# ZPP-Robotics/OSQP-Solver

Hardware: AMD Instinct MI355X
Metric: QPs/sec on a 1024-QP batch of box-QPs (n=512, m=1024), OSQP defaults; ADMM iters/sec alongside (higher is better)
Workload: dtype f64

## Files before the change

include/mi_osqp.h:

```cpp
#ifndef MI_OSQP_H
#define MI_OSQP_H

#include <stdint.h>

#ifdef __cplusplus
extern "C" {
#endif

typedef enum {
  MI_OSQP_OK = 0,
  MI_OSQP_ERR_INVALID_DATA = 1,
  MI_OSQP_ERR_INVALID_SETTINGS = 2,
  MI_OSQP_ERR_PATTERN_CHANGED = 3,
  MI_OSQP_ERR_NONCONVEX = 4,
  MI_OSQP_ERR_DEVICE = 5,
  MI_OSQP_ERR_NULL = 6,
  MI_OSQP_ERR_ALLOC = 7
} mi_osqp_error;

typedef enum {
  MI_OSQP_EXIT_OPTIMAL = 0,
  MI_OSQP_EXIT_PRIMAL_INFEASIBLE = 1,
  MI_OSQP_EXIT_DUAL_INFEASIBLE = 2,
  MI_OSQP_EXIT_OPTIMAL_INACCURATE = 3,
  MI_OSQP_EXIT_PRIMAL_INFEASIBLE_INACCURATE = 4,
  MI_OSQP_EXIT_DUAL_INFEASIBLE_INACCURATE = 5,
  MI_OSQP_EXIT_MAX_ITERATIONS = 6,
  MI_OSQP_EXIT_INTERRUPTED = 7,
  MI_OSQP_EXIT_TIME_LIMIT_REACHED = 8,
  MI_OSQP_EXIT_NON_CONVEX = 9,
  MI_OSQP_EXIT_UNKNOWN = 10
} mi_osqp_exit_code;

typedef struct {
  double  rho;
  double  sigma;
  int64_t scaling;
  int64_t adaptive_rho;
  int64_t adaptive_rho_interval;
  double  adaptive_rho_tolerance;
  int64_t max_iter;
  double  eps_abs;
  double  eps_rel;
  double  eps_prim_inf;
  double  eps_dual_inf;
  double  alpha;
  int64_t scaled_termination;
  int64_t check_termination;
  int64_t warm_start;
  int64_t verbose;
  int64_t polish;
  int64_t polish_refine_iter;
  double  delta;
} mi_osqp_settings;

typedef struct {
  int64_t iter;
  int64_t status_val;
  int64_t exit_code;
  double  obj_val;
  double  pri_res;
  double  dua_res;
  int64_t rho_updates;
  double  rho_estimate;
  double  rho;
  int64_t status_polish;
} mi_osqp_info;

typedef struct {
  int64_t n, m, N, batch, tile, n_tiles;
  int64_t nnz_P_triu, nnz_A, nnz_KKT, nnz_L;
  int64_t n_supernodes, n_blocks;
  int64_t fwd_levels, bwd_levels, fwd_slots, bwd_slots, chk_slots;
  int64_t lds_bytes, threads_per_block;
  int64_t dense_tail_rows, dense_tail_slots;
  double  setup_seconds_host, setup_seconds_factor, setup_seconds_upload;
  int64_t nnz_L_before_tail;
  int64_t solve_groups, solve_group_threads;
  int64_t resident_state, lds_bytes_iterate;
  int64_t pipelined_refactors;
  int64_t resident_factor_steps, lds_bytes_factor;
  int64_t dense_tail_tasks, dense_tail_waves_used, dense_tail_wave_tasks_max;
} mi_osqp_stats;

typedef struct mi_osqp_solver mi_osqp_solver;
typedef struct mi_osqp_batch  mi_osqp_batch;

void        mi_osqp_default_settings(mi_osqp_settings *s);
const char *mi_osqp_exit_code_name(int64_t exit_code);
const char *mi_osqp_error_name(int64_t err);
const char *mi_osqp_version(void);
const char *mi_osqp_last_error(void);

int mi_osqp_setup(mi_osqp_solver **out, int64_t n, int64_t m,
                  const int64_t *P_colptr, const int64_t *P_rowidx, const double *P_val,
                  const double *q,
                  const int64_t *A_colptr, const int64_t *A_rowidx, const double *A_val,
                  const double *l, const double *u, const mi_osqp_settings *settings);
int mi_osqp_update_A(mi_osqp_solver *h, const int64_t *A_colptr, const int64_t *A_rowidx,
                     const double *A_val);
int mi_osqp_update_bounds(mi_osqp_solver *h, const double *l, const double *u);
int mi_osqp_update_A_bounds(mi_osqp_solver *h, const int64_t *A_colptr, const int64_t *A_rowidx, const double *A_val,
                            const double *l, const double *u);
int mi_osqp_warm_start_x(mi_osqp_solver *h, const double *x);
int mi_osqp_update_q(mi_osqp_solver *h, const double *q);
int mi_osqp_update_P(mi_osqp_solver *h, const int64_t *P_colptr, const int64_t *P_rowidx, const double *P_val);
int mi_osqp_update_P_A(mi_osqp_solver *h, const int64_t *P_colptr, const int64_t *P_rowidx, const double *P_val,
                       const int64_t *A_colptr, const int64_t *A_rowidx, const double *A_val);
int mi_osqp_warm_start_y(mi_osqp_solver *h, const double *y);
int mi_osqp_solve(mi_osqp_solver *h, mi_osqp_info *info);
int mi_osqp_get_primal(mi_osqp_solver *h, double *x_out);
int mi_osqp_get_dual(mi_osqp_solver *h, double *y_out);
int mi_osqp_get_prim_inf_cert(mi_osqp_solver *h, double *dy_out );
int mi_osqp_get_dual_inf_cert(mi_osqp_solver *h, double *dx_out );
int mi_osqp_adjoint(mi_osqp_solver *h, const double *dx, const double *dy, double *dq, double *dP, double *dA, double *dl, double *du,
                    int32_t *status);
int mi_osqp_get_stats(mi_osqp_solver *h, mi_osqp_stats *st);
int mi_osqp_get_settings(mi_osqp_solver *h, mi_osqp_settings *out);
int mi_osqp_update_settings(mi_osqp_solver *h, const mi_osqp_settings *s);
void mi_osqp_free(mi_osqp_solver *h);

int mi_osqp_batch_setup(mi_osqp_batch **out, int64_t B, int64_t n, int64_t m,
                        const int64_t *P_colptr, const int64_t *P_rowidx, const double *P_val,
                        const double *q,
                        const int64_t *A_colptr, const int64_t *A_rowidx, const double *A_val,
                        const double *l, const double *u, const mi_osqp_settings *settings,
                        int64_t device);
int mi_osqp_batch_update_A(mi_osqp_batch *h, const int64_t *A_colptr, const int64_t *A_rowidx,
                           const double *A_val);
int mi_osqp_batch_update_bounds(mi_osqp_batch *h, const double *l, const double *u);
int mi_osqp_batch_update_A_bounds(mi_osqp_batch *h, const int64_t *A_colptr, const int64_t *A_rowidx, const double *A_val,
                                  const double *l, const double *u);
int mi_osqp_batch_warm_start_x(mi_osqp_batch *h, const double *x);
int mi_osqp_batch_update_q(mi_osqp_batch *h, const double *q);
int mi_osqp_batch_update_P(mi_osqp_batch *h, const int64_t *P_colptr, const int64_t *P_rowidx, const double *P_val);
int mi_osqp_batch_update_P_A(mi_osqp_batch *h, const int64_t *P_colptr, const int64_t *P_rowidx, const double *P_val,
                             const int64_t *A_colptr, const int64_t *A_rowidx, const double *A_val);
int mi_osqp_batch_warm_start_y(mi_osqp_batch *h, const double *y);
int mi_osqp_batch_get_P_upper_pattern(mi_osqp_batch *h, int64_t *colptr, int64_t *rowidx, int64_t *nnz_out);
int mi_osqp_batch_solve(mi_osqp_batch *h);
int mi_osqp_batch_get_primal(mi_osqp_batch *h, double *x_out );
int mi_osqp_batch_get_dual(mi_osqp_batch *h, double *y_out );
int mi_osqp_batch_get_info(mi_osqp_batch *h, mi_osqp_info *info );
int mi_osqp_batch_get_prim_inf_cert(mi_osqp_batch *h, double *dy_out );
int mi_osqp_batch_get_dual_inf_cert(mi_osqp_batch *h, double *dx_out );
int mi_osqp_batch_get_stats(mi_osqp_batch *h, mi_osqp_stats *st);
int mi_osqp_batch_get_ordering(mi_osqp_batch *h, int64_t *kkt_perm);
void mi_osqp_batch_free(mi_osqp_batch *h);
int mi_osqp_prefetch_analysis(int64_t B, int64_t n, int64_t m, const int64_t *Pp, const int64_t *Pi,
                              const int64_t *Ap, const int64_t *Ai, int64_t device);
void mi_osqp_release_device_cache(void);

int mi_osqp_batch_update_bounds_device(mi_osqp_batch *h, const double *d_l, const double *d_u, void *stream);
int mi_osqp_batch_update_A_bounds_device(mi_osqp_batch *h, const double *d_Av, const double *d_l, const double *d_u, void *stream);
int mi_osqp_batch_update_q_device(mi_osqp_batch *h, const double *d_q, void *stream);
int mi_osqp_batch_update_P_device(mi_osqp_batch *h, const double *d_Pv, void *stream);
int mi_osqp_batch_update_P_A_bounds_device(mi_osqp_batch *h, const double *d_Pv, const double *d_Av, const double *d_l, const double *d_u,
                                           void *stream);
int mi_osqp_batch_solve_device(mi_osqp_batch *h, double *d_x_out, int32_t *d_status, int32_t *d_iters, void *stream);
int mi_osqp_batch_reset(mi_osqp_batch *h);
int mi_osqp_batch_last_solve_stats(mi_osqp_batch *h, int64_t *total_iters, int64_t *kernel_launches,
                                   double *device_seconds, double *refactor_seconds, int64_t *refactor_count,
                                   double *compact_seconds);
int mi_osqp_batch_last_polish_stats(mi_osqp_batch *h, int64_t *polished, int64_t *accepted, double *seconds);
int mi_osqp_batch_get_polish_active(mi_osqp_batch *h, int8_t *act);
// ... 40 lines not shown
  MI_GOMP_MODEL_DH_CHAIN = 6
} mi_gomp_model;
typedef struct { int32_t model; int32_t is_gripper; double radius; double param[12]; } mi_gomp_ball;
typedef struct { double dir[2]; double point[3]; int32_t below; int32_t reserved; } mi_gomp_line;
typedef struct mi_gomp_scene mi_gomp_scene;
int mi_gomp_scene_create(mi_gomp_scene **out, mi_osqp_batch *h, int64_t dims, int64_t waypoints,
                         int64_t n_balls, const mi_gomp_ball *balls, int64_t n_lines, const mi_gomp_line *lines,
                         const double *con_lo, const double *con_hi);
typedef struct { int32_t n_joints; int32_t reserved; double a[8], d[8], alpha[8], theta0[8]; } mi_gomp_chain;
int mi_gomp_scene_create_chain(mi_gomp_scene **out, mi_osqp_batch *h, int64_t dims, int64_t waypoints,
                               const mi_gomp_chain *chain, int64_t n_balls, const mi_gomp_ball *balls,
                               int64_t n_lines, const mi_gomp_line *lines, const double *con_lo, const double *con_hi);
typedef struct { double a[3], b[3]; double radius; double margin; } mi_gomp_capsule;
int mi_gomp_scene_create_world(mi_gomp_scene **out, mi_osqp_batch *h, int64_t dims, int64_t waypoints,
                               const mi_gomp_chain *chain, int64_t n_balls, const mi_gomp_ball *balls,
                               int64_t n_lines, const mi_gomp_line *lines, int64_t n_capsules, const mi_gomp_capsule *capsules,
                               const double *con_lo, const double *con_hi);
void mi_gomp_scene_free(mi_gomp_scene *sc);
int mi_gomp_scene_set_rows(mi_gomp_scene *sc, int64_t n_ids, const int64_t *ids, const double *A_val, const double *l, const double *u);
int mi_gomp_scene_get_rows(mi_gomp_scene *sc, int64_t id, double *A_val, double *l, double *u);
int mi_gomp_assemble_some(mi_gomp_scene *sc, int64_t n_ids, const int64_t *ids, const double *x, int32_t *ok_out);
int mi_gomp_relinearise_some(mi_gomp_scene *sc, int64_t n_ids, const int64_t *ids, const double *x, int32_t *ok_out);

typedef struct mi_osqp_multi mi_osqp_multi;
int mi_osqp_multi_batch_setup(mi_osqp_multi **out, int64_t n_devices, const int64_t *devices,
                              int64_t B, int64_t n, int64_t m,
                              const int64_t *P_colptr, const int64_t *P_rowidx, const double *P_val,
                              const double *q,
                              const int64_t *A_colptr, const int64_t *A_rowidx, const double *A_val,
                              const double *l, const double *u, const mi_osqp_settings *settings);
int mi_osqp_multi_batch_update_A(mi_osqp_multi *h, const int64_t *A_colptr, const int64_t *A_rowidx, const double *A_val);
int mi_osqp_multi_batch_update_bounds(mi_osqp_multi *h, const double *l, const double *u);
int mi_osqp_multi_batch_update_A_bounds(mi_osqp_multi *h, const int64_t *A_colptr, const int64_t *A_rowidx, const double *A_val,
                                        const double *l, const double *u);
int mi_osqp_multi_batch_warm_start_x(mi_osqp_multi *h, const double *x);
int mi_osqp_multi_batch_update_q(mi_osqp_multi *h, const double *q);
int mi_osqp_multi_batch_update_P(mi_osqp_multi *h, const int64_t *P_colptr, const int64_t *P_rowidx, const double *P_val);
int mi_osqp_multi_batch_update_P_A(mi_osqp_multi *h, const int64_t *P_colptr, const int64_t *P_rowidx, const double *P_val,
                                   const int64_t *A_colptr, const int64_t *A_rowidx, const double *A_val);
int mi_osqp_multi_batch_warm_start_y(mi_osqp_multi *h, const double *y);
int mi_osqp_multi_batch_get_settings(mi_osqp_multi *h, mi_osqp_settings *out);
int mi_osqp_multi_batch_update_settings(mi_osqp_multi *h, const mi_osqp_settings *s);
int mi_osqp_multi_batch_update_rho_each(mi_osqp_multi *h, const double *rho );
int mi_osqp_multi_batch_solve(mi_osqp_multi *h);
int mi_osqp_multi_batch_solve_async(mi_osqp_multi *h);
int mi_osqp_multi_batch_wait(mi_osqp_multi *h);
int mi_osqp_multi_batch_get_primal(mi_osqp_multi *h, double *x_out );
int mi_osqp_multi_batch_get_dual(mi_osqp_multi *h, double *y_out );
int mi_osqp_multi_batch_get_info(mi_osqp_multi *h, mi_osqp_info *info );
int mi_osqp_multi_batch_get_prim_inf_cert(mi_osqp_multi *h, double *dy_out );
int mi_osqp_multi_batch_get_dual_inf_cert(mi_osqp_multi *h, double *dx_out );
int64_t mi_osqp_multi_batch_shards(mi_osqp_multi *h);
int mi_osqp_multi_batch_shard(mi_osqp_multi *h, int64_t k, int64_t *device, int64_t *begin, int64_t *end, mi_osqp_batch **handle);
void mi_osqp_multi_batch_free(mi_osqp_multi *h);

int mi_osqp_batch_spmv(mi_osqp_batch *h, const double *d_x, const double *d_y,
                       double *d_Px, double *d_Aty, double *d_Ax, void *stream);
int mi_osqp_batch_kkt_solve(mi_osqp_batch *h, const double *d_rhs, double *d_sol, void *stream);
int mi_osqp_batch_refactor_device(mi_osqp_batch *h);
int mi_osqp_batch_kernel_time(mi_osqp_batch *h, double *avg_ms, int64_t *launches);
int mi_osqp_batch_refactor_time(mi_osqp_batch *h, double *factor_ms, double *tail_ms, int64_t *launches, int64_t *qps);
int mi_osqp_batch_refactor_peak(mi_osqp_batch *h, int64_t *qps, double *factor_ms, double *tail_ms);

int mi_osqp_batch_get_scaling(mi_osqp_batch *h, double *D , double *E , double *c );

int mi_osqp_debug_host_kkt_solve(int64_t n, int64_t m,
                                 const int64_t *P_colptr, const int64_t *P_rowidx, const double *P_val,
                                 const int64_t *A_colptr, const int64_t *A_rowidx, const double *A_val,
                                 const double *l, const double *u, const mi_osqp_settings *settings,
                                 int64_t tile, const double *rhs ,
                                 double *sol_schedule , double *sol_direct ,
                                 mi_osqp_stats *st);

int mi_osqp_debug_host_block_factor(int64_t n, int64_t m,
                                    const int64_t *P_colptr, const int64_t *P_rowidx, const double *P_val,
                                    const int64_t *A_colptr, const int64_t *A_rowidx, const double *A_val,
                                    const double *l, const double *u, const mi_osqp_settings *settings,
                                    double *max_rel_diff_L, double *max_rel_diff_Dinv, int64_t *counts);

int mi_osqp_debug_refactor_chunks(int64_t n_flagged, const int64_t *flagged, int64_t n_active, const int64_t *active, int64_t tile,
                                  int64_t chunk_qps, int64_t max_chunks, int64_t *n_chunks, int64_t *work_begin, int64_t *tiles,
                                  int64_t *tile_begin);

int mi_osqp_debug_trace_kkt_solve(mi_osqp_batch *h, int32_t which, const double *d_rhs, double *d_sol,
                                  uint32_t *out, int64_t out_capacity_words, int64_t *dims);

#ifdef __cplusplus
}
#endif
#endif
```

osqp-solver_amd/__init__.py:

```python
import ctypes as C
import os

import numpy as np

try:
    import torch
except ImportError:
    torch = None

from . import build as _build

_HERE = os.path.dirname(os.path.abspath(__file__))
_LIB = None

EXIT_NAMES = ["kOptimal", "kPrimalInfeasible", "kDualInfeasible", "kOptimalInaccurate",
              "kPrimalInfeasibleInaccurate", "kDualInfeasibleInaccurate", "kMaxIterations",
              "kInterrupted", "kTimeLimitReached", "kNonConvex", "kUnknown"]
K_OPTIMAL = 0


class Settings(C.Structure):
    _fields_ = [("rho", C.c_double), ("sigma", C.c_double), ("scaling", C.c_int64),
                ("adaptive_rho", C.c_int64), ("adaptive_rho_interval", C.c_int64),
                ("adaptive_rho_tolerance", C.c_double), ("max_iter", C.c_int64),
                ("eps_abs", C.c_double), ("eps_rel", C.c_double), ("eps_prim_inf", C.c_double),
                ("eps_dual_inf", C.c_double), ("alpha", C.c_double), ("scaled_termination", C.c_int64),
                ("check_termination", C.c_int64), ("warm_start", C.c_int64), ("verbose", C.c_int64),
                ("polish", C.c_int64), ("polish_refine_iter", C.c_int64), ("delta", C.c_double)]


class Info(C.Structure):
    _fields_ = [("iter", C.c_int64), ("status_val", C.c_int64), ("exit_code", C.c_int64),
                ("obj_val", C.c_double), ("pri_res", C.c_double), ("dua_res", C.c_double),
                ("rho_updates", C.c_int64), ("rho_estimate", C.c_double), ("rho", C.c_double),
                ("status_polish", C.c_int64)]

    def as_dict(self):
        return {k: getattr(self, k) for k, _ in self._fields_}


class Stats(C.Structure):
    _fields_ = [(k, C.c_int64) for k in
                ("n", "m", "N", "batch", "tile", "n_tiles", "nnz_P_triu", "nnz_A", "nnz_KKT", "nnz_L",
                 "n_supernodes", "n_blocks", "fwd_levels", "bwd_levels", "fwd_slots", "bwd_slots",
                 "chk_slots", "lds_bytes", "threads_per_block", "dense_tail_rows", "dense_tail_slots")] + \
               [(k, C.c_double) for k in ("setup_seconds_host", "setup_seconds_factor", "setup_seconds_upload")] + \
               [("nnz_L_before_tail", C.c_int64), ("solve_groups", C.c_int64), ("solve_group_threads", C.c_int64),
                ("resident_state", C.c_int64), ("lds_bytes_iterate", C.c_int64), ("pipelined_refactors", C.c_int64),
                ("resident_factor_steps", C.c_int64), ("lds_bytes_factor", C.c_int64),
                ("dense_tail_tasks", C.c_int64), ("dense_tail_waves_used", C.c_int64), ("dense_tail_wave_tasks_max", C.c_int64)]

    def as_dict(self):
        return {k: getattr(self, k) for k, _ in self._fields_}


class MiOsqpError(RuntimeError):
    def __init__(self, code, where):
        self.code = int(code)
        L = lib()
        msg = L.mi_osqp_error_name(int(code)).decode()
        extra = L.mi_osqp_last_error().decode()
        super().__init__(f"{where}: error {int(code)} ({msg}) {extra}")


def lib():
    global _LIB
    if _LIB is None:
        path = os.path.join(_HERE, "libmi_osqp.so")
        if os.environ.get("MI_OSQP_LIBRARY"):
            path = os.environ["MI_OSQP_LIBRARY"]
        else:
            try:
                path = _build.build()
            except Exception as e:
                if not os.path.exists(path):
                    raise ImportError(f"libmi_osqp.so missing and could not be built: {e}") from e
        L = C.CDLL(path)
        ip, dp, vp = C.POINTER(C.c_int64), C.POINTER(C.c_double), C.c_void_p
        L.mi_osqp_default_settings.argtypes = [C.POINTER(Settings)]
        for f in ("mi_osqp_exit_code_name", "mi_osqp_error_name"):
            getattr(L, f).restype = C.c_char_p; getattr(L, f).argtypes = [C.c_int64]
        L.mi_osqp_version.restype = C.c_char_p
        L.mi_osqp_last_error.restype = C.c_char_p
        L.mi_osqp_batch_setup.argtypes = [C.POINTER(vp), C.c_int64, C.c_int64, C.c_int64, ip, ip, dp, dp, ip, ip, dp,
                                          dp, dp, C.POINTER(Settings), C.c_int64]
        L.mi_osqp_batch_update_A.argtypes = [vp, ip, ip, dp]
        L.mi_osqp_batch_update_A_bounds.argtypes = [vp, ip, ip, dp, dp, dp]
        L.mi_osqp_batch_update_bounds.argtypes = [vp, dp, dp]
        L.mi_osqp_batch_warm_start_x.argtypes = [vp, dp]
        L.mi_osqp_batch_update_q.argtypes = [vp, dp]
        L.mi_osqp_batch_update_q_device.argtypes = [vp, vp, vp]
        L.mi_osqp_batch_update_P.argtypes = [vp, ip, ip, dp]
        L.mi_osqp_batch_update_P_A.argtypes = [vp, ip, ip, dp, ip, ip, dp]
        L.mi_osqp_batch_warm_start_y.argtypes = [vp, dp]
        L.mi_osqp_batch_get_P_upper_pattern.argtypes = [vp, ip, ip, ip]
        L.mi_osqp_batch_update_P_device.argtypes = [vp, vp, vp]
        L.mi_osqp_batch_update_P_A_bounds_device.argtypes = [vp, vp, vp, vp, vp, vp]
        L.mi_osqp_batch_update_P_some.argtypes = [vp, C.c_int64, ip, dp]
        L.mi_osqp_batch_update_P_A_bounds_some.argtypes = [vp, C.c_int64, ip, dp, dp, dp, dp]
        L.mi_osqp_batch_update_q_some.argtypes = [vp, C.c_int64, ip, dp]
        L.mi_osqp_batch_warm_start_y_some.argtypes = [vp, C.c_int64, ip, dp]
        L.mi_osqp_settings_update_check.argtypes = [C.POINTER(Settings), C.POINTER(Settings)]
        L.mi_osqp_batch_get_settings.argtypes = [vp, C.POINTER(Settings)]
        L.mi_osqp_batch_update_settings.argtypes = [vp, C.POINTER(Settings)]
        L.mi_osqp_batch_update_rho_each.argtypes = [vp, dp]
        L.mi_osqp_batch_update_rho_some.argtypes = [vp, C.c_int64, ip, dp]
        L.mi_osqp_get_settings.argtypes = [vp, C.POINTER(Settings)]
        L.mi_osqp_update_settings.argtypes = [vp, C.POINTER(Settings)]
        L.mi_osqp_multi_batch_get_settings.argtypes = [vp, C.POINTER(Settings)]
        L.mi_osqp_multi_batch_update_settings.argtypes = [vp, C.POINTER(Settings)]
        L.mi_osqp_multi_batch_update_rho_each.argtypes = [vp, dp]
        L.mi_osqp_batch_solve.argtypes = [vp]
        L.mi_osqp_batch_get_primal.argtypes = [vp, dp]
        L.mi_osqp_batch_get_dual.argtypes = [vp, dp]
        L.mi_osqp_batch_get_info.argtypes = [vp, C.POINTER(Info)]
        for f in ("mi_osqp_get_prim_inf_cert", "mi_osqp_get_dual_inf_cert", "mi_osqp_batch_get_prim_inf_cert",
                  "mi_osqp_batch_get_dual_inf_cert", "mi_osqp_multi_batch_get_prim_inf_cert", "mi_osqp_multi_batch_get_dual_inf_cert"):
            getattr(L, f).argtypes = [vp, dp]
        L.mi_osqp_batch_get_prim_inf_cert_some.argtypes = [vp, C.c_int64, ip, dp]
        L.mi_osqp_batch_get_dual_inf_cert_some.argtypes = [vp, C.c_int64, ip, dp]
        L.mi_osqp_batch_get_stats.argtypes = [vp, C.POINTER(Stats)]
        L.mi_osqp_batch_get_ordering.argtypes = [vp, ip]
        L.mi_osqp_batch_free.argtypes = [vp]; L.mi_osqp_batch_free.restype = None
        L.mi_osqp_batch_update_bounds_device.argtypes = [vp, vp, vp, vp]
        L.mi_osqp_batch_update_A_bounds_device.argtypes = [vp, vp, vp, vp, vp]
        L.mi_osqp_batch_solve_device.argtypes = [vp, vp, vp, vp, vp]
        L.mi_osqp_batch_reset.argtypes = [vp]
        L.mi_osqp_batch_refactor_device.argtypes = [vp]
        L.mi_osqp_batch_last_solve_stats.argtypes = [vp, ip, ip, dp, dp, ip, dp]
        L.mi_osqp_batch_last_polish_stats.argtypes = [vp, ip, ip, dp]
        L.mi_osqp_batch_get_polish_active.argtypes = [vp, C.POINTER(C.c_int8)]
        L.mi_osqp_batch_adjoint.argtypes = [vp, dp, dp, dp, dp, dp, dp, dp, C.POINTER(C.c_int32)]
        L.mi_osqp_adjoint.argtypes = [vp, dp, dp, dp, dp, dp, dp, dp, C.POINTER(C.c_int32)]
        L.mi_osqp_batch_adjoint_device.argtypes = [vp] * 10
        L.mi_osqp_batch_get_scaling.argtypes = [vp, dp, dp, dp]
        L.mi_osqp_batch_spmv.argtypes = [vp, vp, vp, vp, vp, vp, vp]
        L.mi_osqp_batch_kkt_solve.argtypes = [vp, vp, vp, vp]
        L.mi_osqp_batch_kernel_time.argtypes = [vp, dp, ip]
        L.mi_osqp_batch_refactor_time.argtypes = [vp, dp, dp, ip, ip]
        L.mi_osqp_batch_refactor_peak.argtypes = [vp, ip, dp, dp]
        L.mi_osqp_batch_reinit_some.argtypes = [vp, C.c_int64, ip, dp, dp, dp]
        L.mi_osqp_batch_update_A_bounds_some.argtypes = [vp, C.c_int64, ip, dp, dp, dp]
        L.mi_osqp_batch_warm_start_x_some.argtypes = [vp, C.c_int64, ip, dp]
        L.mi_osqp_batch_solve_begin_some.argtypes = [vp, C.c_int64, ip]
        L.mi_osqp_batch_polish_some.argtypes = [vp, C.c_int64, ip]
        L.mi_osqp_batch_advance.argtypes = [vp, C.c_int64]
        L.mi_osqp_batch_poll.argtypes = [vp, C.c_int64, ip, ip, C.c_int64]
        L.mi_osqp_batch_get_primal_some.argtypes = [vp, C.c_int64, ip, dp]
        L.mi_osqp_batch_get_dual_some.argtypes = [vp, C.c_int64, ip, dp]
        L.mi_osqp_batch_get_info_some.argtypes = [vp, C.c_int64, ip, C.POINTER(Info)]
        L.mi_osqp_batch_running.argtypes = [vp]; L.mi_osqp_batch_running.restype = C.c_int64
        L.mi_osqp_batch_ring_wraps.argtypes = [vp]; L.mi_osqp_batch_ring_wraps.restype = C.c_int64
        L.mi_osqp_release_device_cache.argtypes = []; L.mi_osqp_release_device_cache.restype = None
        L.mi_osqp_setup.argtypes = [C.POINTER(vp), C.c_int64, C.c_int64, ip, ip, dp, dp, ip, ip, dp, dp, dp, C.POINTER(Settings)]
        L.mi_osqp_update_A.argtypes = [vp, ip, ip, dp]
        L.mi_osqp_update_bounds.argtypes = [vp, dp, dp]
        L.mi_osqp_warm_start_x.argtypes = [vp, dp]
        L.mi_osqp_update_q.argtypes = [vp, dp]
        L.mi_osqp_update_P.argtypes = [vp, ip, ip, dp]
        L.mi_osqp_update_P_A.argtypes = [vp, ip, ip, dp, ip, ip, dp]
        L.mi_osqp_warm_start_y.argtypes = [vp, dp]
        L.mi_osqp_solve.argtypes = [vp, C.POINTER(Info)]
        L.mi_osqp_get_primal.argtypes = [vp, dp]
        L.mi_osqp_get_dual.argtypes = [vp, dp]
        L.mi_osqp_get_stats.argtypes = [vp, C.POINTER(Stats)]
        L.mi_osqp_free.argtypes = [vp]; L.mi_osqp_free.restype = None
        L.mi_osqp_multi_batch_setup.argtypes = [C.POINTER(vp), C.c_int64, ip, C.c_int64, C.c_int64, C.c_int64, ip, ip, dp, dp,
                                                ip, ip, dp, dp, dp, C.POINTER(Settings)]
        L.mi_osqp_multi_batch_update_A.argtypes = [vp, ip, ip, dp]
        L.mi_osqp_multi_batch_update_bounds.argtypes = [vp, dp, dp]
        L.mi_osqp_multi_batch_update_A_bounds.argtypes = [vp, ip, ip, dp, dp, dp]
        L.mi_osqp_multi_batch_warm_start_x.argtypes = [vp, dp]
        L.mi_osqp_multi_batch_update_q.argtypes = [vp, dp]
        L.mi_osqp_multi_batch_update_P.argtypes = [vp, ip, ip, dp]
        L.mi_osqp_multi_batch_update_P_A.argtypes = [vp, ip, ip, dp, ip, ip, dp]
        L.mi_osqp_multi_batch_warm_start_y.argtypes = [vp, dp]
        L.mi_osqp_multi_batch_solve.argtypes = [vp]
        L.mi_osqp_multi_batch_solve_async.argtypes = [vp]
        L.mi_osqp_multi_batch_wait.argtypes = [vp]
        L.mi_osqp_multi_batch_get_primal.argtypes = [vp, dp]
        L.mi_osqp_multi_batch_get_dual.argtypes = [vp, dp]
        L.mi_osqp_multi_batch_get_info.argtypes = [vp, C.POINTER(Info)]
        L.mi_osqp_multi_batch_shards.argtypes = [vp]; L.mi_osqp_multi_batch_shards.restype = C.c_int64
        L.mi_osqp_multi_batch_shard.argtypes = [vp, C.c_int64, ip, ip, ip, C.POINTER(vp)]
        L.mi_osqp_multi_batch_free.argtypes = [vp]; L.mi_osqp_multi_batch_free.restype = None
        L.mi_osqp_debug_host_kkt_solve.argtypes = [C.c_int64, C.c_int64, ip, ip, dp, ip, ip, dp, dp, dp,
                                                   C.POINTER(Settings), C.c_int64, dp, dp, dp, C.POINTER(Stats)]
        L.mi_osqp_debug_refactor_chunks.argtypes = [C.c_int64, ip, C.c_int64, ip, C.c_int64, C.c_int64, C.c_int64, ip, ip, ip, ip]
        L.mi_osqp_prefetch_analysis.argtypes = [C.c_int64, C.c_int64, C.c_int64, ip, ip, ip, ip, C.c_int64]
        L.mi_osqp_debug_host_block_factor.argtypes = [C.c_int64, C.c_int64, ip, ip, dp, ip, ip, dp, dp, dp,
                                                      C.POINTER(Settings), dp, dp, ip]
        _LIB = L
    return _LIB


def host_cores():
    try:
        n = len(os.sched_getaffinity(0))
    except Exception:
        n = os.cpu_count() or 1
    for path in ("/sys/fs/cgroup/cpu.max",):
        try:
            quota, period = open(path).read().split()[:2]
            if quota != "max":
                n = min(n, max(1, int(round(int(quota) / int(period)))))
        except Exception:
            pass
    try:
        q = int(open("/sys/fs/cgroup/cpu/cpu.cfs_quota_us").read())
        p = int(open("/sys/fs/cgroup/cpu/cpu.cfs_period_us").read())
        if q > 0:
            n = min(n, max(1, int(round(q / p))))
    except Exception:
        pass
    return n


def default_settings(**kw):
    s = Settings()
    lib().mi_osqp_default_settings(C.byref(s))
    for k, v in kw.items():
        if not hasattr(s, k):
            raise KeyError(k)
        setattr(s, k, v)
    return s


class HandleSettings(Settings):

    def bind(self, getter):
        self._getter = getter
        return self

    def __call__(self):
        out = Settings()
        self._getter(out)
        C.memmove(C.byref(self), C.byref(out), C.sizeof(Settings))
        return out


def settings_update_check(in_force, wanted):
    return int(lib().mi_osqp_settings_update_check(C.byref(in_force), C.byref(wanted)))


def _handle_settings(kw, get_name, owner):
    import weakref
    hs = HandleSettings()
    C.memmove(C.byref(hs), C.byref(default_settings(**kw)), C.sizeof(Settings))
    ref = weakref.ref(owner)

    def getter(out):
        _chk(getattr(lib(), get_name)(ref()._h, C.byref(out)), get_name)
    return hs.bind(getter)


def _update_settings(self, fn_name, fields):
    s = self.settings()
    for k, v in fields.items():
        if not hasattr(s, k):
            raise KeyError(k)
        setattr(s, k, v)
    _chk(getattr(lib(), fn_name)(self._h, C.byref(s)), fn_name)
    return self.settings()


def _i64(a):
    return np.ascontiguousarray(a, dtype=np.int64)


def _f64(a):
    return np.ascontiguousarray(a, dtype=np.float64)
# ... 479 lines not shown

    def __init__(self, constraints, P, q=None, **settings):
        l, A, u = constraints
        self._b = BatchSolver(P, _csc(P).data, q, A, _csc(A).data, l, u, **settings)

    def update(self, constraints):
        l, A, u = constraints
        A = _csc(A)
        try:
            self._b.update_A(A.data, A_pattern=A)
            self._b.update_bounds(l, u)
        except MiOsqpError as e:
            raise ValueError(str(e)) from e

    def setWarmStart(self, x):
        self._b.warm_start_x(x)

    def update_settings(self, **fields):
        return self._b.update_settings(**fields)

    def solve(self):
        info = self._b.solve()[0]
        return int(info.exit_code), self._b.primal()[0]

    def info(self):
        return self._b.info()[0]

    def dual(self):
        return self._b.dual()[0]

    def prim_inf_cert(self):
        return self._b.prim_inf_cert()[0]

    def dual_inf_cert(self):
        return self._b.dual_inf_cert()[0]

    def adjoint(self, dx, dy=None):
        out = self._b.adjoint(dx, dy)
        return {k: (int(v[0]) if k == "status" else v[0]) for k, v in out.items()}

    def stats(self):
        return self._b.stats()


def debug_host_kkt_solve(P, A, l, u, rhs, tri_waves=0, **settings):
    L = lib()
    P, A = _csc(P), _csc(A)
    n, m = A.shape[1], A.shape[0]
    s = default_settings(**settings)
    rhs = _f64(rhs)
    sol_s, sol_d = np.empty(n + m), np.empty(n + m)
    st = Stats()
    Pp, Pi, Px = _i64(P.indptr), _i64(P.indices), _f64(P.data)
    Ap, Ai, Ax = _i64(A.indptr), _i64(A.indices), _f64(A.data)
    l, u = _f64(l), _f64(u)
    rc = L.mi_osqp_debug_host_kkt_solve(n, m, _ip(Pp), _ip(Pi), _dp(Px), _ip(Ap), _ip(Ai), _dp(Ax), _dp(l), _dp(u),
                                        C.byref(s), 1 + int(tri_waves), _dp(rhs), _dp(sol_s), _dp(sol_d), C.byref(st))
    _chk(rc, "debug_host_kkt_solve")
    return sol_s, sol_d, st.as_dict()


def prefetch_analysis(P, A, B=1, device=-1, check=True):
    L = lib()
    P, A = _csc(P), _csc(A)
    n, m = A.shape[1], A.shape[0]
    Pp, Pi, Ap, Ai = _i64(P.indptr), _i64(P.indices), _i64(A.indptr), _i64(A.indices)
    rc = L.mi_osqp_prefetch_analysis(B, n, m, _ip(Pp), _ip(Pi), _ip(Ap), _ip(Ai), device)
    if check:
        _chk(rc, "prefetch_analysis")
    return rc


def debug_refactor_chunks(flagged, active, tile, chunk_qps, max_chunks=8):
    f, a = _i64(flagged), _i64(active)
    nch = C.c_int64()
    wb = np.zeros(max_chunks + 2, dtype=np.int64); tb = np.zeros(max_chunks + 2, dtype=np.int64)
    tl = np.zeros(max(1, len(a)), dtype=np.int64)
    _chk(lib().mi_osqp_debug_refactor_chunks(len(f), _ip(f), len(a), _ip(a), tile, chunk_qps, max_chunks, C.byref(nch), _ip(wb), _ip(tl),
                                             _ip(tb)), "debug_refactor_chunks")
    k = int(nch.value)
    return ([f[wb[c]:wb[c + 1]].tolist() for c in range(k)], [tl[tb[c]:tb[c + 1]].tolist() for c in range(k)])


def debug_host_block_factor(P, A, l, u, **settings):
    L = lib()
    P, A = _csc(P), _csc(A)
    n, m = A.shape[1], A.shape[0]
    s = default_settings(**settings)
    Pp, Pi, Px = _i64(P.indptr), _i64(P.indices), _f64(P.data)
    Ap, Ai, Ax = _i64(A.indptr), _i64(A.indices), _f64(A.data)
    l, u = _f64(l), _f64(u)
    dL, dD = C.c_double(), C.c_double()
    cnt = (C.c_int64 * 4)()
    rc = L.mi_osqp_debug_host_block_factor(n, m, _ip(Pp), _ip(Pi), _dp(Px), _ip(Ap), _ip(Ai), _dp(Ax), _dp(l), _dp(u),
                                           C.byref(s), C.byref(dL), C.byref(dD), cnt)
    _chk(rc, "debug_host_block_factor")
    return dL.value, dD.value, dict(blocks=cnt[0], triples=cnt[1], storage=cnt[2], levels=cnt[3])
```

osqp-solver_amd/csrc/device_types.h:

```cpp
#pragma once
#include <hip/hip_runtime.h>
#include <stdint.h>

namespace miosqp {

#define MI_CHUNK 16

struct SchedDev {
  const uint32_t *step, *idxw;
  const uint64_t *idxw64;
  const uint32_t *lvl_pos, *tail_bar;
  int n_phases, nw, n_levels;
  uint32_t n_steps, n_slots;
};

struct DenseTailDev {
  int s, k, n_phases;
  uint32_t n_steps;
  const uint32_t *task;
  const uint32_t *wave_task, *wave_step, *tail_bar;
};

enum { DS_C = 0, DS_CINV, DS_RHO, DS_RHO_EST, DS_PRI_RES, DS_DUA_RES, DS_OBJ, DS_COUNT };
enum { IS_STATUS = 0, IS_ITER, IS_RHO_UPDATES, IS_DONE, IS_NEED_REFACTOR, IS_CUR, IS_PENDING, IS_EPOCH, IS_COUNT };

struct KernelArgs {
  int n, m, N, B;
  SchedDev fwd, bwd, chk;
  const uint32_t *pinv;
  const uint32_t *xloc;
  const double *fwd_val, *bwd_val, *chk_val, *dinv;
  DenseTailDev dt;
  const double *dt_val;
  const double *fwd_val0, *bwd_val0, *dt_val0;
  const int *use_work;
  double *x, *z, *y;
  const double *q, *l, *u, *rho_vec, *rho_inv, *Dsc, *Dsc_inv, *Esc, *Esc_inv;
  double *dx, *dy, *out1, *out2, *dscal;
  int *iscal;
  double *x_out, *y_out;
  double *cert_out;
  int cert_stride;
  double *xs_global;
  int xs_len;
  int rs_off;
  int rf_off;
  int wide;
  double sigma, alpha, eps_abs, eps_rel, eps_prim_inf, eps_dual_inf, rho_tolerance;
  int check_termination, rho_interval, max_iter, scaled_termination, scaling, adaptive_rho;
  int iter_begin, iter_end;
  int op_out_lds;
  int info_at_end;
  int mw_groups;
  unsigned *mw_bar;
  double *mw_scratch;
  int df;
  unsigned df_shadow;
  const unsigned char *rflag;
  const int *sel;
  const int *tiles;
};

struct FactorArgs {
  int n, m, N, B, nnzP, nnzK, pa_len, n_levels, force_all;
  int debug_skip;
  uint32_t storage;
  SchedDev fwd, bwd;
  const uint32_t *blk, *lvl, *utask, *tri4, *dtask, *ttask, *asm_dst, *asm_src;
  const uint32_t *ubig;
  int *use_work;
  const int32_t *fwd_srcblk, *bwd_srcblk;
  const double *pa_val, *l, *u, *dscal;
  double *rho_vec, *rho_inv, *Lblk, *Dl, *dinv_scratch, *fwd_val, *bwd_val, *dinv;
  int *iscal, *npos;
  int home_bt;
  const int *work;
  double sigma;
  int dt_k;
  int mw_groups;
  unsigned *mw_bar;
  const signed char *pmask;
  const int32_t *arow;
  int *pstat;
  double pdelta;
};

struct TailArgs {
  int n, N, s, k, kbt, home_bt;
  uint32_t storage, n_slots;
  int n_lt, n_ltcol;
  uint32_t n_quads;
  int nh;
  uint32_t cs_doubles;
  const int *work;
  const uint32_t *lt_pos, *ltcol_col, *tile_tab, *wave_tiles, *diag_tile;
  const uint64_t *asm_q64;
  const int32_t *src_tile;
  const uint32_t *dt_task, *dt_task_step;
  uint32_t n_tasks;
  const double *Lblk, *Dl;
  double *Sd, *dt_val, *dinv;
  int *npos, *iscal;
  unsigned long long *trace;
  int *pstat;
};
hipError_t launch_tail(const TailArgs &a, int nwork, size_t lds_asm, size_t lds, hipStream_t st);

struct PolishArgs {
  int *stat;
  signed char *act;
  double *sol;
  int refine_iter;
  int inner;
  double delta;
};
hipError_t launch_polish_active(const KernelArgs &a, const PolishArgs &p, int BT, hipStream_t st);
hipError_t launch_polish_active_list(const KernelArgs &a, const PolishArgs &p, const int *slots, int nslots, int BT, hipStream_t st);
hipError_t launch_polish_publish(const KernelArgs &a, const PolishArgs &p, const int *slots, int nslots, int *host_stat, int BT, hipStream_t st);
hipError_t launch_polish(const KernelArgs &a, const PolishArgs &p, int BT, int tiles, int threads, size_t lds, int n_cus, hipStream_t st);
struct AdjointArgs {
  const double *gx, *gy;
  double *dq, *dP, *dA, *dl, *du;
  const int32_t *prow, *pcol, *arow, *acol;
  int nnzP, nnzA;
};
hipError_t launch_adjoint(const KernelArgs &a, const PolishArgs &p, const AdjointArgs &g, int BT, int tiles, int threads, size_t lds, int n_cus, hipStream_t st);
hipError_t launch_adjoint_finish(const int *stat, const AdjointArgs &g, int32_t *status, int B, int n, int m, hipStream_t st);
hipError_t launch_factor(const FactorArgs &a, int BT, int tiles, int threads, hipStream_t st);
size_t factor_lds_bytes(int BT, int threads);
bool factor_fits_lds(const FactorArgs &a, int threads);

int max_coresident_groups(int threads, size_t lds, int n_cus);
int max_coresident_factor_groups(int threads, int n_cus);
hipError_t launch_iterate(const KernelArgs &a, int BT, int tiles, int threads, size_t lds, hipStream_t st);
int rf_head_steps();
int rf_lds_steps();
hipError_t launch_check(const KernelArgs &a, int BT, int tiles, int threads, size_t lds, hipStream_t st);
hipError_t launch_advance(const KernelArgs &a, int BT, int tiles, int threads, size_t lds, hipStream_t st, int max_segments, int seg_len,
                          int *host_is, double *host_ds, unsigned *stop, unsigned seq, unsigned *counter, unsigned *host_done);
hipError_t launch_spmv(const KernelArgs &a, int BT, int tiles, int threads, size_t lds, hipStream_t st,
                       const double *x, const double *y, double *Px, double *Aty, double *Ax);
struct SpmvFused {
  const uint32_t *ptr, *ent;
  const double *pa_val;
  int pa_len;
  const uint32_t *ell, *rowid;
  int n_pass;
  uint32_t ell_off[4], ell_k[4];
};
hipError_t launch_spmv_fused(const KernelArgs &a, const SpmvFused &t, int BT, int tiles, int n_cus, hipStream_t st,
                             const double *x, const double *y, double *Px, double *Aty, double *Ax);
size_t spmv_fused_lds_bytes(int n, int m, int pa_len, int BT);
hipError_t launch_kkt_solve(const KernelArgs &a, int BT, int tiles, int threads, size_t lds, hipStream_t st,
                            const double *rhs, double *sol);
hipError_t launch_kkt_trace(const KernelArgs &a, int BT, int tiles, int threads, size_t lds, hipStream_t st,
                            const double *rhs, double *sol, uint32_t *trace, uint32_t words);
hipError_t launch_warm_start(const KernelArgs &a, int BT, int tiles, int threads, size_t lds, hipStream_t st,
                             const double *x0);
hipError_t launch_interleave(const double *src, double *dst, const int *ids, int nq, int len, int BT, hipStream_t st);
hipError_t launch_scatter(const double *src, double *dst, const int *map, const int *ids, int nq, int srclen,
                          const SchedDev &sd, int BT, hipStream_t st);
hipError_t launch_deinterleave(const double *src, double *dst, int nq, int len, int BT, hipStream_t st);
struct RuizArgs {
  int n, m, nnzP, nnzA, B, BT, iters;
  const int *ids;
  int raw_by_qp;
  int fresh;
  const double *rawP, *rawq;
  const int32_t *Prow, *Pcol, *Arow, *Acol;
  const double *rawPnew;
  const double *rawA;
  const double *rawl, *rawu;
  double *pa_val, *q, *Dsc, *Dsc_inv, *Esc, *Esc_inv, *l, *u, *dscal;
  double *dn, *en;
  double *pa_out;
};
hipError_t launch_ruiz(const RuizArgs &a, hipStream_t st);
hipError_t launch_lin_cost(const double *gq, const int *ids, double *q, double *rawq, const double *Dsc, const double *dscal,
                           int nq, int n, int BT, int scaling, hipStream_t st);
hipError_t launch_warm_start_y(const KernelArgs &a, int nslots, int BT, hipStream_t st, const double *y0);
hipError_t launch_start_slots(const KernelArgs &a, const int *slots, const int *clear, int nslots, int BT, int cold, hipStream_t st);
hipError_t launch_fresh_slots(const KernelArgs &a, const int *slots, int nslots, int BT, double rho0, hipStream_t st);
hipError_t launch_set_rho_slots(const KernelArgs &a, const int *slots, const double *rho, double rho_all, int nslots, int BT, hipStream_t st);
hipError_t launch_worklist(const int *iscal, int *work, int nslots, int BT, hipStream_t st);
hipError_t launch_resume_flagged(const KernelArgs &a, int nslots, int BT, hipStream_t st);
hipError_t launch_copy_slot_streams(double *dst, const double *src, const int *slots, int nslots, size_t per, hipStream_t st);
hipError_t launch_keep_rows(double *dst, const double *src, const int *ids, int n_ids, int len, hipStream_t st);
hipError_t launch_copy_flagged_streams(double *dst, const double *src, const int *flags, int want, int nslots, size_t per, hipStream_t st);
hipError_t launch_copy_slot_rows(double *dst, const double *src, const int *slots, int nslots, int len, int BT, hipStream_t st);
enum { MI_GM_UR5E_FLANGE = 1, MI_GM_UR5E_WRIST3 = 2, MI_GM_UR5E_ELBOW = 3, MI_GM_YAW_2LINK = 4, MI_GM_TABLE = 5, MI_GM_DH_CHAIN = 6 };
#define MI_GOMP_MAXD 8
struct GompChainDev { int n_joints, pad; double a[MI_GOMP_MAXD], d[MI_GOMP_MAXD], ca[MI_GOMP_MAXD], sa[MI_GOMP_MAXD], theta0[MI_GOMP_MAXD]; };
struct GompBallDev { int model, is_gripper; double radius; double param[12]; };
struct GompLineDev { double D[3], A[3]; int below, pad; };
struct GompCapsuleDev { double a[3], e[3], ee, R, margin; };
struct GompArgs {
  int dims, W, n_balls, n_lines, n, m, nnzA, n_ids, row0, write_rows;
  int n_caps, pad;
  const int *ids;
  const GompBallDev *balls;
  const GompLineDev *lines;
  const GompCapsuleDev *caps;
  double con_lo[3], con_hi[3];
  const int *aidx;
  const double *traj;
  double *A, *l, *u;
  int *ok;
  GompChainDev chain;
};
hipError_t launch_gomp_relinearise(const GompArgs &g, hipStream_t st);
hipError_t launch_gather_status(const int *iscal, int32_t *status, int32_t *iters, int B, int BT, hipStream_t st);
hipError_t launch_fail_slots(const KernelArgs &a, const int *slots, int nfail, int BT, int iter, hipStream_t st);
hipError_t launch_bounds(const double *gl, const double *gu, double *l, double *u, const double *Esc,
                         const double *rho_vec, const double *dscal, int *changed, int B, int m, int BT,
                         int scaling, hipStream_t st);

}
```

osqp-solver_amd/csrc/host_core.cpp:

```cpp
#include "host_core.hpp"
#include "sched_format.h"

#include <algorithm>
#include <cmath>
#include <cstdio>
#include <cstdlib>
#include <cstring>
#include <numeric>
#include <set>
#include <chrono>
#include <thread>

#include "../../include/mi_osqp.h"

namespace miosqp {

int validate_settings(const Settings &s) {
  if (s.scaling < 0 || s.max_iter <= 0 || s.check_termination < 0) return 1;
  if (s.adaptive_rho != 0 && s.adaptive_rho != 1) return 1;
  if (s.adaptive_rho_interval < 0 || s.adaptive_rho_tolerance < 1.0) return 1;
  if (!(s.rho > 0.0) || !(s.sigma > 0.0)) return 1;
  if (s.eps_abs < 0.0 || s.eps_rel < 0.0 || (s.eps_abs == 0.0 && s.eps_rel == 0.0)) return 1;
  if (!(s.eps_prim_inf > 0.0) || !(s.eps_dual_inf > 0.0)) return 1;
  if (!(s.alpha > 0.0) || !(s.alpha < 2.0)) return 1;
// ... 841 lines not shown
        dt.lt_pos.push_back((uint32_t)bf.lpos[p]);
      }
    }
    dt.n_lt = (int)dt.lt_pos.size(); dt.n_ltcol = (int)dt.ltcol_col.size();
    const uint16_t zero_slot = (uint16_t)dt.n_lt;
    for (auto &fr : frag) for (auto &f : fr) for (uint16_t &v : f.second) if (v == 0xFFFFu) v = zero_slot;
    struct TileRec { int I, J; std::vector<std::pair<int, int>> src; };
    std::vector<TileRec> tiles;
    for (int I = 0; I < nt; I++)
      for (int J = 0; J <= I; J++) {
        TileRec t{I, J, {}};
        size_t a = 0, b = 0;
        while (a < frag[I].size() && b < frag[J].size()) {
          if (frag[I][a].first < frag[J][b].first) a++;
          else if (frag[I][a].first > frag[J][b].first) b++;
          else { t.src.push_back({(int)a, (int)b}); a++; b++; }
        }
        tiles.push_back(std::move(t));
      }
    const int nw = 16;
    std::vector<int> order(tiles.size());
    std::iota(order.begin(), order.end(), 0);
    std::stable_sort(order.begin(), order.end(), [&](int x, int y) { return tiles[x].src.size() > tiles[y].src.size(); });
    std::vector<std::vector<int>> mine(nw);
    for (size_t d = 0; d < order.size(); d++) { const size_t round = d / nw, pos = d % nw; mine[(round & 1) ? nw - 1 - pos : pos].push_back(order[d]); }
    dt.tile_tab.clear(); dt.wave_tiles.assign(nw + 1, 0u); dt.asm_q.clear(); dt.asm_qcol.clear();
    for (int w = 0; w < nw; w++) {
      dt.wave_tiles[w] = (uint32_t)(dt.tile_tab.size() / 4);
      for (int ti : mine[w]) {
        const TileRec &t = tiles[ti];
        const uint32_t q0 = (uint32_t)(dt.asm_q.size() / 64);
        const size_t padded = (t.src.size() + 31) / 32 * 32;
        for (size_t s0 = 0; s0 < padded; s0 += 4) {
          for (int g = 0; g < 4; g++) {
            const bool real = s0 + g < t.src.size();
            const auto *fa = real ? &frag[t.I][t.src[s0 + g].first] : nullptr;
            const auto *fb = real ? &frag[t.J][t.src[s0 + g].second] : nullptr;
            dt.asm_qcol.push_back(real ? (uint16_t)fa->first : (uint16_t)0);
            for (int e = 0; e < 16; e++) dt.asm_q.push_back(real ? ((uint32_t)fa->second[e] | ((uint32_t)fb->second[e] << 16)) : ((uint32_t)zero_slot | ((uint32_t)zero_slot << 16)));
          }
        }
        const uint32_t blk_id = find_blk(ct0 + t.I, ct0 + t.J);
        dt.tile_tab.insert(dt.tile_tab.end(), {((uint32_t)t.I << 16) | (uint32_t)t.J, bf.blk[4 * blk_id], q0, (uint32_t)(dt.asm_q.size() / 64)});
      }
    }
    dt.wave_tiles[nw] = (uint32_t)(dt.tile_tab.size() / 4);
    dt.asm_q64.resize(dt.asm_q.size());
    for (size_t e = 0; e < dt.asm_q.size(); e++) {
      const uint64_t w = dt.asm_q[e], ci = dt.asm_qcol[e / 16];
      dt.asm_q64[e] = ((w & 0xFFFFu) * 8u) | ((((w >> 16) * 8u) | ((ci * 8u) << 17)) << 32);
    }
    dt.src_tile.resize(dt.src.size());
    for (size_t e = 0; e < dt.src.size(); e++) {
      const int32_t sc = dt.src[e];
      dt.src_tile[e] = sc < 0 ? sc : (int32_t)dt_tile_offset(sc % k, sc / k);
    }
    dt.diag_tile.resize(k);
    for (int i = 0; i < k; i++) dt.diag_tile[i] = dt_tile_offset(i, i);
    dt.task_step.clear();
    { uint32_t pos = 0; for (size_t t = 0; t < dt.task.size() / 4; t++) { dt.task_step.push_back(pos); pos += dt.task[4 * t + 3]; } }
  }
}


Tuning tuning_from_env() {
  Tuning t;
  if (const char *e = getenv("MI_OSQP_TILE")) { const int v = atoi(e); if (v == 1 || v == 2 || v == 4) t.tile = v; }
  if (const char *e = getenv("MI_OSQP_THREADS")) t.threads = std::max(64, std::min(1024, atoi(e) / 64 * 64));
  t.global_xs = getenv("MI_OSQP_GLOBAL_XS") != nullptr;
  if (const char *e = getenv("MI_OSQP_GROUPS")) t.groups = std::max(0, std::min(256, atoi(e)));
  if (const char *e = getenv("MI_OSQP_GROUP_THREADS")) t.group_threads = std::max(64, std::min(512, atoi(e) / 64 * 64));
  if (const char *e = getenv("MI_OSQP_ASSUME_CUS")) t.assume_cus = std::max(0, atoi(e));
  if (const char *e = getenv("MI_OSQP_FACTOR_THREADS")) t.factor_threads = std::max(64, std::min(1024, atoi(e) / 64 * 64));
  if (const char *e = getenv("MI_OSQP_FACTOR_GROUPS")) t.factor_groups = std::max(1, std::min(256, atoi(e)));
  t.ruiz = getenv("MI_OSQP_HOST_RUIZ") ? 1 : getenv("MI_OSQP_DEVICE_RUIZ") ? -1 : 0;
  if (const char *e = getenv("MI_OSQP_CONT_RING_KB")) t.cont_ring_kb = std::max(0L, atol(e));
  if (const char *e = getenv("MI_OSQP_ANALYSIS_CACHE")) t.analysis_cache = atoi(e) != 0;
  t.stream_state = getenv("MI_OSQP_STREAM_STATE") != nullptr;
  t.stream_factor = getenv("MI_OSQP_STREAM_FACTOR") != nullptr;
  if (const char *e = getenv("MI_OSQP_REFACTOR_PIPELINE")) t.refactor_pipeline = atoi(e) != 0;
  if (const char *e = getenv("MI_OSQP_REFACTOR_PIPELINE_MIN")) t.pipeline_min = std::max(0, atoi(e));
  if (const char *e = getenv("MI_OSQP_REFACTOR_CHUNKS")) t.pipeline_chunks = std::max(0, std::min(8, atoi(e)));
  if (const char *e = getenv("MI_OSQP_REFACTOR_CHUNK_QPS")) t.pipeline_chunk_qps = std::max(0, atoi(e));
  AnalysisTuning &a = t.analysis;
  if (const char *e = getenv("MI_OSQP_DENSE_TAIL")) a.dense_tail = atoi(e);
  if (const char *e = getenv("MI_OSQP_ORDERING")) a.ordering = e[0];
  if (const char *e = getenv("MI_OSQP_ND_LEAF")) a.nd_leaf = atoi(e);
  if (const char *e = getenv("MI_OSQP_RELAX")) a.relax = atoi(e);
  a.serial = getenv("MI_OSQP_SERIAL_ANALYSIS") != nullptr;
  return t;
}

RefactorChunks refactor_chunks(const std::vector<int> &flagged, const std::vector<int> &active, int bt, int chunk_qps, int max_chunks) {
  RefactorChunks rc;
  const int nq = (int)flagged.size();
  max_chunks = std::max(1, max_chunks);
  chunk_qps = std::max(1, chunk_qps);
  if ((nq + chunk_qps - 1) / chunk_qps > max_chunks) chunk_qps = (nq + max_chunks - 1) / max_chunks;
  const int n_ref = (nq + chunk_qps - 1) / chunk_qps;
  rc.n_chunks = 1 + n_ref;
  rc.work_begin.assign(1, 0);
  for (int c = 0; c <= n_ref; c++) rc.work_begin.push_back(std::min(nq, c * chunk_qps));
  std::vector<std::pair<int, int>> tc;
  size_t f = 0;
  for (size_t i = 0; i < active.size(); i++) {
    const int tile = active[i] / bt;
    if (i && active[i - 1] / bt == tile) continue;
    int chunk = 0;
    while (f < flagged.size() && flagged[f] / bt < tile) f++;
    for (size_t g = f; g < flagged.size() && flagged[g] / bt == tile; g++) chunk = 1 + (int)g / chunk_qps;
    tc.emplace_back(chunk, tile);
  }
  std::stable_sort(tc.begin(), tc.end(), [](const std::pair<int, int> &x, const std::pair<int, int> &y) { return x.first < y.first; });
  rc.tile_begin.assign((size_t)rc.n_chunks + 1, 0);
  for (const auto &p : tc) { rc.tiles.push_back(p.second); rc.tile_begin[(size_t)p.first + 1]++; }
  for (int c = 0; c < rc.n_chunks; c++) rc.tile_begin[(size_t)c + 1] += rc.tile_begin[c];
  return rc;
}


int analyze(int64_t n64, int64_t m64, const int64_t *Pp, const int64_t *Pi, const int64_t *Ap,
            const int64_t *Ai, const AnalysisTuning &tune, Analysis &an, int nwaves, int bt, int max_extra_rows, int dense_tail_max, int tri_waves, int n_tiles) {
  if (nwaves < 1 || nwaves > 16 || (bt != 1 && bt != 2 && bt != 4) || tri_waves < 0 || tri_waves > 2048) return MI_OSQP_ERR_INVALID_SETTINGS;
  if (n64 <= 0 || m64 < 0 || !Pp || !Ap || n64 + m64 > (int64_t)1 << 30) return MI_OSQP_ERR_INVALID_DATA;
  int n = (int)n64, m = (int)m64, N = n + m;
  an = Analysis();
  an.n = n; an.m = m; an.N = N;
  if (Pp[0] != 0 || Ap[0] != 0) return MI_OSQP_ERR_INVALID_DATA;
  for (int j = 0; j < n; j++) {
    if (Pp[j + 1] < Pp[j] || Ap[j + 1] < Ap[j]) return MI_OSQP_ERR_INVALID_DATA;
    for (int64_t k = Pp[j]; k < Pp[j + 1]; k++) if (Pi[k] < 0 || Pi[k] >= n) return MI_OSQP_ERR_INVALID_DATA;
    for (int64_t k = Ap[j]; k < Ap[j + 1]; k++) if (Ai[k] < 0 || Ai[k] >= m) return MI_OSQP_ERR_INVALID_DATA;
  }
  if (Pp[n] > (int64_t)1 << 30 || Ap[n] > (int64_t)1 << 30) return MI_OSQP_ERR_INVALID_DATA;
  an.Pp.assign(n + 1, 0);
  for (int j = 0; j < n; j++) {
    an.Pp[j] = (int)an.Pi.size();
    for (int64_t k = Pp[j]; k < Pp[j + 1]; k++)
      if (Pi[k] <= j) { an.Pi.push_back((int)Pi[k]); an.Psrc.push_back((int)k); }
  }
  an.Pp[n] = (int)an.Pi.size();
  an.Ap.assign(Ap, Ap + n + 1);
  an.Ai.assign(Ai, Ai + Ap[n]);
  int nnzP = an.Pp[n], nnzA = an.Ap[n];
  std::vector<int> cnt(N, 0);
  an.PisDiag.assign(nnzP, 0);
  std::vector<char> hasDiag(n, 0);
  for (int j = 0; j < n; j++)
    for (int k = an.Pp[j]; k < an.Pp[j + 1]; k++) { cnt[j]++; if (an.Pi[k] == j) { hasDiag[j] = 1; an.PisDiag[k] = 1; } }
  for (int j = 0; j < n; j++) if (!hasDiag[j]) cnt[j]++;
  for (int k = 0; k < nnzA; k++) cnt[n + an.Ai[k]]++;
  for (int r = 0; r < m; r++) cnt[n + r]++;
  an.Kp.assign(N + 1, 0);
  for (int j = 0; j < N; j++) an.Kp[j + 1] = an.Kp[j] + cnt[j];
  an.Ki.assign(an.Kp[N], 0);
  an.PtoK.assign(nnzP, 0); an.AtoK.assign(nnzA, 0); an.rhotoK.assign(m, 0);
  std::vector<int> nxt(an.Kp.begin(), an.Kp.end() - 1);
  for (int j = 0; j < n; j++) {
    for (int k = an.Pp[j]; k < an.Pp[j + 1]; k++) { int pos = nxt[j]++; an.Ki[pos] = an.Pi[k]; an.PtoK[k] = pos; }
    if (!hasDiag[j]) { int pos = nxt[j]++; an.Ki[pos] = j; an.sigmaOnlyK.push_back(pos); }
  }
  for (int j = 0; j < n; j++)
    for (int k = an.Ap[j]; k < an.Ap[j + 1]; k++) { int pos = nxt[n + an.Ai[k]]++; an.Ki[pos] = j; an.AtoK[k] = pos; }
  for (int r = 0; r < m; r++) { int pos = nxt[n + r]++; an.Ki[pos] = n + r; an.rhotoK[r] = pos; }
  an.tri_waves = tri_waves;
  an.wide = N >= 65535 || 2 * n + m >= 65535 || tri_waves > 0;
  if (max_extra_rows < 0) max_extra_rows = 1 << 30;
  if (!an.wide && max_extra_rows > 65534 - N) max_extra_rows = 65534 - N;
  auto finalize = [&](Analysis &an, const std::vector<int> &perm0, double &cost, int relax_zeros = 0, int *phases_out = nullptr, double *stream_out = nullptr) {
    an.perm = perm0;
    an.pinv.assign(N, 0);
    for (int k = 0; k < N; k++) an.pinv[an.perm[k]] = k;
    build_permuted_lower(an);
    std::vector<std::vector<int>> cols;
    std::vector<int> parent, post;
    symbolic(an, cols, parent);
    postorder(parent, post);
    {
      std::vector<int> p2(N);
      for (int k = 0; k < N; k++) p2[k] = an.perm[post[k]];
      an.perm.swap(p2);
      for (int k = 0; k < N; k++) an.pinv[an.perm[k]] = k;
    }
    build_permuted_lower(an);
    symbolic(an, cols, parent);
    an.etree = parent;
    if (relax_zeros > 0) {
      auto close = [&](int s0, int e) {
        for (int c = s0; c < e; c++) {
          std::vector<int> ns;
          ns.reserve((size_t)(e - c) + cols[e].size());
          for (int r = c + 1; r <= e; r++) ns.push_back(r);
          ns.insert(ns.end(), cols[e].begin(), cols[e].end());
          cols[c].swap(ns);
        }
      };
      int s0 = 0;
      for (int j = 0; j < N; j++) {
        bool extend = false;
        if (j + 1 < N && parent[j] == j + 1 && j + 2 - s0 <= kChunk) {
// ... 712 lines not shown
```

osqp-solver_amd/csrc/host_core.hpp:

```cpp
#pragma once

#include <cstdint>
#include <string>
#include <vector>

namespace miosqp {

constexpr double kInfty = 1e30;
constexpr double kRhoMin = 1e-6, kRhoMax = 1e6, kRhoEqOverIneq = 1e3, kRhoTol = 1e-4;
constexpr double kMinScaling = 1e-4, kMaxScaling = 1e4;
constexpr double kDivisionTol = 1.0 / kInfty;
constexpr int kChunk = 16;
constexpr uint32_t kNoRow = 0xFFFFFFFFu;

struct Settings {
  double rho = 0.1, sigma = 1e-6;
  int64_t scaling = 10, adaptive_rho = 1, adaptive_rho_interval = 0;
  double adaptive_rho_tolerance = 5.0;
  int64_t max_iter = 4000;
  double eps_abs = 1e-3, eps_rel = 1e-3, eps_prim_inf = 1e-4, eps_dual_inf = 1e-4, alpha = 1.6;
  int64_t scaled_termination = 0, check_termination = 25, warm_start = 1, verbose = 0;
  int64_t polish = 0, polish_refine_iter = 3;
  double delta = 1e-6;
};
int validate_settings(const Settings &s);

struct AnalysisTuning {
  int dense_tail = -1;
  char ordering = 0;
  int nd_leaf = 0;
  int relax = -1;
  bool serial = false;
  bool operator==(const AnalysisTuning &o) const {
    return dense_tail == o.dense_tail && ordering == o.ordering && nd_leaf == o.nd_leaf && relax == o.relax && serial == o.serial;
  }
};
struct Tuning {
  int tile = 0;
  int threads = 0;
  bool global_xs = false;
  int groups = -1;
  int group_threads = 0;
  int assume_cus = 0;
  int factor_threads = 1024;
  int factor_groups = 0;
  int ruiz = 0;
  long cont_ring_kb = -1;
  bool analysis_cache = true;
  bool stream_state = false;
  bool stream_factor = false;
  bool refactor_pipeline = true;
  int pipeline_min = 0;
  int pipeline_chunks = 0;
  int pipeline_chunk_qps = 0;
  AnalysisTuning analysis;
};
Tuning tuning_from_env();

struct RefactorChunks {
  int n_chunks = 1;
  std::vector<int> work_begin;
  std::vector<int> tiles;
  std::vector<int> tile_begin;
};
RefactorChunks refactor_chunks(const std::vector<int> &flagged, const std::vector<int> &active, int bt, int chunk_qps, int max_chunks);

struct Schedule {
  int n_phases = 0, nw = 0, bt = 1;
  bool barriers = true;
  std::vector<uint32_t> phase;
  std::vector<int> level_first_phase;
  std::vector<uint32_t> step;
  std::vector<uint32_t> step_ob;
  std::vector<uint32_t> outA;
  std::vector<uint32_t> idx;
  std::vector<uint32_t> idxw;
  std::vector<uint64_t> idxw64;
  std::vector<int32_t> src;
  uint32_t n_slots = 0;
  uint32_t n_steps = 0;
  std::vector<uint32_t> wave_range;
  std::vector<uint32_t> lvl_pos;
  std::vector<uint32_t> tail_bar;
  bool dataflow = false;
  uint32_t shadow = 0, pad = 0;
  uint32_t phys_steps() const { return n_steps; }
  size_t phase_stride() const { return 4 * (size_t)nw + 1; }
  int n_levels = 0;
};

struct BlockFactor {
  uint32_t storage = 0;
  std::vector<uint32_t> blk;
  std::vector<uint32_t> lvl;
  std::vector<uint32_t> utask;
  std::vector<uint32_t> tri;
  std::vector<uint32_t> tri4;
  std::vector<uint32_t> utask4;
  bool overflow = false;
  std::vector<uint32_t> ubig;
  std::vector<uint32_t> dtask4;
  std::vector<uint32_t> ttask4;
  std::vector<uint32_t> dtask;
  std::vector<uint32_t> ttask;
  std::vector<uint32_t> asm_dst;
  std::vector<uint32_t> asm_src;
  std::vector<int32_t> lpos;
  int n_levels = 0;
  size_t n_blocks() const { return blk.size() / 4; }
};
enum { ASM_P = 0, ASM_P_SIGMA = 1, ASM_SIGMA = 2, ASM_A = 3, ASM_NEG_RHOINV = 4 };

struct DenseTail {
  int s = 0, k = 0, nb = 0;
  int nw = 0, n_phases = 0;
  uint32_t n_steps = 0;
  std::vector<uint32_t> task;
  std::vector<uint32_t> wave_task;
  std::vector<uint32_t> wave_step;
  std::vector<uint32_t> tail_bar;
  std::vector<int32_t> src;
  std::vector<uint32_t> sblk;
  int n_lt = 0, n_ltcol = 0;
  std::vector<uint32_t> lt_pos;
  std::vector<uint32_t> ltcol_col;
  std::vector<uint32_t> tile_tab;
  std::vector<uint32_t> wave_tiles;
  std::vector<uint32_t> asm_q;
  std::vector<uint16_t> asm_qcol;
  std::vector<uint64_t> asm_q64;
  std::vector<int32_t> src_tile;
  std::vector<uint32_t> diag_tile;
  std::vector<uint32_t> task_step;
  size_t asm_lds_bytes() const { return ((size_t)n_lt + 1 + (size_t)n_ltcol) * sizeof(double); }
};
inline uint32_t dt_tile_offset(int i, int j) {
  const int I = i / 16, J = j / 16, r = i % 16, c = j % 16;
  return (uint32_t)((I * (I + 1) / 2 + J) * 256 + ((r % 4) * 16 + c) * 4 + r / 4);
}
enum { DT_DIAG = 1, DT_SWAP = 2 };

struct Analysis {
  int n = 0, m = 0, N = 0;
  bool wide = false;
  std::vector<int> Pp, Pi, Psrc;
  std::vector<int> Ap, Ai;
  std::vector<int> Kp, Ki, PtoK, AtoK, rhotoK, sigmaOnlyK;
  std::vector<char> PisDiag;
// ... 65 lines not shown
```

osqp-solver_amd/csrc/kernels.hip:

```cpp
#include <hip/hip_runtime.h>
#include <stdint.h>
#include <stdlib.h>
#include <string.h>

#include <algorithm>
#include <map>
#include <mutex>

#include "device_types.h"
#include "sched_format.h"

namespace miosqp {

static hipError_t ensure_dynamic_lds(const void *kern, size_t lds);

#define MI_INFTY 1e30
#define MI_MIN_SCALING 1e-4
#define MI_DIV_TOL 1e-30
#define MI_RHO_EST_DIV 1e-10
#define MI_RHO_MIN 1e-6
#define MI_RHO_MAX 1e6
#define MI_NOROW 0xFFFFFFFFu
#ifdef MI_OSQP_DEBUG_BUILD
#define MI_DBG_SKIP(a) ((a).debug_skip)
// ... 2017 lines not shown
#define MI_QS(k, j) Ss[MI_BS(4 * g + (k), b, (j))]
#pragma unroll
  for (int k = 0; k < 4; k++) MI_QS(k, i) = (ok && (uint32_t)k < w) ? Lb[((size_t)off + k * w + i) * BT + b] : 0.0;
  wave_sync();
#pragma unroll
  for (int j = 0; j < 4; j++) {
    const bool on = ok && (uint32_t)j < w;
    const double d = MI_QS(j, j);
    const double di = 1.0 / d;
    double lij = 0.0;
    if (on && i > j) { lij = MI_QS(j, i) * di; MI_QS(j, i) = lij; }
    if (on && i == j) {
      Dl[((size_t)c0 + j) * BT + b] = d; dinv[((size_t)c0 + j) * BT + b] = di;
      if (d > 0.0) npos++;
    }
    wave_sync();
    if (on && i > j) {
      const double ld = lij * d;
      for (int k = j + 1; k <= i; k++) MI_QS(k, i) -= ld * MI_QS(j, k);
    }
    wave_sync();
  }
  if (ok) { for (int k = 0; k < i; k++) Lb[((size_t)off + k * w + i) * BT + b] = MI_QS(k, i); }
#pragma unroll
  for (int j = 2; j >= 0; j--) {
    const bool on = ok && (uint32_t)(j + 2) <= w && i > j;
    double x = 0.0;
    if (on) {
      x = -MI_QS(j, i);
      for (int p2 = j + 1; p2 < i; p2++) x = fma(-MI_QS(p2, i), MI_QS(j, p2), x);
    }
    wave_sync();
    if (on) MI_QS(j, i) = x;
    wave_sync();
  }
  if (ok && w >= 2) { for (int k = 0; k < i; k++) Lb[((size_t)off + (size_t)i * w + k) * BT + b] = MI_QS(k, i); }
}
template <int BT>
__device__ __forceinline__ void fct_trsm_quad(double *Lb, const double *dinv, double *Ss, const uint4 td, const bool valid, int lane) {
  const int g = lane / (MI_CHUNK * BT), i = (lane / BT) % MI_CHUNK, b = lane % BT;
  const uint32_t off = td.x, h = td.z >> 8, w = td.z & 255u, c0 = td.y, db_off = td.w;
#pragma unroll
  for (int k = 0; k < 4; k++) MI_QS(k, i) = (valid && (uint32_t)k < w && (uint32_t)i < w && i > k) ? Lb[((size_t)db_off + k * w + i) * BT + b] : 0.0;
  wave_sync();
  if (valid && (uint32_t)i < h) {
    double ld[4];
#pragma unroll
    for (int j = 0; j < 4; j++) {
      if ((uint32_t)j < w) {
        double v = Lb[((size_t)off + j * h + i) * BT + b];
#pragma unroll
        for (int k = 0; k < j; k++) v = fma(-ld[k], MI_QS(k, j), v);
        ld[j] = v;
        Lb[((size_t)off + j * h + i) * BT + b] = v * dinv[((size_t)c0 + j) * BT + b];
      }
    }
  }
  wave_sync();
#undef MI_QS
}

template <int BT, bool LBL = false>
__global__ __launch_bounds__(1024) void factor_kernel(FactorArgs a) {
  extern __shared__ double smem[];
  bool multi = false;
  if constexpr (BT == 1) multi = a.mw_groups > 1;
  const unsigned G = multi ? (unsigned)a.mw_groups : 1u;
  const int tile = (int)(blockIdx.x / G), gidx = (int)(blockIdx.x % G);
  const Mw mw{a.mw_bar + 4 * (size_t)tile, G};
  const int tid = gidx * (int)blockDim.x + (int)threadIdx.x, nthr = (int)(blockDim.x * G);
  const int lane = tid & 63, wave = __builtin_amdgcn_readfirstlane(tid >> 6), nw = nthr >> 6, b = tid % BT;
  auto sync = [&]() { if constexpr (BT == 1) wg_or_grid_barrier(mw); else __syncthreads(); };
  const int m = a.m, N = a.N;
  const int slot = a.work ? a.work[tile * BT + b] : tile * BT + b;
  const size_t hbt = (size_t)a.home_bt;
  const size_t home = slot >= 0 ? (size_t)slot / hbt : 0, hb = slot >= 0 ? (size_t)slot % hbt : 0;
  auto H = [&](size_t len, size_t i) { return (home * len + i) * hbt + hb; };
  int flag = 0;
  if (slot >= 0) flag = a.work ? 1 : (a.force_all ? (slot < a.B) : a.iscal[H(IS_COUNT, IS_NEED_REFACTOR)]);
  if (!__syncthreads_or(flag)) return;
  double *Ss = smem + (size_t)(threadIdx.x >> 6) * MI_CHUNK * MI_CHUNK * BT;
  double *lds_rest = smem + (size_t)(blockDim.x >> 6) * MI_CHUNK * MI_CHUNK * BT;
  double *Lb, *Dl;
  if constexpr (LBL) { Lb = lds_rest; Dl = lds_rest + (size_t)a.storage * BT; }
  else { Lb = a.Lblk + (size_t)tile * a.storage * BT; Dl = a.Dl + (size_t)tile * N * BT; }
  const double rho = a.dscal[H(DS_COUNT, DS_RHO)];
  if (flag && !a.force_all && !a.pmask) {
    for (int e = tid; e < m * BT; e += nthr) {
      const size_t k = H(m, e / BT);
      const double l = a.l[k], u = a.u[k];
      double rv;
      if (l < -MI_INFTY * MI_MIN_SCALING && u > MI_INFTY * MI_MIN_SCALING) rv = MI_RHO_MIN;
      else if (u - l < 1e-4) rv = 1e3 * rho;
      else rv = rho;
      a.rho_vec[k] = rv; a.rho_inv[k] = 1.0 / rv;
    }
  }
  {
    const size_t tot = (size_t)a.storage * BT, pairs = tot / 2;
    double2 *L2p = reinterpret_cast<double2 *>(Lb);
    for (size_t e = tid; e < pairs; e += nthr) L2p[e] = make_double2(0.0, 0.0);
    if (tid == 0 && (tot & 1)) Lb[tot - 1] = 0.0;
    if (multi && tid == 0 && slot >= 0) a.npos[slot] = 0;
  }
  sync();
  {
    constexpr int UA = 2;
    const int tot = a.nnzK * BT;
    for (int e0 = tid; e0 < tot; e0 += nthr * UA) {
      uint32_t src[UA], dst[UA];
      double v[UA];
#pragma unroll
      for (int u = 0; u < UA; u++) {
        const int e = e0 + u * nthr;
        const int k = e < tot ? e / BT : 0;
        src[u] = a.asm_src[k]; dst[u] = a.asm_dst[k];
      }
#pragma unroll
      for (int u = 0; u < UA; u++) {
        const uint32_t kind = src[u] >> 29, idx = src[u] & 0x1FFFFFFFu;
        if (kind == 0) v[u] = a.pa_val[H(a.pa_len, idx)];
        else if (kind == 1) v[u] = a.pa_val[H(a.pa_len, idx)] + a.sigma;
        else if (kind == 2) v[u] = a.sigma;
        else if (kind == 3) {
          const bool off = a.pmask && (slot < 0 || a.pmask[(size_t)slot * m + a.arow[idx]] == 0);
          v[u] = off ? 0.0 : a.pa_val[H(a.pa_len, (size_t)a.nnzP + idx)];
        }
        else v[u] = a.pmask ? -a.pdelta : -a.rho_inv[H(m, idx)];
      }
#pragma unroll
      for (int u = 0; u < UA; u++) if (e0 + u * nthr < tot) Lb[(size_t)dst[u] * BT + b] = v[u];
    }
  }
  sync();
  int npos = 0, bad_inertia = 0;
  double *dnew;
  if constexpr (LBL) dnew = lds_rest + ((size_t)a.storage + (size_t)N) * BT;
  else dnew = a.dinv_scratch + (size_t)tile * N * BT;
  for (int L = 0; L < a.n_levels; L++) {
    const uint32_t *lv = a.lvl + 6 * L;
    const uint4 *ut4 = reinterpret_cast<const uint4 *>(a.utask), *dt4 = reinterpret_cast<const uint4 *>(a.dtask), *tt4 = reinterpret_cast<const uint4 *>(a.ttask);
    if (lv[1] > lv[0]) {
      uint32_t ub = lv[1];
      if constexpr (BT <= 2) { if (!(MI_DBG_SKIP(a) & 32)) ub = a.ubig[3 * L]; }
      uint32_t t = lv[0] + wave;
      uint4 nxt = t < ub ? ut4[t] : make_uint4(0, 0, 0, 0);
      for (; t < ub; t += nw) {
        const uint4 cur = nxt;
        if (t + nw < ub) nxt = ut4[t + nw];
        fct_update<BT>(a, Lb, Dl, Ss, cur, lane);
      }
      if constexpr (BT <= 2) {
        constexpr uint32_t NG = 64 / (MI_CHUNK * BT);
        const uint32_t g = (uint32_t)lane / (MI_CHUNK * BT);
        uint32_t tq = ub + NG * (uint32_t)wave;
        uint4 nq = tq + g < lv[1] ? ut4[tq + g] : make_uint4(0, 0, 0, 0);
        for (; tq < lv[1]; tq += NG * (uint32_t)nw) {
          const uint4 cur = nq;
          const bool valid = tq + g < lv[1];
          const uint32_t tn = tq + NG * (uint32_t)nw + g;
          if (tn < lv[1]) nq = ut4[tn];
          fct_update_quad<BT>(a, Lb, Dl, Ss, cur, valid, lane);
        }
      }
      sync();
    }
    if (!(MI_DBG_SKIP(a) & 4)) {
      uint32_t db = lv[3];
      if constexpr (BT <= 2) { if (!(MI_DBG_SKIP(a) & 32)) db = a.ubig[3 * L + 1]; }
      uint32_t t = lv[2] + wave;
      uint4 nxt = t < db ? dt4[t] : make_uint4(0, 0, 0, 0);
      for (; t < db; t += nw) {
        const uint4 cur = nxt;
        if (t + nw < db) nxt = dt4[t + nw];
        fct_diag<BT>(a, Lb, Dl, dnew, Ss, cur, lane, npos);
      }
      if constexpr (BT <= 2) {
        constexpr uint32_t NG = 64 / (MI_CHUNK * BT);
        const uint32_t g = (uint32_t)lane / (MI_CHUNK * BT);
        uint32_t tq = db + NG * (uint32_t)wave;
        uint4 nq = tq + g < lv[3] ? dt4[tq + g] : make_uint4(0, 0, 0, 0);
        for (; tq < lv[3]; tq += NG * (uint32_t)nw) {
          const uint4 cur = nq;
          const bool valid = tq + g < lv[3];
          const uint32_t tn = tq + NG * (uint32_t)nw + g;
          if (tn < lv[3]) nq = dt4[tn];
          fct_diag_quad<BT>(Lb, Dl, dnew, Ss, cur, valid, lane, npos);
        }
      }
    }
    sync();
    if (lv[5] > lv[4] && !(MI_DBG_SKIP(a) & 8)) {
      uint32_t tbg = lv[5];
      if constexpr (BT <= 2) { if (!(MI_DBG_SKIP(a) & 32)) tbg = a.ubig[3 * L + 2]; }
      uint32_t t = lv[4] + wave;
      uint4 nxt = t < tbg ? tt4[t] : make_uint4(0, 0, 0, 0);
      for (; t < tbg; t += nw) {
        const uint4 cur = nxt;
        if (t + nw < tbg) nxt = tt4[t + nw];
        fct_trsm<BT>(a, Lb, Dl, dnew, Ss, cur, lane);
      }
      if constexpr (BT <= 2) {
        constexpr uint32_t NG = 64 / (MI_CHUNK * BT);
        const uint32_t g = (uint32_t)lane / (MI_CHUNK * BT);
        uint32_t tq = tbg + NG * (uint32_t)wave;
        uint4 nq = tq + g < lv[5] ? tt4[tq + g] : make_uint4(0, 0, 0, 0);
        for (; tq < lv[5]; tq += NG * (uint32_t)nw) {
          const uint4 cur = nq;
          const bool valid = tq + g < lv[5];
          const uint32_t tn = tq + NG * (uint32_t)nw + g;
          if (tn < lv[5]) nq = tt4[tn];
          fct_trsm_quad<BT>(Lb, dnew, Ss, cur, valid, lane);
        }
      }
      sync();
    }
  }
  {
    __shared__ int s_npos[4];
    if (threadIdx.x < 4) s_npos[threadIdx.x] = 0;
    __syncthreads();
// ... 3 lines not shown
      if (threadIdx.x == 0 && slot >= 0 && s_npos[0]) atomicAdd(&a.npos[slot], s_npos[0]);
      sync();
      if (threadIdx.x == 0 && slot >= 0) s_npos[0] = __hip_atomic_load(&a.npos[slot], __ATOMIC_RELAXED, __HIP_MEMORY_SCOPE_AGENT);
      __syncthreads();
    } else if (tid < BT && slot >= 0) a.npos[slot] = s_npos[b];
    if (tid < BT && flag && s_npos[b] != a.n && !MI_DBG_SKIP(a) && !a.dt_k) bad_inertia = 1;
  }
  if (flag && !(MI_DBG_SKIP(a) & 16)) {
    double *fv = a.fwd_val + (size_t)slot * a.fwd.n_steps * 64, *bv = a.bwd_val + (size_t)slot * a.bwd.n_steps * 64;
    auto scatter = [&](double *dst, const int32_t *map, uint32_t n_slots) {
      constexpr int US = 4;
      const uint32_t tot = n_slots * (uint32_t)BT;
      for (uint32_t e0 = tid; e0 < tot; e0 += (uint32_t)nthr * US) {
        int32_t mp[US];
        double v[US];
#pragma unroll
        for (int u = 0; u < US; u++) { const uint32_t e = e0 + (uint32_t)(u * nthr); mp[u] = e < tot ? map[e / BT] : MI_SRC_ZERO; }
#pragma unroll
        for (int u = 0; u < US; u++) v[u] = slot_value(mp[u], Lb, BT, b);
#pragma unroll
        for (int u = 0; u < US; u++) { const uint32_t e = e0 + (uint32_t)(u * nthr); if (e < tot) dst[e / BT] = v[u]; }
      }
    };
    scatter(fv, a.fwd_srcblk, a.fwd.n_slots);
    scatter(bv, a.bwd_srcblk, a.bwd.n_slots);
    for (int e = tid; e < N * BT; e += nthr) a.dinv[H(N, e / BT)] = dnew[e];
  }
  if (tid < BT && slot >= 0 && flag && a.use_work) a.use_work[slot] = 1;
  sync();
  __threadfence();
  if (a.pmask) { if (tid < BT && slot >= 0 && bad_inertia) a.pstat[slot] = -1; }
  else if (tid < BT && slot >= 0) a.iscal[H(IS_COUNT, IS_NEED_REFACTOR)] = bad_inertia ? -1 : 0;
}

template <int BT, bool LBL = false>
static hipError_t launch_factor_t(const FactorArgs &a, int tiles, int threads, hipStream_t st) {
  size_t lds = factor_lds_bytes(BT, threads);
  if (LBL) lds += ((size_t)a.storage + 2 * (size_t)a.N) * BT * sizeof(double);
  if (a.mw_groups > 1) { if (BT != 1 || !a.mw_bar || LBL) return hipErrorInvalidValue; tiles *= a.mw_groups; }
#ifdef MI_OSQP_DEBUG_BUILD
  if (a.mw_groups > 1 && debug_drop_group("factor")) tiles--;
#endif
  hipError_t e = ensure_dynamic_lds(reinterpret_cast<const void *>(&factor_kernel<BT, LBL>), lds);
  if (e != hipSuccess) return e;
  hipLaunchKernelGGL((factor_kernel<BT, LBL>), dim3(tiles), dim3(threads), lds, st, a);
  return hipGetLastError();
}
size_t factor_lds_bytes(int BT, int threads) { return (size_t)(threads / 64) * MI_CHUNK * MI_CHUNK * BT * sizeof(double); }
bool factor_fits_lds(const FactorArgs &a, int threads) {
  return !a.dt_k && factor_lds_bytes(1, threads) + ((size_t)a.storage + 2 * (size_t)a.N) * sizeof(double) <= 160 * 1024 - 1024;
}
hipError_t launch_factor(const FactorArgs &a, int BT, int tiles, int threads, hipStream_t st) {
  if (BT == 1 && a.mw_groups <= 1 && factor_fits_lds(a, threads)) return launch_factor_t<1, true>(a, tiles, threads, st);
  switch (BT) {
    case 1: return launch_factor_t<1>(a, tiles, threads, st);
    case 2: return launch_factor_t<2>(a, tiles, threads, st);
    default: return launch_factor_t<4>(a, tiles, threads, st);
  }
}


typedef double mi_v4d __attribute__((ext_vector_type(4)));
__device__ __forceinline__ mi_v4d mfma_f64(double a, double b, mi_v4d c) { return __builtin_amdgcn_mfma_f64_16x16x4f64(a, b, c, 0, 0, 0); }
__device__ __forceinline__ mi_v4d ld_tile(const double *A, uint32_t tix, int lane) {
  const double2 *p = reinterpret_cast<const double2 *>(A + (size_t)tix * 256 + (size_t)lane * 4);
  const double2 v0 = p[0], v1 = p[1];
  return mi_v4d{v0.x, v0.y, v1.x, v1.y};
}
__device__ __forceinline__ void st_tile(double *A, uint32_t tix, int lane, mi_v4d v) {
  double2 *p = reinterpret_cast<double2 *>(A + (size_t)tix * 256 + (size_t)lane * 4);
  p[0] = make_double2(v[0], v[1]); p[1] = make_double2(v[2], v[3]);
}
__device__ __forceinline__ uint32_t tile_ix(int I, int J) { return (uint32_t)(I * (I + 1) / 2 + J); }

#define MI_TAIL_NW 8
#define MI_TAIL_TS 65

__global__ __launch_bounds__(1024) void tail_assemble_kernel(TailArgs a) {
  extern __shared__ double smem[];
  const int g = blockIdx.x, tid = threadIdx.x, nthr = blockDim.x;
  const int lane = tid & 63, wave = __builtin_amdgcn_readfirstlane(tid >> 6);
  const int slot = a.work[g];
  if (slot < 0) return;
  const int k = a.k, kbt = a.kbt, wt = g / kbt, wb = g % kbt;
  double *A = a.Sd + (size_t)g * k * k;
  const double *Lb = a.Lblk + (size_t)wt * a.storage * kbt + wb;
  const double *Dl = a.Dl + (size_t)wt * a.N * kbt + wb;
  const int l15 = lane & 15, l4 = lane >> 4;
  {
    double *La = smem, *Dc = smem + a.n_lt + 1;
    for (int e = tid; e < a.n_lt; e += nthr) La[e] = Lb[(size_t)a.lt_pos[e] * kbt];
    if (tid == 0) La[a.n_lt] = 0.0;
    for (int c = tid; c < a.n_ltcol; c += nthr) Dc[c] = -Dl[(size_t)a.ltcol_col[c] * kbt];
    __syncthreads();
    constexpr int QB = 8;
    const uint32_t t_begin = a.wave_tiles[wave], t_end = a.wave_tiles[wave + 1];
    if (t_begin < t_end) {
      const uint4 *ttab = reinterpret_cast<const uint4 *>(a.tile_tab);
      auto load_init = [&](const uint4 &tt) {
        const int I = (int)(tt.x >> 16), J = (int)(tt.x & 0xFFFFu);
        mi_v4d v;
#pragma unroll
        for (int r = 0; r < 4; r++) {
          int row = l4 + 4 * r, col = l15;
          if (I == J && row < col) { const int t = row; row = col; col = t; }
          v[r] = Lb[((size_t)tt.y + (size_t)col * 16 + row) * kbt];
        }
        return v;
      };
      const mi_rsrc tab = make_rsrc(a.asm_q64, a.n_quads * 512u);
      const uint32_t q_last = a.n_quads ? a.n_quads - 1 : 0u;
      mi_u32x2 nxt[QB];
      auto fetch = [&](uint32_t qb) {
#pragma unroll
        for (int u = 0; u < QB; u++) {
          const uint32_t q = qb + u < q_last ? qb + u : q_last;
          nxt[u] = __builtin_amdgcn_raw_buffer_load_b64(tab, (uint32_t)lane * 8u, q * 512u, 0);
        }
      };
#pragma unroll
      for (int u = 0; u < QB; u++) nxt[u] = mi_u32x2{0u, 0u};
      uint32_t qnext = ttab[t_begin].z;
      if (a.n_quads) { fetch(qnext); qnext += QB; }
      const char *lds = reinterpret_cast<const char *>(smem);
      const uint32_t dc_off = (uint32_t)(a.n_lt + 1) * 8u;
      mi_v4d acc_next = load_init(ttab[t_begin]);
      for (uint32_t ti = t_begin; ti < t_end; ti++) {
        const uint4 tt = ttab[ti];
        mi_v4d acc = acc_next;
        acc_next = load_init(ttab[ti + 1 < t_end ? ti + 1 : ti]);
        for (uint32_t q = tt.z; q < tt.w; q += QB) {
          mi_u32x2 cur[QB];
#pragma unroll
          for (int u = 0; u < QB; u++) cur[u] = nxt[u];
          fetch(qnext); qnext += QB;
          double av[QB], bv[QB];
#pragma unroll
          for (int u = 0; u < QB; u++) {
            av[u] = *reinterpret_cast<const double *>(lds + cur[u].x);
            bv[u] = *reinterpret_cast<const double *>(lds + (cur[u].y & 0x1FFFFu)) * *reinterpret_cast<const double *>(lds + dc_off + (cur[u].y >> 17));
          }
#pragma unroll
          for (int u = 0; u < QB; u++) acc = mfma_f64(av[u], bv[u], acc);
        }
        st_tile(A, tile_ix((int)(tt.x >> 16), (int)(tt.x & 0xFFFFu)), lane, acc);
      }
    }
  }
}

template <int MI_TAIL_MAXSLOT, int PFT>
__global__ __launch_bounds__(512) void tail_kernel(TailArgs a) {
  extern __shared__ double smem[];
  const int g = blockIdx.x, tid = threadIdx.x, nthr = blockDim.x;
  const int lane = tid & 63, wave = __builtin_amdgcn_readfirstlane(tid >> 6);
  const int slot = a.work[g];
  if (slot < 0) return;
  const int k = a.k, kbt = a.kbt, wt = g / kbt, wb = g % kbt, nt = k / 16;
  const size_t hbt = (size_t)a.home_bt, home = (size_t)slot / hbt, hb = (size_t)slot % hbt;
  auto H = [&](size_t len, size_t i) { return (home * len + i) * hbt + hb; };
  double *A = a.Sd + (size_t)g * k * k;
  (void)wt; (void)wb;
  const int l15 = lane & 15, l4 = lane >> 4;
  unsigned long long tr_t = a.trace ? __builtin_amdgcn_s_memtime() : 0ull, tr_acc[8] = {0ull, 0ull, 0ull, 0ull, 0ull, 0ull, 0ull, 0ull};
  auto stamp = [&](int which) {
    if (a.trace && wave == 0) { const unsigned long long t = __builtin_amdgcn_s_memtime(); tr_acc[which] += t - tr_t; tr_t = t; }
  };
  stamp(0);
  const int nrt = nt - 4;
  const int nh = a.nh;
  double *Cs = smem;
  double *Ps = smem + (size_t)a.cs_doubles;
  double *Ts = Cs;
  int npos = 0;
  for (int p = 0; p < k / 64; p++) {
    const int P0 = 4 * p;
    auto nonp = [&](int x) { return x < P0 ? x : x + 4; };
    for (int t = wave; t < 10; t += MI_TAIL_NW) {
      int ta = 0, tb = t;
      while (tb > ta) { tb -= ta + 1; ta++; }
      const mi_v4d v = ld_tile(A, tile_ix(P0 + ta, P0 + tb), lane);
#pragma unroll
      for (int r = 0; r < 4; r++) {
        const int row = 16 * ta + l4 + 4 * r, col = 16 * tb + l15;
        if (ta != tb || row >= col) {
          Ts[row * MI_TAIL_TS + col] = v[r];
          Ts[col * MI_TAIL_TS + row] = v[r];
        }
      }
    }
    __syncthreads();
    for (int q = 0; q < 4; q++) {
      if (wave == 0) {
        double *U = Ts + (16 * q) * MI_TAIL_TS + 16 * q;
        double *rowbuf = Ps;
        const int r = l15, c0 = l4 * 4;
        double u[4];
#pragma unroll
        for (int cc = 0; cc < 4; cc++) u[cc] = U[r * MI_TAIL_TS + c0 + cc];
        for (int kk = 0; kk < 16; kk++) {
          if (r == kk) {
#pragma unroll
            for (int cc = 0; cc < 4; cc++) rowbuf[c0 + cc] = u[cc];
          }
          wave_sync();
          const double d = rowbuf[kk], ta = rowbuf[r];
          double tb[4];
#pragma unroll
          for (int cc = 0; cc < 4; cc++) tb[cc] = rowbuf[c0 + cc];
          wave_sync();
          if (lane == 0 && d > 0.0) npos++;
          double di = __builtin_amdgcn_rcp(d);
          di = fma(fma(-d, di, 1.0), di, di);
          di = fma(fma(-d, di, 1.0), di, di);
#pragma unroll
          for (int cc = 0; cc < 4; cc++) {
            const int c = c0 + cc;
            double v;
            if (r != kk && c != kk) v = fma(-(ta * tb[cc]), di, u[cc]);
            else if (r == kk && c == kk) v = -di;
            else if (c == kk) v = ta * di;
            else v = tb[cc] * di;
            u[cc] = v;
          }
        }
#pragma unroll
        for (int cc = 0; cc < 4; cc++) U[r * MI_TAIL_TS + c0 + cc] = u[cc];
      }
      __syncthreads();
      int ta = -1;
      mi_v4d gnT = {0.0, 0.0, 0.0, 0.0};
      if (wave < 3) {
        ta = wave < q ? wave : wave + 1;
#pragma unroll
        for (int s = 0; s < 4; s++)
          gnT = mfma_f64(Ts[(16 * q + l15) * MI_TAIL_TS + 16 * q + 4 * s + l4], Ts[(16 * ta + l15) * MI_TAIL_TS + 16 * q + 4 * s + l4], gnT);
        for (int bi = 0; bi < 3; bi++) {
          const int tb = bi < q ? bi : bi + 1;
          mi_v4d acc;
#pragma unroll
          for (int r = 0; r < 4; r++) acc[r] = Ts[(16 * ta + l4 + 4 * r) * MI_TAIL_TS + 16 * tb + l15];
#pragma unroll
          for (int s = 0; s < 4; s++) acc = mfma_f64(gnT[s], Ts[(16 * tb + l15) * MI_TAIL_TS + 16 * q + 4 * s + l4], acc);
#pragma unroll
// ... 190 lines not shown
    hipLaunchKernelGGL(kern, dim3(nwork), dim3(512), lds, st, a);
    return hipGetLastError();
  };
  const int slots = (a.k / 16 - 4 + MI_TAIL_NW - 1) / MI_TAIL_NW;
  if (slots <= 1) return go(&tail_kernel<1, 4>);
  if (slots == 2) return go(&tail_kernel<2, 4>);
  if (slots == 3) return go(&tail_kernel<3, 4>);
  return go(&tail_kernel<4, 4>);
}


__global__ void interleave_kernel(const double *__restrict__ src, double *dst, const int *ids, int nq,
                                  int len, int BT) {
  const size_t g = (size_t)blockIdx.x * blockDim.x + threadIdx.x;
  if (g >= (size_t)nq * len) return;
  const int j = (int)(g / len), i = (int)(g % len);
  const int q = ids ? ids[j] : j;
  dst[((size_t)(q / BT) * len + i) * BT + (q % BT)] = src[g];
}
__global__ void scatter_kernel(const double *__restrict__ src, double *dst, const int *__restrict__ map,
                               const int *ids, int nq, int srclen, SchedDev sd, int BT) {
  const size_t g = (size_t)blockIdx.x * blockDim.x + threadIdx.x;
  const uint32_t slots = sd.n_slots;
  if (g >= (size_t)nq * slots) return;
  const int j = (int)(g / slots);
  const uint32_t s = (uint32_t)(g % slots);
  const int q = ids ? ids[j] : j;
  dst[(size_t)q * slots + s] = slot_value(map[s], src + (size_t)j * srclen, 1, 0);
  (void)BT;
}
__global__ void deinterleave_kernel(const double *__restrict__ src, double *dst, int nq, int len, int BT) {
  const size_t g = (size_t)blockIdx.x * blockDim.x + threadIdx.x;
  if (g >= (size_t)nq * len) return;
  const int q = (int)(g / len), i = (int)(g % len);
  dst[g] = src[((size_t)(q / BT) * len + i) * BT + (q % BT)];
}
__global__ void gather_status_kernel(const int *__restrict__ iscal, int32_t *status, int32_t *iters, int B, int BT) {
  const int q = blockIdx.x * blockDim.x + threadIdx.x;
  if (q >= B) return;
  const int *t = iscal + (size_t)(q / BT) * IS_COUNT * BT;
  if (status) status[q] = t[IS_STATUS * BT + q % BT];
  if (iters) iters[q] = t[IS_ITER * BT + q % BT];
}
__global__ void fail_slots_kernel(KernelArgs a, const int *__restrict__ slots, int BT, int iter) {
  const int slot = slots[blockIdx.x], tid = threadIdx.x, nthr = blockDim.x;
  if (slot < 0) return;
  const size_t tile = (size_t)slot / BT, b = (size_t)slot % BT;
  const int qp = slot < a.B ? slot : -1;
  const double nanv = __builtin_nan("");
  for (int i = tid; i < a.n; i += nthr) {
    a.x[(tile * a.n + i) * BT + b] = 0.0;
    if (qp >= 0) a.x_out[(size_t)qp * a.n + i] = nanv;
  }
  for (int j = tid; j < a.m; j += nthr) {
    a.z[(tile * a.m + j) * BT + b] = 0.0; a.y[(tile * a.m + j) * BT + b] = 0.0;
    if (qp >= 0) a.y_out[(size_t)qp * a.m + j] = nanv;
  }
  if (tid == 0) {
    int *is = a.iscal + tile * IS_COUNT * BT;
    is[IS_DONE * BT + b] = 1; is[IS_STATUS * BT + b] = -7; is[IS_NEED_REFACTOR * BT + b] = 0; is[IS_ITER * BT + b] = iter;
    double *ds = a.dscal + tile * DS_COUNT * BT;
    ds[DS_OBJ * BT + b] = nanv; ds[DS_PRI_RES * BT + b] = nanv; ds[DS_DUA_RES * BT + b] = nanv;
  }
}
hipError_t launch_fail_slots(const KernelArgs &a, const int *slots, int nfail, int BT, int iter, hipStream_t st) {
  if (!nfail) return hipSuccess;
  hipLaunchKernelGGL(fail_slots_kernel, dim3(nfail), dim3(256), 0, st, a, slots, BT, iter);
  return hipGetLastError();
}
__device__ __forceinline__ void fail_one_slot(const KernelArgs &a, int slot, int BT, int iter, int tid, int nthr) {
  const size_t tile = (size_t)slot / BT, b = (size_t)slot % BT;
  const double nanv = __builtin_nan("");
  for (int i = tid; i < a.n; i += nthr) { a.x[(tile * a.n + i) * BT + b] = 0.0; if (slot < a.B) a.x_out[(size_t)slot * a.n + i] = nanv; }
  for (int j = tid; j < a.m; j += nthr) {
    a.z[(tile * a.m + j) * BT + b] = 0.0; a.y[(tile * a.m + j) * BT + b] = 0.0;
    if (slot < a.B) a.y_out[(size_t)slot * a.m + j] = nanv;
  }
  if (tid == 0) {
    int *is = a.iscal + tile * IS_COUNT * BT;
    is[IS_DONE * BT + b] = 1; is[IS_STATUS * BT + b] = -7; is[IS_ITER * BT + b] = iter;
    double *ds = a.dscal + tile * DS_COUNT * BT;
    ds[DS_OBJ * BT + b] = nanv; ds[DS_PRI_RES * BT + b] = nanv; ds[DS_DUA_RES * BT + b] = nanv;
  }
}
__global__ void start_slots_kernel(KernelArgs a, const int *__restrict__ slots, const int *__restrict__ clear, int BT, int cold) {
  const int slot = slots[blockIdx.x], tid = threadIdx.x, nthr = blockDim.x;
  if (slot < 0) return;
  const size_t tile = (size_t)slot / BT, b = (size_t)slot % BT;
  int *is = a.iscal + tile * IS_COUNT * BT;
  if (is[IS_NEED_REFACTOR * BT + b] < 0) {
    fail_one_slot(a, slot, BT, 0, tid, nthr);
    __syncthreads();
    if (tid == 0) { is[IS_PENDING * BT + b] = 0; __threadfence_system(); is[IS_EPOCH * BT + b] += 1; }
    return;
  }
  if (cold) {
    for (int i = tid; i < a.n; i += nthr) a.x[(tile * a.n + i) * BT + b] = 0.0;
    for (int j = tid; j < a.m; j += nthr) { a.z[(tile * a.m + j) * BT + b] = 0.0; a.y[(tile * a.m + j) * BT + b] = 0.0; }
  }
  __syncthreads();
  if (tid == 0) {
    is[IS_STATUS * BT + b] = -10; is[IS_ITER * BT + b] = 0; is[IS_NEED_REFACTOR * BT + b] = 0;
    is[IS_CUR * BT + b] = 0;
    if (clear[blockIdx.x]) is[IS_RHO_UPDATES * BT + b] = 0;
    __threadfence();
    __hip_atomic_store(&is[IS_PENDING * BT + b], 1, __ATOMIC_RELEASE, __HIP_MEMORY_SCOPE_AGENT);
    __threadfence();
    is[IS_EPOCH * BT + b] += 1;
  }
}
hipError_t launch_start_slots(const KernelArgs &a, const int *slots, const int *clear, int nslots, int BT, int cold, hipStream_t st) {
  if (!nslots) return hipSuccess;
  hipLaunchKernelGGL(start_slots_kernel, dim3(nslots), dim3(256), 0, st, a, slots, clear, BT, cold);
  return hipGetLastError();
}
__global__ void fresh_slots_kernel(KernelArgs a, const int *__restrict__ slots, int BT, double rho0) {
  const int slot = slots[blockIdx.x], tid = threadIdx.x, nthr = blockDim.x;
  if (slot < 0) return;
  const size_t tile = (size_t)slot / BT, b = (size_t)slot % BT;
  for (int i = tid; i < a.n; i += nthr) { a.x[(tile * a.n + i) * BT + b] = 0.0; a.dx[(tile * a.n + i) * BT + b] = 0.0; }
  for (int j = tid; j < a.m; j += nthr) { a.z[(tile * a.m + j) * BT + b] = 0.0; a.y[(tile * a.m + j) * BT + b] = 0.0; a.dy[(tile * a.m + j) * BT + b] = 0.0; }
  if (tid == 0) {
    int *is = a.iscal + tile * IS_COUNT * BT;
    is[IS_STATUS * BT + b] = -10; is[IS_ITER * BT + b] = 0; is[IS_RHO_UPDATES * BT + b] = 0; is[IS_DONE * BT + b] = 1;
    is[IS_NEED_REFACTOR * BT + b] = 0; is[IS_CUR * BT + b] = 0; is[IS_PENDING * BT + b] = 0;
    double *ds = a.dscal + tile * DS_COUNT * BT;
    ds[DS_RHO * BT + b] = rho0; ds[DS_RHO_EST * BT + b] = rho0; ds[DS_PRI_RES * BT + b] = 0.0; ds[DS_DUA_RES * BT + b] = 0.0; ds[DS_OBJ * BT + b] = 0.0;
  }
}
hipError_t launch_fresh_slots(const KernelArgs &a, const int *slots, int nslots, int BT, double rho0, hipStream_t st) {
  if (!nslots) return hipSuccess;
  hipLaunchKernelGGL(fresh_slots_kernel, dim3(nslots), dim3(256), 0, st, a, slots, BT, rho0);
  return hipGetLastError();
}
__global__ void set_rho_slots_kernel(KernelArgs a, const int *__restrict__ slots, const double *__restrict__ rho, double rho_all, int nslots, int BT) {
  const int j = (int)(blockIdx.x * blockDim.x + threadIdx.x);
  if (j >= nslots) return;
  const int slot = slots ? slots[j] : j;
  if (slot < 0) return;
  const size_t tile = (size_t)slot / BT, b = (size_t)slot % BT;
  a.dscal[(tile * DS_COUNT + DS_RHO) * BT + b] = rho ? rho[j] : rho_all;
}
hipError_t launch_set_rho_slots(const KernelArgs &a, const int *slots, const double *rho, double rho_all, int nslots, int BT, hipStream_t st) {
  if (nslots <= 0) return hipSuccess;
  hipLaunchKernelGGL(set_rho_slots_kernel, dim3((nslots + 255) / 256), dim3(256), 0, st, a, slots, rho, rho_all, nslots, BT);
  return hipGetLastError();
}
__global__ __launch_bounds__(1024) void worklist_kernel(const int *__restrict__ iscal, int *work, int nslots, int BT) {
  __shared__ int s_cnt;
  if (threadIdx.x == 0) s_cnt = 0;
  for (int s = threadIdx.x; s < nslots; s += blockDim.x) work[s] = -1;
  __syncthreads();
  for (int s = threadIdx.x; s < nslots; s += blockDim.x)
    if (iscal[(size_t)(s / BT) * IS_COUNT * BT + IS_NEED_REFACTOR * BT + s % BT] == 1) work[atomicAdd(&s_cnt, 1)] = s;
}
hipError_t launch_worklist(const int *iscal, int *work, int nslots, int BT, hipStream_t st) {
  hipLaunchKernelGGL(worklist_kernel, dim3(1), dim3(1024), 0, st, iscal, work, nslots, BT);
  return hipGetLastError();
}
__global__ void resume_flagged_kernel(KernelArgs a, int BT) {
  const int slot = blockIdx.x, tid = threadIdx.x, nthr = blockDim.x;
  const size_t tile = (size_t)slot / BT, b = (size_t)slot % BT;
  int *is = a.iscal + tile * IS_COUNT * BT;
  if (is[IS_PENDING * BT + b] != 2) return;
  const int flag = is[IS_NEED_REFACTOR * BT + b];
  if (flag == 1) return;
// ... 790 lines not shown
```

osqp-solver_amd/csrc/solver.hip:

```cpp
#include <hip/hip_runtime.h>
#include <time.h>

#include <algorithm>
#include <atomic>
#include <chrono>
#include <cmath>
#include <condition_variable>
#include <functional>
#include <limits>
#include <cstdio>
#include <cstdlib>
#include <cstring>
#include <string>
#include <thread>
#include <map>
#include <memory>
#include <mutex>
#include <vector>

#include "../../include/mi_osqp.h"
#include "device_types.h"
#include "host_core.hpp"

using namespace miosqp;
// ... 62 lines not shown
      fclose(f);
    }
    long long q1 = -1, p1 = 0;
    if (FILE *f = fopen("/sys/fs/cgroup/cpu/cpu.cfs_quota_us", "r")) { if (fscanf(f, "%lld", &q1) != 1) q1 = -1; fclose(f); }
    if (FILE *f = fopen("/sys/fs/cgroup/cpu/cpu.cfs_period_us", "r")) { if (fscanf(f, "%lld", &p1) != 1) p1 = 0; fclose(f); }
    if (q1 > 0 && p1 > 0) t = std::min<long long>(t, std::max<long long>(1, (q1 + p1 / 2) / p1));
  }
  cached = std::max(1, std::min(t, 128));
  return cached;
}

template <class F>
static void parallel_for(int count, F &&fn) {
  int nt = std::min(host_threads(), count);
  if (nt <= 1) { for (int i = 0; i < count; i++) fn(i, 0); return; }
  std::atomic<int> next{0};
  std::vector<std::thread> th;
  for (int t = 0; t < nt; t++)
    th.emplace_back([&, t]() { for (int i; (i = next.fetch_add(1)) < count;) fn(i, t); });
  for (auto &x : th) x.join();
}

namespace devpool {
static std::mutex mu;
static std::multimap<std::pair<int, size_t>, void *> blocks;
static size_t kept = 0;
constexpr size_t kMaxKept = (size_t)8 << 30;
static void *take(int dev, size_t bytes, size_t &cap) {
  std::lock_guard<std::mutex> lk(mu);
  auto it = blocks.lower_bound({dev, bytes});
  if (it == blocks.end() || it->first.first != dev || it->first.second > 2 * bytes + 4096) return nullptr;
  void *p = it->second; cap = it->first.second; kept -= cap;
  blocks.erase(it);
  return p;
}
static bool give(int dev, void *p, size_t cap) {
  std::lock_guard<std::mutex> lk(mu);
  if (kept + cap > kMaxKept) return false;
  blocks.emplace(std::make_pair(dev, cap), p); kept += cap;
  return true;
}
static void release_all() {
  std::lock_guard<std::mutex> lk(mu);
  for (auto &b : blocks) (void)hipFree(b.second);
  blocks.clear(); kept = 0;
}
}

namespace hostpool {
static std::mutex mu;
static std::multimap<size_t, void *> blocks;
static size_t kept = 0;
constexpr size_t kMaxKept = (size_t)1 << 30;
static void *take(size_t bytes, size_t &cap) {
  std::lock_guard<std::mutex> lk(mu);
  auto it = blocks.lower_bound(bytes);
  if (it == blocks.end() || it->first > 4 * bytes + 65536) return nullptr;
  void *p = it->second; cap = it->first; kept -= cap;
  blocks.erase(it);
  return p;
}
static void give(void *p, size_t cap) {
  if (!p) return;
  {
    std::lock_guard<std::mutex> lk(mu);
    if (kept + cap <= kMaxKept) { blocks.emplace(cap, p); kept += cap; return; }
  }
  (void)hipHostFree(p);
}
static void release_all() {
  std::lock_guard<std::mutex> lk(mu);
  for (auto &b : blocks) (void)hipHostFree(b.second);
  blocks.clear(); kept = 0;
}
static hipError_t alloc(void **p, size_t bytes, size_t *cap) {
  bytes = (bytes + 4095) & ~(size_t)4095;
  if (void *q = take(bytes, *cap)) { *p = q; return hipSuccess; }
  *cap = bytes;
  return hipHostMalloc(p, bytes, hipHostMallocPortable);
}
}
namespace streampool {
constexpr int kPipeChunks = 8;
constexpr int kPipeEvents = 3 + 3 * kPipeChunks;
struct Bundle { int dev; hipStream_t stream; hipEvent_t ev[5]; hipStream_t pipe_r, pipe_i; hipEvent_t pipe_ev[kPipeEvents]; };
static void destroy(const Bundle &b) {
  for (hipEvent_t e : b.ev) if (e) (void)hipEventDestroy(e);
  for (hipEvent_t e : b.pipe_ev) if (e) (void)hipEventDestroy(e);
  for (hipStream_t st : {b.stream, b.pipe_r, b.pipe_i}) if (st) (void)hipStreamDestroy(st);
}
static std::mutex mu;
static std::vector<Bundle> idle;
static bool take(int dev, Bundle &out) {
  std::lock_guard<std::mutex> lk(mu);
  for (size_t i = 0; i < idle.size(); i++)
    if (idle[i].dev == dev) { out = idle[i]; idle.erase(idle.begin() + i); return true; }
  return false;
}
static void give(const Bundle &b) {
  {
    std::lock_guard<std::mutex> lk(mu);
    if (idle.size() < 64) { idle.push_back(b); return; }
  }
  destroy(b);
}
static void release_all() {
  std::lock_guard<std::mutex> lk(mu);
  for (Bundle &b : idle) destroy(b);
  idle.clear();
}
}

template <class T>
struct DevBuf {
  T *p = nullptr; size_t n = 0;
  size_t cap = 0;
  int dev = 0;
  int alloc(size_t count) {
    free();
    n = count;
    if (!count) return 0;
    const size_t bytes = (count * sizeof(T) + 255) & ~(size_t)255;
    if (hipGetDevice(&dev) != hipSuccess) dev = 0;
    if (void *q = devpool::take(dev, bytes, cap)) { p = (T *)q; return 0; }
    hipError_t e = hipMalloc((void **)&p, bytes);
    if (e != hipSuccess) {
      devpool::release_all();
      e = hipMalloc((void **)&p, bytes);
    }
    if (e != hipSuccess) { p = nullptr; g_last_error = std::string("hipMalloc: ") + hipGetErrorString(e); return MI_OSQP_ERR_ALLOC; }
    cap = bytes;
    return 0;
  }
  int zero(hipStream_t s) { if (n && hipMemsetAsync(p, 0, n * sizeof(T), s) != hipSuccess) return MI_OSQP_ERR_DEVICE; return 0; }
  int upload(const std::vector<T> &v) {
    int rc = alloc(v.size());
    if (rc) return rc;
    if (v.size() && hipMemcpy(p, v.data(), v.size() * sizeof(T), hipMemcpyHostToDevice) != hipSuccess) return MI_OSQP_ERR_DEVICE;
    return 0;
  }
  void free() { if (p && !devpool::give(dev, p, cap)) (void)hipFree(p); p = nullptr; n = 0; cap = 0; }
  ~DevBuf() { free(); }
};

struct SchedBufs {
  DevBuf<uint32_t> step, idxw, lvl_pos, tail_bar;
  DevBuf<uint64_t> idxw64;
  DevBuf<int32_t> src;
  int upload(const Schedule &s) {
    int rc;
    if ((rc = step.upload(s.step)) || (rc = idxw.upload(s.idxw)) || (rc = idxw64.upload(s.idxw64)) || (rc = src.upload(s.src)) ||
        (rc = lvl_pos.upload(s.lvl_pos)) || (rc = tail_bar.upload(s.tail_bar))) return rc;
    return 0;
  }
  SchedDev view(const Schedule &s) const {
    SchedDev d; d.step = step.p; d.idxw = idxw.p; d.idxw64 = idxw64.p; d.lvl_pos = lvl_pos.p; d.tail_bar = tail_bar.p;
    d.n_phases = s.n_phases; d.nw = s.nw; d.n_levels = s.n_levels;
    d.n_steps = s.n_steps; d.n_slots = s.n_slots;
    return d;
  }
};

struct mi_osqp_batch {
  Settings st;
  bool rho_interval_auto = false;
  Tuning tune;
  std::shared_ptr<const Analysis> anp;
  int B = 0, BT = 1, ntiles = 0, threads = 512, device = 0, n_cus = 256;
  size_t lds = 0;
  size_t lds_iter = 0;
  int rs_off = 0;
  size_t lds_factor = 0;
  int rf_off = 0, rf_steps = 0;
  std::vector<QPNumeric> qp;
  bool host_bounds_stale = false;
  hipStream_t stream = nullptr;
  SchedBufs fwd, bwd, chk;
  DevBuf<uint32_t> pinv, xloc;
  DevBuf<double> fwd_val, bwd_val, chk_val, dinv, x, z, y, q, l, u, rho_vec, rho_inv, Dsc, Dsc_inv, Esc, Esc_inv;
  DevBuf<double> dx, dy, out1, out2, dscal, x_out, y_out, xs_global;
  DevBuf<double> cert_out;
  bool global_xs = false;
  int mw_groups = 0, mw_threads = 0;
  DevBuf<uint32_t> mw_bar;
  DevBuf<unsigned char> rflag;
  DevBuf<double> mw_scratch;
  DevBuf<double> fwd_val0, bwd_val0, dinv0, rho_vec0, rho_inv0, dscal0;
  DevBuf<int> use_work;
  DevBuf<int> iscal, flag, npos;
  DevBuf<uint32_t> bf_blk, bf_lvl, bf_utask, bf_tri, bf_dtask, bf_ttask, bf_asm_dst, bf_asm_src, bf_ubig;
  DevBuf<int32_t> fwd_srcblk, bwd_srcblk;
  DevBuf<double> pa_val, Lblk, Dl, dinv_scratch;
  DevBuf<uint32_t> dt_task, dt_wave_task, dt_wave_step, dt_tail_bar;
  DevBuf<uint32_t> dt_lt_pos, dt_ltcol_col, dt_tile_tab, dt_wave_tiles, dt_diag_tile, dt_task_step;
  DevBuf<uint64_t> dt_asm_q64;
  DevBuf<int32_t> dt_src_tile;
  int dt_nh = 0; uint32_t dt_cs_doubles = 0; size_t dt_lds = 0, dt_lds_asm = 0;
  DevBuf<int32_t> dt_src;
  DevBuf<double> dt_val, dt_val0, dt_Sd;
  DevBuf<uint32_t> sp_ptr, sp_ent;
  DevBuf<uint32_t> sp_ell, sp_rowid;
  int sp_npass = 0;
  uint32_t sp_ell_off[4] = {0, 0, 0, 0}, sp_ell_k[4] = {0, 0, 0, 0};
  bool host_rho_stale = false;
  bool host_scaling_stale = false;
  DevBuf<int32_t> rz_prow, rz_pcol, rz_arow, rz_acol;
  bool clear_rho_updates = true;
  int *h_npos = nullptr;
  DevBuf<double> stage; DevBuf<int> ids, work;
  int *h_iscal = nullptr;
  double *h_dscal = nullptr;
  size_t h_iscal_cap = 0, h_dscal_cap = 0, h_npos_cap = 0, pin_cap = 0;
  double *pin = nullptr;
  size_t pin_n = 0;
  hipEvent_t ev0 = nullptr, ev1 = nullptr, evf0 = nullptr, evf1 = nullptr, evf2 = nullptr;
  hipStream_t pipe_r = nullptr, pipe_i = nullptr;
  hipEvent_t pipe_ev[streampool::kPipeEvents] = {};
  DevBuf<int> tile_list;
  int64_t pipelined_refactors = 0;
  double factor_ms_sum = 0.0, dense_ms_sum = 0.0;
  int64_t refactor_launches = 0, refactor_qps = 0, peak_qps = 0;
  double peak_factor_ms = 0.0, peak_tail_ms = 0.0;
  mi_osqp_stats stats{};
  int64_t last_total_iters = 0, last_launches = 0, last_refactors = 0;
  double last_device_s = 0.0, last_refactor_s = 0.0, kernel_ms_sum = 0.0;
  int64_t kernel_launches = 0, kernel_qp_iters = 0;
  bool solved_once = false;
  std::vector<char> failed;
  DevBuf<int> fail_list;
  DevBuf<double> rawP, rawq;
  DevBuf<double> pol_fwd, pol_bwd, pol_dinv, pol_dt, pol_sol;
  DevBuf<signed char> pol_act;
  DevBuf<int> pol_stat;
  std::vector<int> pol_status;
  int64_t pol_count = 0, pol_accepted = 0;
  double pol_seconds = 0.0;
  hipEvent_t evp0 = nullptr, evp1 = nullptr;
  DevBuf<int> adj_stat;
  struct Cont {
    bool on = false;
    int L = 25;
    unsigned launch_seq = 0;
    DevBuf<unsigned> stop;
    int64_t adv_seq = 0, polled_seq = 0;
    std::vector<char> running, clear_rho;
    std::vector<mi_osqp_info> info;
    int n_running = 0;
    int *h_is[2] = {nullptr, nullptr}; double *h_ds[2] = {nullptr, nullptr}; size_t h_is_cap[2] = {0, 0}, h_ds_cap[2] = {0, 0};
    hipEvent_t ev[2] = {nullptr, nullptr}; int64_t seq_of[2] = {0, 0};
    double *xh = nullptr, *yh = nullptr; size_t xh_cap = 0, yh_cap = 0;
    double *ch = nullptr; size_t ch_cap = 0;
    std::vector<int> cert_status;
    char *ring_h = nullptr; size_t ring_cap = 0, ring_h_cap = 0, ring_head = 0;
    int64_t ring_wraps = 0;
    DevBuf<char> ring_d;
    DevBuf<int> work;
    hipEvent_t ev_adv = nullptr;
    std::vector<int> epoch;
    DevBuf<double> rz_scratch;
    double *keepA = nullptr, *keepl = nullptr, *keepu = nullptr;
    DevBuf<unsigned> counter;
    unsigned *h_done = nullptr; size_t h_done_cap = 0;
    std::vector<char> polishable, polishing;
    std::vector<int> pol_status;
    int *h_pstat = nullptr; size_t h_pstat_cap = 0;
  } cont;
  ~mi_osqp_batch() {
    DevGuard guard(device);
    if (stream) (void)hipStreamSynchronize(stream);
    for (int k = 0; k < 2; k++) { hostpool::give(cont.h_is[k], cont.h_is_cap[k]); hostpool::give(cont.h_ds[k], cont.h_ds_cap[k]); if (cont.ev[k]) (void)hipEventDestroy(cont.ev[k]); }
    hostpool::give(cont.xh, cont.xh_cap); hostpool::give(cont.yh, cont.yh_cap); hostpool::give(cont.ch, cont.ch_cap); hostpool::give(cont.ring_h, cont.ring_h_cap);
    if (cont.ev_adv) (void)hipEventDestroy(cont.ev_adv);
    if (evp0) (void)hipEventDestroy(evp0);
    if (evp1) (void)hipEventDestroy(evp1);
    hostpool::give(cont.h_done, cont.h_done_cap); hostpool::give(cont.h_pstat, cont.h_pstat_cap);
    hostpool::give(h_iscal, h_iscal_cap); hostpool::give(h_dscal, h_dscal_cap); hostpool::give(pin, pin_cap); hostpool::give(h_npos, h_npos_cap);
    if (pipe_r) (void)hipStreamSynchronize(pipe_r);
    if (pipe_i) (void)hipStreamSynchronize(pipe_i);
    streampool::Bundle sb{device, stream, {ev0, ev1, evf0, evf1, evf2}, pipe_r, pipe_i, {}};
    for (int k = 0; k < streampool::kPipeEvents; k++) sb.pipe_ev[k] = pipe_ev[k];
    if (stream && ev0 && ev1 && evf0 && evf1 && evf2) streampool::give(sb);
    else streampool::destroy(sb);
  }
};

struct mi_osqp_solver { mi_osqp_batch *b = nullptr; };


static Settings to_settings(const mi_osqp_settings *s) {
  Settings t;
  if (!s) return t;
  t.rho = s->rho; t.sigma = s->sigma; t.scaling = s->scaling; t.adaptive_rho = s->adaptive_rho;
  t.adaptive_rho_interval = s->adaptive_rho_interval; t.adaptive_rho_tolerance = s->adaptive_rho_tolerance;
  t.max_iter = s->max_iter; t.eps_abs = s->eps_abs; t.eps_rel = s->eps_rel; t.eps_prim_inf = s->eps_prim_inf;
  t.eps_dual_inf = s->eps_dual_inf; t.alpha = s->alpha; t.scaled_termination = s->scaled_termination;
  t.check_termination = s->check_termination; t.warm_start = s->warm_start; t.verbose = s->verbose;
  t.polish = s->polish; t.polish_refine_iter = s->polish_refine_iter; t.delta = s->delta;
  return t;
}

static void dense_tail_deal_stats(const DenseTail &dt, mi_osqp_stats &s) {
  s.dense_tail_tasks = s.dense_tail_waves_used = s.dense_tail_wave_tasks_max = 0;
  if (!dt.k) return;
  s.dense_tail_tasks = (int64_t)dt.task.size() / 4;
  for (int w = 0; w < dt.nw; w++) {
    const int64_t c = (int64_t)dt.wave_task[w + 1] - (int64_t)dt.wave_task[w];
    s.dense_tail_waves_used += c > 0; s.dense_tail_wave_tasks_max = std::max(s.dense_tail_wave_tasks_max, c);
  }
}

static size_t lds_bytes(int N, int BT, int threads) {
  int nw = threads / 64;
  return ((size_t)N * BT + (size_t)nw * 14 * BT + 14 * BT) * sizeof(double);
}

static KernelArgs make_args(mi_osqp_batch *h) {
  KernelArgs a{};
  a.n = (*h->anp).n; a.m = (*h->anp).m; a.N = (*h->anp).N; a.B = h->B;
  a.fwd = h->fwd.view((*h->anp).fwd); a.bwd = h->bwd.view((*h->anp).bwd); a.chk = h->chk.view((*h->anp).chk);
  a.pinv = h->pinv.p; a.xloc = h->xloc.p;
  a.fwd_val = h->fwd_val.p; a.bwd_val = h->bwd_val.p; a.chk_val = h->chk_val.p; a.dinv = h->dinv.p;
  a.fwd_val0 = h->fwd_val0.p; a.bwd_val0 = h->bwd_val0.p; a.dt_val0 = h->dt_val0.p;
  a.use_work = (h->fwd_val0.p && h->bwd_val0.p && (!(*h->anp).dt.k || h->dt_val0.p)) ? h->use_work.p : nullptr;
  a.x = h->x.p; a.z = h->z.p; a.y = h->y.p; a.q = h->q.p; a.l = h->l.p; a.u = h->u.p;
  a.rho_vec = h->rho_vec.p; a.rho_inv = h->rho_inv.p; a.Dsc = h->Dsc.p; a.Dsc_inv = h->Dsc_inv.p;
  a.Esc = h->Esc.p; a.Esc_inv = h->Esc_inv.p; a.dx = h->dx.p; a.dy = h->dy.p; a.out1 = h->out1.p; a.out2 = h->out2.p;
  a.dscal = h->dscal.p; a.iscal = h->iscal.p;
  a.x_out = h->x_out.p; a.y_out = h->y_out.p;
  a.cert_out = h->cert_out.p; a.cert_stride = (int)std::max<int64_t>(std::max<int64_t>(a.n, a.m), 1);
  a.xs_global = h->global_xs ? h->xs_global.p : nullptr; a.xs_len = (*h->anp).xs_total; a.wide = (*h->anp).wide ? 1 : 0;
  a.rs_off = h->rs_off; a.rf_off = h->rf_off;
  a.mw_groups = h->mw_groups; a.mw_bar = h->mw_bar.p; a.mw_scratch = h->mw_scratch.p;
  a.df = (*h->anp).df ? 1 : 0; a.df_shadow = (unsigned)(*h->anp).Next; a.rflag = h->rflag.p;
  {
    const DenseTail &dt = (*h->anp).dt;
    a.dt.s = dt.s; a.dt.k = dt.k; a.dt.n_phases = dt.n_phases; a.dt.n_steps = dt.n_steps;
    a.dt.task = h->dt_task.p; a.dt.wave_task = h->dt_wave_task.p; a.dt.wave_step = h->dt_wave_step.p; a.dt.tail_bar = h->dt_tail_bar.p;
    a.dt_val = h->dt_val.p;
  }
  const Settings &s = h->st;
  a.sigma = s.sigma; a.alpha = s.alpha; a.eps_abs = s.eps_abs; a.eps_rel = s.eps_rel;
  a.eps_prim_inf = s.eps_prim_inf; a.eps_dual_inf = s.eps_dual_inf; a.rho_tolerance = s.adaptive_rho_tolerance;
  a.check_termination = (int)s.check_termination; a.rho_interval = (int)s.adaptive_rho_interval;
  a.max_iter = (int)s.max_iter; a.scaled_termination = (int)s.scaled_termination; a.scaling = s.scaling ? 1 : 0;
  a.adaptive_rho = (int)s.adaptive_rho; a.iter_begin = 0; a.iter_end = 0; a.info_at_end = 1;
  return a;
}

static FactorArgs make_factor_args(mi_osqp_batch *h, int force_all) {
  FactorArgs a{};
  const Analysis &an = (*h->anp);
  a.n = an.n; a.m = an.m; a.N = an.N; a.B = h->B; a.nnzP = an.Pp[an.n]; a.nnzK = an.nnzK();
  a.pa_len = an.Pp[an.n] + an.Ap[an.n]; a.n_levels = an.bf.n_levels; a.force_all = force_all;
  a.storage = an.bf.storage; a.fwd = h->fwd.view(an.fwd); a.bwd = h->bwd.view(an.bwd);
  a.blk = h->bf_blk.p; a.lvl = h->bf_lvl.p; a.utask = h->bf_utask.p; a.tri4 = h->bf_tri.p; a.dtask = h->bf_dtask.p; a.ubig = h->bf_ubig.p;
  a.ttask = h->bf_ttask.p; a.asm_dst = h->bf_asm_dst.p; a.asm_src = h->bf_asm_src.p;
  a.fwd_srcblk = h->fwd_srcblk.p; a.bwd_srcblk = h->bwd_srcblk.p;
  a.pa_val = h->pa_val.p; a.l = h->l.p; a.u = h->u.p; a.dscal = h->dscal.p;
  a.rho_vec = h->rho_vec.p; a.rho_inv = h->rho_inv.p; a.Lblk = h->Lblk.p; a.Dl = h->Dl.p; a.dinv_scratch = h->dinv_scratch.p;
  a.fwd_val = h->fwd_val.p; a.bwd_val = h->bwd_val.p; a.dinv = h->dinv.p; a.iscal = h->iscal.p; a.npos = h->npos.p; a.use_work = h->use_work.p;
  a.sigma = h->st.sigma; a.home_bt = h->BT; a.dt_k = an.dt.k;
  a.mw_groups = 0; a.mw_bar = h->mw_bar.p;
// ... 283 lines not shown
    if (dev < 0 && hipGetDevice(&dev) != hipSuccess) dev = 0;
    if (hipDeviceGetAttribute(&cus, hipDeviceAttributeMultiprocessorCount, dev) != hipSuccess || cus <= 0) cus = 256;
    (void)hipGetLastError();
    const int64_t tiles = (B + BT - 1) / BT;
    if (tiles <= cus || lds_bytes((int)(n + m), BT, 1024) > 80 * 1024) h->threads = 1024;
  }
  h->global_xs = wide || lds_bytes((int)(n + m), BT, h->threads) > lds_cap || tu.global_xs;
  int max_extra = -1;
  if (!h->global_xs) {
    const size_t cap_rows = (lds_cap - lds_bytes(0, BT, h->threads)) / (sizeof(double) * BT);
    max_extra = (int)(cap_rows - (size_t)(n + m));
  }
  h->mw_groups = 0; h->mw_threads = 0;
  if (h->global_xs && BT == 1 && B == 1 && h->threads <= 512) {
    const int64_t Nrows = n + m;
    h->mw_groups = tu.groups >= 0 ? tu.groups : (Nrows >= 250000 ? 256 : Nrows >= 60000 ? 128 : Nrows >= 30000 ? 64 : 32);
    h->mw_threads = tu.group_threads ? tu.group_threads : 128;
    if (h->mw_groups * (h->mw_threads / 64) > 2048) h->mw_groups = 2048 / (h->mw_threads / 64);
    int dev = (int)device, cus = 0;
    if ((dev >= 0 || hipGetDevice(&dev) == hipSuccess) && hipDeviceGetAttribute(&cus, hipDeviceAttributeMultiprocessorCount, dev) == hipSuccess && cus > 0) {
      DevGuard guard(dev);
      if (tu.assume_cus > 0) cus = std::min(cus, tu.assume_cus);
      const int cap = max_coresident_groups(h->mw_threads, lds_bytes(0, 1, h->threads), cus);
      if (cap > 0 && h->mw_groups > cap) h->mw_groups = cap;
      if (h->mw_groups == 1) h->mw_groups = 0;
    }
    (void)hipGetLastError();
  }
  BT_out = BT; max_extra_out = max_extra;
}

static int shape_and_analysis(mi_osqp_batch *h, int64_t B, int64_t n, int64_t m, const int64_t *Pp, const int64_t *Pi, const int64_t *Ap,
                              const int64_t *Ai, int64_t device, int &BT, int &max_extra, std::shared_ptr<const Analysis> &out) {
  derive_shape(h, B, n, m, device, BT, max_extra);
  int rc = cached_analysis(n, m, Pp, Pi, Ap, Ai, h->tune, h->threads / 64, BT, max_extra, h->global_xs ? 0 : 512, h->mw_groups * (h->mw_threads / 64), (int)((B + BT - 1) / BT), out);
  if (rc) return rc;
  const size_t lds_cap = 160 * 1024 - 1024;
  if (out->dt.k > 0 && (BT != 1 || h->threads != 1024) && !h->global_xs && !h->tune.tile && !h->tune.threads &&
      lds_bytes((int)(n + m), 1, 1024) + (size_t)2 * 512 * sizeof(double) <= lds_cap) {
    const int BT2 = 1, thr2 = 1024;
    const size_t cap_rows = (lds_cap - lds_bytes(0, BT2, thr2)) / (sizeof(double) * BT2);
    const int max_extra2 = (int)(cap_rows - (size_t)(n + m));
    std::shared_ptr<const Analysis> an2;
    rc = cached_analysis(n, m, Pp, Pi, Ap, Ai, h->tune, thr2 / 64, BT2, max_extra2, 512, 0, (int)B, an2);
    if (!rc && an2->dt.k > 0) { BT = BT2; h->threads = thr2; max_extra = max_extra2; out = an2; }
  }
  return MI_OSQP_OK;
}

static int batch_setup_impl(mi_osqp_batch *h, int64_t B, int64_t n, int64_t m, const int64_t *Pp, const int64_t *Pi,
                            const double *Pv, const double *q, const int64_t *Ap, const int64_t *Ai,
                            const double *Av, const double *l, const double *u, int64_t device) {
  double t0 = now_s();
  if (B <= 0 || !Pp || !Ap || (m > 0 && (!l || !u)) || (Pp[n] > 0 && !Pv) || (Ap[n] > 0 && !Av)) return MI_OSQP_ERR_INVALID_DATA;
  if (validate_settings(h->st)) return MI_OSQP_ERR_INVALID_SETTINGS;
  if (h->st.adaptive_rho && !h->st.adaptive_rho_interval) {
    h->rho_interval_auto = true;
    h->st.adaptive_rho_interval = h->st.check_termination ? 4 * h->st.check_termination : 100;
  }
  for (int64_t k = 0; k < B * m; k++) if (l[k] > u[k]) return MI_OSQP_ERR_INVALID_DATA;
  int BT = 1, max_extra = -1;
  const size_t lds_cap = 160 * 1024 - 1024;
  h->tune = tuning_from_env();
  const double ta0 = now_s();
  int rc = shape_and_analysis(h, B, n, m, Pp, Pi, Ap, Ai, device, BT, max_extra, h->anp);
  const double t_analysis = now_s() - ta0;
  if (rc) return rc;
  const Analysis &an = (*h->anp);
  h->B = (int)B;
  h->failed.assign((size_t)B, 0);
  int ndev = 0;
  if (hipGetDeviceCount(&ndev) != hipSuccess || ndev <= 0) { g_last_error = "no HIP device visible"; return MI_OSQP_ERR_DEVICE; }
  if (device >= ndev) { g_last_error = "no such HIP device"; return MI_OSQP_ERR_DEVICE; }
  if (device >= 0) h->device = (int)device; else HIPCHK(hipGetDevice(&h->device));
  DevGuard guard(h->device);
  hipDeviceProp_t prop;
  HIPCHK(hipGetDeviceProperties(&prop, h->device));
  h->n_cus = prop.multiProcessorCount > 0 ? prop.multiProcessorCount : 256;
  if (strncmp(prop.gcnArchName, "gfx950", 6) != 0) { g_last_error = std::string("device is not gfx950: ") + prop.gcnArchName; return MI_OSQP_ERR_DEVICE; }
  {
    streampool::Bundle sb;
    if (streampool::take(h->device, sb)) {
      h->stream = sb.stream; h->ev0 = sb.ev[0]; h->ev1 = sb.ev[1]; h->evf0 = sb.ev[2]; h->evf1 = sb.ev[3]; h->evf2 = sb.ev[4];
      h->pipe_r = sb.pipe_r; h->pipe_i = sb.pipe_i;
      for (int k = 0; k < streampool::kPipeEvents; k++) h->pipe_ev[k] = sb.pipe_ev[k];
    }
    else {
      HIPCHK(hipStreamCreateWithFlags(&h->stream, hipStreamNonBlocking));
      HIPCHK(hipEventCreate(&h->ev0)); HIPCHK(hipEventCreate(&h->ev1));
      HIPCHK(hipEventCreate(&h->evf0)); HIPCHK(hipEventCreate(&h->evf1)); HIPCHK(hipEventCreate(&h->evf2));
    }
  }
  h->BT = BT; h->ntiles = (int)((B + BT - 1) / BT);
  h->lds = h->global_xs ? lds_bytes(0, BT, h->threads) : lds_bytes(an.Next + 2 * an.dt.k, BT, h->threads);
  if (h->lds > lds_cap) { g_last_error = "internal: LDS budget exceeded"; return MI_OSQP_ERR_ALLOC; }
  h->lds_iter = h->lds; h->rs_off = 0;
  {
    const size_t state = sizeof(double) * (size_t)BT * (2 * (size_t)n + 6 * (size_t)m + (size_t)an.N);
    if (!h->tune.stream_state && !h->global_xs && h->mw_groups <= 0 && h->threads == 1024 && h->lds + state <= lds_cap) {
      h->rs_off = (int)(h->lds / sizeof(double)); h->lds_iter = h->lds + state;
    }
  }
  h->lds_factor = 0; h->rf_off = 0; h->rf_steps = 0;
  if (h->rs_off && BT == 1 && an.dt.k > 0 && !h->tune.stream_factor) {
    const size_t part = (size_t)(h->threads / 64) * rf_lds_steps() * 64 * sizeof(double);
    if (h->lds_iter + part <= lds_cap) {
      h->rf_off = (int)(h->lds_iter / sizeof(double)); h->lds_factor = part; h->rf_steps = rf_head_steps();
    }
  }
  size_t T = (size_t)h->ntiles * BT;
  if ((rc = h->fwd.upload(an.fwd)) || (rc = h->bwd.upload(an.bwd)) || (rc = h->chk.upload(an.chk))) return rc;
  { std::vector<uint32_t> pv(an.pinv.begin(), an.pinv.end()); if ((rc = h->pinv.upload(pv))) return rc; }
  { std::vector<uint32_t> xv(an.xloc.begin(), an.xloc.end()); if ((rc = h->xloc.upload(xv))) return rc; }
  {
    std::vector<int32_t> pr(an.Pi.begin(), an.Pi.begin() + an.Pp[n]), pc(an.Pp[n]), ar(an.Ai.begin(), an.Ai.begin() + an.Ap[n]), ac(an.Ap[n]);
    for (int j = 0; j < n; j++) { for (int k = an.Pp[j]; k < an.Pp[j + 1]; k++) pc[k] = j; for (int k = an.Ap[j]; k < an.Ap[j + 1]; k++) ac[k] = j; }
    if ((rc = h->rz_prow.upload(pr)) || (rc = h->rz_pcol.upload(pc)) || (rc = h->rz_arow.upload(ar)) || (rc = h->rz_acol.upload(ac))) return rc;
  }
  if ((rc = h->use_work.alloc(T)) || (rc = h->use_work.zero(h->stream))) return rc;
#define ALLOC(buf, len) if ((rc = h->buf.alloc((size_t)(len) * T)) || (rc = h->buf.zero(h->stream))) return rc
  ALLOC(fwd_val, (size_t)an.fwd.phys_steps() * 64); ALLOC(bwd_val, (size_t)an.bwd.phys_steps() * 64); ALLOC(chk_val, (size_t)an.chk.phys_steps() * 64); ALLOC(dinv, an.N);
  ALLOC(x, n); ALLOC(z, m); ALLOC(y, m); ALLOC(q, n); ALLOC(l, m); ALLOC(u, m); ALLOC(rho_vec, m); ALLOC(rho_inv, m);
  ALLOC(Dsc, n); ALLOC(Dsc_inv, n); ALLOC(Esc, m); ALLOC(Esc_inv, m); ALLOC(dx, n); ALLOC(dy, m);
  ALLOC(out1, 2 * n + m); ALLOC(out2, 2 * n + m); ALLOC(dscal, DS_COUNT);
  if (h->global_xs) { ALLOC(xs_global, an.xs_total); }
  if ((rc = h->mw_bar.alloc(4 * (size_t)std::max(h->n_cus, 1))) || (rc = h->mw_bar.zero(h->stream))) return rc;
  if (an.df && ((rc = h->rflag.upload(an.rflag)) || (rc = h->mw_scratch.alloc((size_t)8 * 256 * 16)) || (rc = h->mw_scratch.zero(h->stream)))) return rc;
  if (an.dt.k) {
    const DenseTail &dt = an.dt;
    ALLOC(dt_val, (size_t)dt.n_steps * 64);
    if ((rc = h->dt_task.upload(dt.task)) || (rc = h->dt_wave_task.upload(dt.wave_task)) || (rc = h->dt_wave_step.upload(dt.wave_step)) ||
        (rc = h->dt_tail_bar.upload(dt.tail_bar)) || (rc = h->dt_src.upload(dt.src)) ||
        (rc = h->dt_lt_pos.upload(dt.lt_pos)) || (rc = h->dt_ltcol_col.upload(dt.ltcol_col)) || (rc = h->dt_tile_tab.upload(dt.tile_tab)) ||
        (rc = h->dt_wave_tiles.upload(dt.wave_tiles)) || (rc = h->dt_asm_q64.upload(dt.asm_q64)) ||
        (rc = h->dt_src_tile.upload(dt.src_tile)) || (rc = h->dt_diag_tile.upload(dt.diag_tile)) || (rc = h->dt_task_step.upload(dt.task_step)) ||
        (rc = h->dt_Sd.alloc((size_t)dt.k * dt.k * (T + 4)))) return rc;
    const int nrt = dt.k / 16 - 4;
    h->dt_nh = nrt <= 14 ? std::max(nrt, 1) : (nrt + 1) / 2;
    h->dt_cs_doubles = (uint32_t)std::max(h->dt_nh * 1024, 64 * 65 + 63) / 64 * 64;
    h->dt_lds = std::max<size_t>((size_t)h->dt_cs_doubles + 4096, 2 * 64 * 65) * sizeof(double);
    h->dt_lds_asm = (dt.asm_lds_bytes() + 255) & ~(size_t)255;
    if (h->dt_lds > lds_cap || h->dt_lds_asm > lds_cap) { g_last_error = "internal: LDS budget of tail_kernel exceeded"; return MI_OSQP_ERR_ALLOC; }
  }
#undef ALLOC
  if ((rc = h->iscal.alloc((size_t)IS_COUNT * T)) || (rc = h->flag.alloc(4))) return rc;
  {
    const BlockFactor &bf = an.bf;
    if ((rc = h->bf_blk.upload(bf.blk)) || (rc = h->bf_lvl.upload(bf.lvl)) || (rc = h->bf_ubig.upload(bf.ubig)) || (rc = h->bf_utask.upload(bf.utask4)) ||
        (rc = h->bf_tri.upload(bf.tri4)) || (rc = h->bf_dtask.upload(bf.dtask4)) || (rc = h->bf_ttask.upload(bf.ttask4)) ||
        (rc = h->bf_asm_dst.upload(bf.asm_dst)) || (rc = h->bf_asm_src.upload(bf.asm_src)) ||
        (rc = h->fwd_srcblk.upload(an.fwd_srcblk)) || (rc = h->bwd_srcblk.upload(an.bwd_srcblk))) return rc;
    if ((rc = h->pa_val.alloc((size_t)(an.Pp[n] + an.Ap[n]) * T)) || (rc = h->pa_val.zero(h->stream)) ||
        (rc = h->Lblk.alloc((size_t)bf.storage * (T + 4))) || (rc = h->Dl.alloc((size_t)an.N * (T + 4))) || (rc = h->Dl.zero(h->stream)) ||
        (rc = h->dinv_scratch.alloc((size_t)an.N * (T + 4))) || (rc = h->npos.alloc(T))) return rc;
    HIPCHK(hostpool::alloc((void **)&h->h_npos, T * sizeof(int), &h->h_npos_cap));
  }
  if (!h->global_xs && an.Pp[n] + an.Ap[n] < 65536 && n + m < 65536 &&
      spmv_fused_lds_bytes((int)n, (int)m, an.Pp[n] + an.Ap[n], BT) <= 150 * 1024) {
    const int nnzP = an.Pp[n];
    std::vector<std::vector<uint32_t>> rows((size_t)2 * n + m);
    for (int c = 0; c < (int)n; c++)
      for (int k = an.Pp[c]; k < an.Pp[c + 1]; k++) {
        const int r = an.Pi[k];
        rows[r].push_back((uint32_t)k | ((uint32_t)c << 16));
        if (r != c) rows[c].push_back((uint32_t)k | ((uint32_t)r << 16));
      }
    for (int c = 0; c < (int)n; c++)
// ... 275 lines not shown
  if ((int)bad.size() == h->B) { g_last_error = "the KKT factor lost its inertia"; return MI_OSQP_ERR_NONCONVEX; }
  return 0;
}

static int ensure_polish_buffers(mi_osqp_batch *h) {
  if (h->pol_stat.p) return MI_OSQP_OK;
  const Analysis &an = (*h->anp);
  const size_t T = (size_t)h->ntiles * h->BT;
  int rc;
  if ((rc = h->pol_fwd.alloc(h->fwd_val.n)) || (rc = h->pol_fwd.zero(h->stream)) || (rc = h->pol_bwd.alloc(h->bwd_val.n)) ||
      (rc = h->pol_bwd.zero(h->stream)) || (rc = h->pol_dinv.alloc(h->dinv.n)) || (rc = h->pol_dinv.zero(h->stream)) ||
      (rc = h->pol_sol.alloc(T * an.N)) || (rc = h->pol_act.alloc(std::max<size_t>(1, T * an.m))) || (rc = h->pol_act.zero(h->stream)) ||
      (rc = h->pol_stat.alloc(T)) || (rc = h->pol_stat.zero(h->stream))) return rc;
  if (an.dt.k && ((rc = h->pol_dt.alloc(h->dt_val.n)) || (rc = h->pol_dt.zero(h->stream)))) return rc;
  if (!h->evp0) HIPCHK(hipEventCreate(&h->evp0));
  if (!h->evp1) HIPCHK(hipEventCreate(&h->evp1));
  return MI_OSQP_OK;
}

static constexpr int kPolishInner = 4;

static int polish_impl(mi_osqp_batch *h, const KernelArgs &a) {
  const int BT = h->BT, ntl = h->ntiles;
  int rc;
  h->pol_count = h->pol_accepted = 0; h->pol_seconds = 0.0;
  h->pol_status.assign((size_t)h->B, 0);
  if ((rc = ensure_polish_buffers(h))) return rc;
  std::vector<int> work = koptimal_slots(h);
  PolishArgs pa{h->pol_stat.p, h->pol_act.p, h->pol_sol.p, (int)h->st.polish_refine_iter, kPolishInner, h->st.delta};
  HIPCHK(hipEventRecord(h->evp0, h->stream));
  HIPCHK(launch_polish_active(a, pa, BT, h->stream));
  const int n_pol = (int)work.size();
  if (n_pol) {
    if ((rc = device_refactor_slots(h, std::move(work), nullptr, &pa))) return rc;
    if ((rc = run_spinning(h, h->stream, [&]() -> int {
          HIPCHK(launch_polish(polish_stream_args(h, a), pa, BT, ntl, h->mw_groups > 0 ? h->mw_threads : h->threads, h->lds, h->n_cus, h->stream));
          HIPCHK(hipEventRecord(h->evp1, h->stream));
          return MI_OSQP_OK;
        }))) return rc;
  } else {
    HIPCHK(hipEventRecord(h->evp1, h->stream));
  }
  HIPCHK(hipMemcpyAsync(h->pol_status.data(), h->pol_stat.p, (size_t)h->B * sizeof(int), hipMemcpyDeviceToHost, h->stream));
  HIPCHK(hipStreamSynchronize(h->stream));
  float ms = 0.f;
  HIPCHK(hipEventElapsedTime(&ms, h->evp0, h->evp1));
  h->pol_seconds = ms * 1e-3;
  h->pol_count = n_pol;
  for (int v : h->pol_status) h->pol_accepted += v == 1;
  return MI_OSQP_OK;
}

static int adjoint_impl(mi_osqp_batch *h, const AdjointArgs &ga, int32_t *d_status, hipStream_t user_stream) {
  hipStream_t keep = h->stream;
  struct Restore { mi_osqp_batch *h; hipStream_t s; ~Restore() { h->stream = s; } } restore{h, keep};
  if (user_stream) h->stream = user_stream;
  const Analysis &an = (*h->anp);
  const int BT = h->BT, ntl = h->ntiles;
  int rc;
  if ((rc = ensure_polish_buffers(h))) return rc;
  if (!h->adj_stat.p && ((rc = h->adj_stat.alloc((size_t)ntl * BT)))) return rc;
  if ((rc = h->adj_stat.zero(h->stream))) return rc;
  std::vector<int> work;
  if (h->solved_once) {
    HIPCHK(hipMemcpyAsync(h->h_iscal, h->iscal.p, (size_t)ntl * IS_COUNT * BT * sizeof(int), hipMemcpyDeviceToHost, h->stream));
    HIPCHK(hipStreamSynchronize(h->stream));
    work = koptimal_slots(h);
  }
  if (!work.empty()) {
    const KernelArgs a = make_args(h);
    PolishArgs pa{h->adj_stat.p, h->pol_act.p, h->pol_sol.p, (int)h->st.polish_refine_iter};
    HIPCHK(launch_polish_active(a, pa, BT, h->stream));
    if ((rc = device_refactor_slots(h, std::move(work), nullptr, &pa))) return rc;
    if ((rc = run_spinning(h, h->stream, [&]() -> int {
          HIPCHK(launch_adjoint(polish_stream_args(h, a), pa, ga, BT, ntl, h->mw_groups > 0 ? h->mw_threads : h->threads, h->lds, h->n_cus, h->stream));
          return MI_OSQP_OK;
        }))) return rc;
  }
  HIPCHK(launch_adjoint_finish(h->adj_stat.p, ga, d_status, h->B, an.n, an.m, h->stream));
  HIPCHK(hipStreamSynchronize(h->stream));
  return MI_OSQP_OK;
}

static bool pipeline_applies(const mi_osqp_batch *h, int n_ref) {
  const int longer_than = h->tune.pipeline_min > 0 ? h->tune.pipeline_min : h->n_cus;
  return h->tune.refactor_pipeline && n_ref > longer_than && h->mw_groups <= 0 && !h->global_xs && !(*h->anp).wide && !(*h->anp).df;
}

static int pipelined_refactor_iterate(mi_osqp_batch *h, const KernelArgs &a, const std::vector<int> &work, const std::vector<int> &active, std::vector<int> *bad) {
  using streampool::kPipeChunks; using streampool::kPipeEvents;
  const double t_begin = now_s();
  const int BT = h->BT, nq = (int)work.size();
  int rc;
  if (!h->pipe_r) HIPCHK(hipStreamCreateWithFlags(&h->pipe_r, hipStreamNonBlocking));
  if (!h->pipe_i) HIPCHK(hipStreamCreateWithFlags(&h->pipe_i, hipStreamNonBlocking));
  for (int k = 0; k < kPipeEvents; k++) if (!h->pipe_ev[k]) HIPCHK(hipEventCreate(&h->pipe_ev[k]));
  hipEvent_t ev_fork = h->pipe_ev[0], ev_i0 = h->pipe_ev[1], ev_i1 = h->pipe_ev[2];
  auto ev_chunk = [&](int c, int k) { return h->pipe_ev[3 + 3 * (c - 1) + k]; };
  int n_even = h->tune.pipeline_chunks > 0 ? h->tune.pipeline_chunks : (nq + h->n_cus - 1) / h->n_cus;
  int chunk_qps = (nq + n_even - 1) / n_even;
  if (h->tune.pipeline_chunks <= 0 && h->tune.pipeline_chunk_qps > 0) chunk_qps = h->tune.pipeline_chunk_qps;
  const RefactorChunks ch = refactor_chunks(work, active, BT, chunk_qps, kPipeChunks);
  const int kbt = nq <= h->n_cus ? 1 : BT;
  std::vector<int> wl, wl_begin(1, 0);
  for (int c = 1; c < ch.n_chunks; c++) {
    wl.insert(wl.end(), work.begin() + ch.work_begin[c], work.begin() + ch.work_begin[c + 1]);
    wl.resize((wl.size() + kbt - 1) / kbt * kbt, -1);
    wl_begin.push_back((int)wl.size());
  }
  if (h->work.n < wl.size() && (rc = h->work.alloc((size_t)h->ntiles * BT + 4 + (size_t)BT * kPipeChunks))) return rc;
  if (h->tile_list.n < ch.tiles.size() && (rc = h->tile_list.alloc((size_t)h->ntiles))) return rc;
  HIPCHK(hipMemcpyAsync(h->work.p, wl.data(), wl.size() * sizeof(int), hipMemcpyHostToDevice, h->stream));
  HIPCHK(hipMemcpyAsync(h->tile_list.p, ch.tiles.data(), ch.tiles.size() * sizeof(int), hipMemcpyHostToDevice, h->stream));
  const double t_fork = now_s();
  HIPCHK(hipEventRecord(ev_fork, h->stream));
  HIPCHK(hipStreamWaitEvent(h->pipe_r, ev_fork, 0));
  HIPCHK(hipStreamWaitEvent(h->pipe_i, ev_fork, 0));
  FactorArgs fa = make_factor_args(h, 0);
  const bool tail = (*h->anp).dt.k != 0;
  for (int c = 1; c < ch.n_chunks; c++) {
    const int *wc = h->work.p + wl_begin[c - 1];
    const int slots = wl_begin[c] - wl_begin[c - 1];
    fa.work = wc;
    HIPCHK(hipEventRecord(ev_chunk(c, 0), h->pipe_r));
    HIPCHK(launch_factor(fa, kbt, slots / kbt, h->tune.factor_threads, h->pipe_r));
    HIPCHK(hipEventRecord(ev_chunk(c, 1), h->pipe_r));
    if (tail) HIPCHK(launch_tail(make_tail_args(h, kbt, wc), slots, h->dt_lds_asm, h->dt_lds, h->pipe_r));
    HIPCHK(hipEventRecord(ev_chunk(c, 2), h->pipe_r));
  }
  KernelArgs ai = a;
  HIPCHK(hipEventRecord(ev_i0, h->pipe_i));
  for (int c = 0; c < ch.n_chunks; c++) {
    const int nt = ch.tile_begin[c + 1] - ch.tile_begin[c];
    if (c) HIPCHK(hipStreamWaitEvent(h->pipe_i, ev_chunk(c, 2), 0));
    if (!nt) continue;
    ai.tiles = h->tile_list.p + ch.tile_begin[c];
    HIPCHK(launch_iterate(ai, BT, nt, h->threads, h->lds_iter + h->lds_factor, h->pipe_i));
  }
  HIPCHK(hipEventRecord(ev_i1, h->pipe_i));
  HIPCHK(hipStreamWaitEvent(h->stream, ev_i1, 0));
  HIPCHK(hipMemcpyAsync(h->h_iscal, h->iscal.p, (size_t)h->ntiles * IS_COUNT * BT * sizeof(int), hipMemcpyDeviceToHost, h->stream));
  HIPCHK(hipStreamSynchronize(h->stream));
  const double t_end = now_s();
  float f_ms = 0.f, d_ms = 0.f, r_ms = 0.f, i_ms = 0.f;
  for (int c = 1; c < ch.n_chunks; c++) {
    float f = 0.f, d = 0.f;
    HIPCHK(hipEventElapsedTime(&f, ev_chunk(c, 0), ev_chunk(c, 1))); HIPCHK(hipEventElapsedTime(&d, ev_chunk(c, 1), ev_chunk(c, 2)));
    f_ms += f; d_ms += tail ? d : 0.f;
  }
  HIPCHK(hipEventElapsedTime(&r_ms, ev_fork, ev_chunk(ch.n_chunks - 1, 2)));
  HIPCHK(hipEventElapsedTime(&i_ms, ev_i0, ev_i1));
  const double wall = t_end - t_begin, ref_s = std::min(wall, (t_fork - t_begin) + 1e-3 * r_ms);
  h->last_refactor_s += ref_s; h->last_device_s += wall - ref_s;
  h->kernel_ms_sum += i_ms; h->kernel_launches++; h->last_launches++;
  h->factor_ms_sum += f_ms; h->dense_ms_sum += d_ms; h->refactor_launches++; h->refactor_qps += nq;
  if (nq >= h->peak_qps) { h->peak_qps = nq; h->peak_factor_ms = f_ms; h->peak_tail_ms = d_ms; }
  h->pipelined_refactors++;
  for (int s : work)
    if (h->h_iscal[(size_t)(s / BT) * IS_COUNT * BT + IS_NEED_REFACTOR * BT + s % BT] < 0) bad->push_back(s);
  return 0;
}

static int solve_impl(mi_osqp_batch *h, double *d_x_out, hipStream_t user_stream) {
  hipStream_t keep = h->stream;
  struct Restore { mi_osqp_batch *h; hipStream_t s; ~Restore() { h->stream = s; } } restore{h, keep};
  if (user_stream) h->stream = user_stream;
  int rc;
  if ((rc = reset_solve_state(h, !h->st.warm_start))) return rc;
  KernelArgs a = make_args(h);
  if (d_x_out) a.x_out = d_x_out;
  h->last_total_iters = h->last_launches = h->last_refactors = 0;
  h->last_device_s = h->last_refactor_s = 0.0;
  const int BT = h->BT, ntl = h->ntiles, nslots = ntl * BT;
  const Settings &S = h->st;
  {
    std::vector<int> bad;
    for (int q = 0; q < h->B; q++) if (h->failed[q]) bad.push_back(q);
    if ((rc = fail_slots(h, a, bad, 0))) return rc;
  }
  auto segment_end = [&](int iter) {
    int seg_end = (int)S.max_iter;
    if (S.check_termination > 0) seg_end = std::min<int64_t>(seg_end, (iter / S.check_termination + 1) * S.check_termination);
    if (S.adaptive_rho && S.adaptive_rho_interval > 0)
      seg_end = std::min<int64_t>(seg_end, (iter / S.adaptive_rho_interval + 1) * S.adaptive_rho_interval);
    return seg_end;
  };
  auto loop = [&]() -> int {
    int iter = 0;
    bool iterated = false;
    while (true) {
      const int seg_end = segment_end(iter);
      a.iter_begin = iter; a.iter_end = seg_end; a.info_at_end = 1;
      {
        std::unique_lock<std::mutex> spin_lock(spin_mutex(h->device), std::defer_lock);
        if (h->mw_groups > 0) spin_lock.lock();
        if (!iterated) {
          HIPCHK(hipEventRecord(h->ev0, h->stream));
          if (h->mw_groups > 0) HIPCHK(hipMemsetAsync(h->mw_bar.p, 0, 4 * sizeof(uint32_t), h->stream));
          HIPCHK(launch_iterate(a, BT, ntl, h->mw_groups > 0 ? h->mw_threads : h->threads, h->lds_iter + h->lds_factor, h->stream));
          HIPCHK(hipEventRecord(h->ev1, h->stream));
        }
        {
          int chk_threads = h->mw_groups > 0 ? h->mw_threads : h->threads;
          if (h->mw_groups <= 0 && h->threads == 1024 && ntl > 2 * h->n_cus) chk_threads = 512;
          HIPCHK(launch_check(a, BT, ntl, chk_threads, h->lds, h->stream));
        }
        HIPCHK(hipMemcpyAsync(h->h_iscal, h->iscal.p, (size_t)ntl * IS_COUNT * BT * sizeof(int), hipMemcpyDeviceToHost, h->stream));
        HIPCHK(hipStreamSynchronize(h->stream));
      }
      if ((rc = mw_barrier_ok(h))) {
        const std::string why = g_last_error;
        (void)restore_snapshot(h);
        g_last_error = why + " (the handle is back in the state of its last setup / update, cold-started)";
        return rc;
      }
      if (!iterated) {
        float ms = 0.f;
        HIPCHK(hipEventElapsedTime(&ms, h->ev0, h->ev1));
        h->last_device_s += ms * 1e-3; h->kernel_ms_sum += ms; h->kernel_launches++; h->last_launches++;
      }
      iterated = false;
      iter = seg_end;
      std::vector<int> active, work;
      for (int s = 0; s < h->B; s++) {
        const int *t = h->h_iscal + (size_t)(s / BT) * IS_COUNT * BT;
        if (!t[IS_DONE * BT + s % BT]) active.push_back(s);
        if (t[IS_NEED_REFACTOR * BT + s % BT]) work.push_back(s);
      }
      const int n_ref = (int)work.size();
      if (active.empty() && !n_ref) break;
      if (n_ref) {
        double tr = now_s();
        std::vector<int> bad;
        int rc2;
        if (!active.empty() && pipeline_applies(h, n_ref)) {
          KernelArgs nx = a;
          nx.iter_begin = iter; nx.iter_end = segment_end(iter); nx.info_at_end = 1;
          if ((rc2 = pipelined_refactor_iterate(h, nx, work, active, &bad))) return rc2;
          iterated = true;
          tr = now_s();
        } else if ((rc2 = device_refactor_slots(h, std::move(work), &bad))) return rc2;
        if ((rc2 = fail_slots(h, a, bad, iter))) return rc2;
        h->host_rho_stale = true;
        h->last_refactors += n_ref;
        h->last_refactor_s += now_s() - tr;
        if (!bad.empty()) {
          std::vector<char> isbad(nslots, 0);
          for (int q : bad) isbad[q] = 1;
          active.erase(std::remove_if(active.begin(), active.end(), [&](int q) { return isbad[q] != 0; }), active.end());
        }
      }
      if (active.empty()) break;
    }
    return MI_OSQP_OK;
  };
  rc = loop();
  if (rc) {
    if (h->pipe_r) (void)hipStreamSynchronize(h->pipe_r);
    if (h->pipe_i) (void)hipStreamSynchronize(h->pipe_i);
    (void)hipStreamSynchronize(h->stream);
    return rc;
  }
  HIPCHK(hipMemcpyAsync(h->h_iscal, h->iscal.p, (size_t)nslots * IS_COUNT * sizeof(int), hipMemcpyDeviceToHost, h->stream));
  HIPCHK(hipStreamSynchronize(h->stream));
  for (int qi = 0; qi < h->B; qi++)
    h->last_total_iters += h->h_iscal[(size_t)(qi / BT) * IS_COUNT * BT + IS_ITER * BT + qi % BT];
  h->solved_once = true;
  if (h->st.polish && (rc = polish_impl(h, a))) return rc;
  if (!h->st.polish) { h->pol_status.clear(); h->pol_count = h->pol_accepted = 0; }
  return MI_OSQP_OK;
}


extern "C" {

void mi_osqp_default_settings(mi_osqp_settings *s) {
  if (!s) return;
  s->rho = 0.1; s->sigma = 1e-6; s->scaling = 10; s->adaptive_rho = 1; s->adaptive_rho_interval = 0;
  s->adaptive_rho_tolerance = 5.0; s->max_iter = 4000; s->eps_abs = 1e-3; s->eps_rel = 1e-3;
  s->eps_prim_inf = 1e-4; s->eps_dual_inf = 1e-4; s->alpha = 1.6; s->scaled_termination = 0;
  s->check_termination = 25; s->warm_start = 1; s->verbose = 0;
  s->polish = 0; s->polish_refine_iter = 3; s->delta = 1e-6;
}

const char *mi_osqp_exit_code_name(int64_t c) {
  static const char *names[] = {"kOptimal", "kPrimalInfeasible", "kDualInfeasible", "kOptimalInaccurate",
                                "kPrimalInfeasibleInaccurate", "kDualInfeasibleInaccurate", "kMaxIterations",
                                "kInterrupted", "kTimeLimitReached", "kNonConvex", "kUnknown"};
  return (c >= 0 && c <= 10) ? names[c] : "kUnknown";
}
const char *mi_osqp_error_name(int64_t e) {
  static const char *names[] = {"ok", "invalid data", "invalid settings", "sparsity pattern changed",
                                "non-convex problem / KKT inertia", "device error", "null argument", "allocation / size"};
  return (e >= 0 && e <= 7) ? names[e] : "unknown";
}
const char *mi_osqp_version(void) { return "mi-osqp 0.2 (gfx950)"; }
const char *mi_osqp_last_error(void) { return g_last_error.c_str(); }

static int64_t exit_code_of(int status) {
  switch (status) {
    case 1: return MI_OSQP_EXIT_OPTIMAL;
    case 2: return MI_OSQP_EXIT_OPTIMAL_INACCURATE;
    case -3: return MI_OSQP_EXIT_PRIMAL_INFEASIBLE;
    case 3: return MI_OSQP_EXIT_PRIMAL_INFEASIBLE_INACCURATE;
    case -4: return MI_OSQP_EXIT_DUAL_INFEASIBLE;
    case 4: return MI_OSQP_EXIT_DUAL_INFEASIBLE_INACCURATE;
    case -2: return MI_OSQP_EXIT_MAX_ITERATIONS;
    case -5: return MI_OSQP_EXIT_INTERRUPTED;
    case -6: return MI_OSQP_EXIT_TIME_LIMIT_REACHED;
    case -7: return MI_OSQP_EXIT_NON_CONVEX;
    default: return MI_OSQP_EXIT_UNKNOWN;
  }
}

int mi_osqp_batch_setup(mi_osqp_batch **out, int64_t B, int64_t n, int64_t m, const int64_t *Pp, const int64_t *Pi,
                        const double *Pv, const double *q, const int64_t *Ap, const int64_t *Ai, const double *Av,
                        const double *l, const double *u, const mi_osqp_settings *settings, int64_t device) {
  CallTimer timer_("batch_setup");
  if (!out) return MI_OSQP_ERR_NULL;
  *out = nullptr;
  if (n <= 0 || m < 0) return MI_OSQP_ERR_INVALID_DATA;
  mi_osqp_batch *h = new (std::nothrow) mi_osqp_batch();
  if (!h) return MI_OSQP_ERR_ALLOC;
  h->st = to_settings(settings);
  int rc = batch_setup_impl(h, B, n, m, Pp, Pi, Pv, q, Ap, Ai, Av, l, u, device);
  if (rc) { delete h; return rc; }
  *out = h;
  return MI_OSQP_OK;
}

int mi_osqp_prefetch_analysis(int64_t B, int64_t n, int64_t m, const int64_t *Pp, const int64_t *Pi, const int64_t *Ap, const int64_t *Ai, int64_t device) {
  CallTimer timer_("prefetch_analysis");
  if (B <= 0 || n <= 0 || m < 0 || !Pp || !Ap || (Pp[n] > 0 && !Pi) || (Ap[n] > 0 && !Ai)) return MI_OSQP_ERR_INVALID_DATA;
  mi_osqp_batch tmp;
  tmp.tune = tuning_from_env();
  int BT = 1, max_extra = -1;
  std::shared_ptr<const Analysis> an;
  return shape_and_analysis(&tmp, B, n, m, Pp, Pi, Ap, Ai, device, BT, max_extra, an);
}

void mi_osqp_batch_free(mi_osqp_batch *h) { delete h; }
void mi_osqp_release_device_cache(void) { devpool::release_all(); hostpool::release_all(); streampool::release_all(); }
// ... 103 lines not shown
}

int mi_osqp_batch_get_polish_active(mi_osqp_batch *h, int8_t *act) {
  if (!h || !act) return MI_OSQP_ERR_NULL;
  const size_t cnt = (size_t)h->B * (*h->anp).m;
  if (!h->pol_act.p) { memset(act, 0, cnt); return MI_OSQP_OK; }
  DevGuard guard(h->device);
  if (h->cont.on) HIPCHK(hipStreamSynchronize(h->stream));
  if (cnt) HIPCHK(hipMemcpy(act, h->pol_act.p, cnt, hipMemcpyDeviceToHost));
  return MI_OSQP_OK;
}

static AdjointArgs adjoint_args(mi_osqp_batch *h, const double *d_dx, const double *d_dy, double *d_dq, double *d_dP, double *d_dA,
                                double *d_dl, double *d_du) {
  const Analysis &an = (*h->anp);
  AdjointArgs ga{};
  ga.gx = d_dx; ga.gy = d_dy; ga.dq = d_dq; ga.dP = d_dP; ga.dA = d_dA; ga.dl = d_dl; ga.du = d_du;
  ga.prow = h->rz_prow.p; ga.pcol = h->rz_pcol.p; ga.arow = h->rz_arow.p; ga.acol = h->rz_acol.p;
  ga.nnzP = (int)an.Pp[an.n]; ga.nnzA = (int)an.Ap[an.n];
  return ga;
}
int mi_osqp_batch_adjoint_device(mi_osqp_batch *h, const double *d_dx, const double *d_dy, double *d_dq, double *d_dP, double *d_dA,
                                 double *d_dl, double *d_du, int32_t *d_status, void *stream) {
  CallTimer timer_("batch_adjoint_device");
  if (!h) return MI_OSQP_ERR_NULL;
  if (!d_dx) { g_last_error = "adjoint: dx is null (dL/dx is required; only dy may be null)"; return MI_OSQP_ERR_NULL; }
  for (const double *o : {(const double *)d_dq, (const double *)d_dP, (const double *)d_dA, (const double *)d_dl, (const double *)d_du})
    if (o && (o == d_dx || o == d_dy)) { g_last_error = "adjoint: an output aliases dx or dy"; return MI_OSQP_ERR_INVALID_DATA; }
  DevGuard guard(h->device);
  { const int rc_ = cont_leave(h); if (rc_) return rc_; }
  return adjoint_impl(h, adjoint_args(h, d_dx, d_dy, d_dq, d_dP, d_dA, d_dl, d_du), d_status, (hipStream_t)stream);
}
int mi_osqp_batch_adjoint(mi_osqp_batch *h, const double *dx, const double *dy, double *dq, double *dP, double *dA, double *dl,
                          double *du, int32_t *status) {
  CallTimer timer_("batch_adjoint");
  if (!h) return MI_OSQP_ERR_NULL;
  if (!dx) { g_last_error = "adjoint: dx is null (dL/dx is required; only dy may be null)"; return MI_OSQP_ERR_NULL; }
  DevGuard guard(h->device);
  { const int rc_ = cont_leave(h); if (rc_) return rc_; }
  const Analysis &an = (*h->anp);
  const size_t B = (size_t)h->B, n = (size_t)an.n, m = (size_t)an.m, nnzP = (size_t)an.Pp[an.n], nnzA = (size_t)an.Ap[an.n];
  const size_t len[7] = {B * n, dy ? B * m : 0, dq ? B * n : 0, dP ? B * nnzP : 0, dA ? B * nnzA : 0, dl ? B * m : 0, du ? B * m : 0};
  size_t off[8] = {0};
  for (int k = 0; k < 7; k++) off[k + 1] = off[k] + len[k];
  DevBuf<double> buf;
  DevBuf<int> stat;
  int rc;
  if ((rc = buf.alloc(off[7])) || (rc = stat.alloc(B))) return rc;
  auto at = [&](int k) -> double * { return len[k] ? buf.p + off[k] : nullptr; };
  HIPCHK(hipMemcpy(at(0), dx, len[0] * sizeof(double), hipMemcpyHostToDevice));
  if (len[1]) HIPCHK(hipMemcpy(at(1), dy, len[1] * sizeof(double), hipMemcpyHostToDevice));
  if ((rc = adjoint_impl(h, adjoint_args(h, at(0), at(1), at(2), at(3), at(4), at(5), at(6)), stat.p, nullptr))) return rc;
  double *out[7] = {nullptr, nullptr, dq, dP, dA, dl, du};
  for (int k = 2; k < 7; k++) if (len[k]) HIPCHK(hipMemcpy(out[k], at(k), len[k] * sizeof(double), hipMemcpyDeviceToHost));
  if (status) HIPCHK(hipMemcpy(status, stat.p, B * sizeof(int32_t), hipMemcpyDeviceToHost));
  return MI_OSQP_OK;
}

int mi_osqp_batch_get_scaling(mi_osqp_batch *h, double *D, double *E, double *c) {
  if (!h || !D || !E || !c) return MI_OSQP_ERR_NULL;
  DevGuard guard(h->device);
  { const int rc_ = cont_leave(h); if (rc_) return rc_; }
  const int n = (*h->anp).n, m = (*h->anp).m, B = h->B, BT = h->BT;
  int rc;
  if ((rc = ensure_stage(h, (size_t)B * std::max({n, m, 1}) + 1, 0))) return rc;
  auto down = [&](const double *src, int len, double *dst) -> int {
    if (!len) return 0;
    HIPCHK(launch_deinterleave(src, h->stage.p, B, len, BT, h->stream));
    HIPCHK(hipMemcpyAsync(dst, h->stage.p, (size_t)B * len * sizeof(double), hipMemcpyDeviceToHost, h->stream));
    HIPCHK(hipStreamSynchronize(h->stream));
    return 0;
  };
  if ((rc = down(h->Dsc.p, n, D)) || (rc = down(h->Esc.p, m, E))) return rc;
  const size_t dcnt = (size_t)h->ntiles * DS_COUNT * BT;
  HIPCHK(hipMemcpy(h->h_dscal, h->dscal.p, dcnt * sizeof(double), hipMemcpyDeviceToHost));
  for (int q = 0; q < B; q++) c[q] = h->h_dscal[(size_t)(q / BT) * DS_COUNT * BT + DS_C * BT + q % BT];
  return MI_OSQP_OK;
}

int mi_osqp_batch_get_stats(mi_osqp_batch *h, mi_osqp_stats *st) {
  if (!h || !st) return MI_OSQP_ERR_NULL;
  *st = h->stats;
  st->pipelined_refactors = h->pipelined_refactors;
  return MI_OSQP_OK;
}

int mi_osqp_batch_get_ordering(mi_osqp_batch *h, int64_t *kkt_perm) {
  if (!h || !kkt_perm) return MI_OSQP_ERR_NULL;
  const Analysis &an = (*h->anp);
  for (int k = 0; k < an.N; k++) kkt_perm[k] = an.perm[(size_t)k];
  return MI_OSQP_OK;
}

int mi_osqp_batch_last_solve_stats(mi_osqp_batch *h, int64_t *total_iters, int64_t *kernel_launches, double *device_seconds,
                                   double *refactor_seconds, int64_t *refactor_count, double *compact_seconds) {
  if (!h) return MI_OSQP_ERR_NULL;
  if (compact_seconds) *compact_seconds = 0.0;
  if (total_iters) *total_iters = h->last_total_iters;
  if (kernel_launches) *kernel_launches = h->last_launches;
  if (device_seconds) *device_seconds = h->last_device_s;
  if (refactor_seconds) *refactor_seconds = h->last_refactor_s;
  if (refactor_count) *refactor_count = h->last_refactors;
  return MI_OSQP_OK;
}

int mi_osqp_batch_kernel_time(mi_osqp_batch *h, double *avg_ms, int64_t *launches) {
  if (!h) return MI_OSQP_ERR_NULL;
  if (avg_ms) *avg_ms = h->kernel_launches ? h->kernel_ms_sum / (double)h->kernel_launches : 0.0;
  if (launches) *launches = h->kernel_launches;
  h->kernel_ms_sum = 0.0; h->kernel_launches = 0;
  return MI_OSQP_OK;
}

int mi_osqp_batch_refactor_time(mi_osqp_batch *h, double *factor_ms, double *dense_ms, int64_t *launches, int64_t *qps) {
  if (!h) return MI_OSQP_ERR_NULL;
  if (factor_ms) *factor_ms = h->factor_ms_sum;
  if (dense_ms) *dense_ms = h->dense_ms_sum;
  if (launches) *launches = h->refactor_launches;
  if (qps) *qps = h->refactor_qps;
  h->factor_ms_sum = h->dense_ms_sum = 0.0; h->refactor_launches = h->refactor_qps = 0;
  h->peak_qps = 0; h->peak_factor_ms = h->peak_tail_ms = 0.0;
  return MI_OSQP_OK;
}

int mi_osqp_batch_refactor_peak(mi_osqp_batch *h, int64_t *qps, double *factor_ms, double *tail_ms) {
  if (!h) return MI_OSQP_ERR_NULL;
  if (qps) *qps = h->peak_qps;
  if (factor_ms) *factor_ms = h->peak_factor_ms;
  if (tail_ms) *tail_ms = h->peak_tail_ms;
  return MI_OSQP_OK;
}

int mi_osqp_batch_reset(mi_osqp_batch *h) {
  CallTimer timer_("batch_reset");
  if (!h) return MI_OSQP_ERR_NULL;
  DevGuard guard(h->device);
  { const int rc_ = cont_leave(h); if (rc_) return rc_; }
  return restore_snapshot(h);
}
}
static int restore_snapshot(mi_osqp_batch *h) {
  h->clear_rho_updates = true;
  auto cp = [&](DevBuf<double> &dst, DevBuf<double> &src) -> int {
    if (src.n) HIPCHK(hipMemcpyAsync(dst.p, src.p, src.n * sizeof(double), hipMemcpyDeviceToDevice, h->stream));
    return 0;
  };
  int rc;
  const size_t nflags = (size_t)h->ntiles * h->BT;
  HIPCHK(hipMemsetD32Async((hipDeviceptr_t)h->use_work.p, 0, nflags, h->stream));
  if ((rc = cp(h->dinv, h->dinv0)) || (rc = cp(h->rho_vec, h->rho_vec0)) || (rc = cp(h->rho_inv, h->rho_inv0)) || (rc = cp(h->dscal, h->dscal0))) return rc;
  if ((rc = reset_solve_state(h, true))) return rc;
  HIPCHK(hipStreamSynchronize(h->stream));
  h->host_rho_stale = true;
  return MI_OSQP_OK;
}
extern "C" {

int mi_osqp_batch_warm_start_x(mi_osqp_batch *h, const double *x) {
  CallTimer timer_("batch_warm_start_x");
  if (!h || !x) return MI_OSQP_ERR_NULL;
  DevGuard guard(h->device);
  { const int rc_ = cont_leave(h); if (rc_) return rc_; }
  h->st.warm_start = 1;
  size_t cnt = (size_t)h->B * (*h->anp).n;
  int rc;
  if ((rc = ensure_stage(h, cnt, 0)) || (rc = ensure_pin(h, cnt))) return rc;
// ... 1515 lines not shown
}

int mi_gomp_relinearise_some(mi_gomp_scene *sc, int64_t n_ids, const int64_t *ids, const double *x, int32_t *ok_out) {
  CallTimer timer_("gomp_relinearise_some");
  if (!sc || (n_ids > 0 && (!ids || !x || !ok_out))) return MI_OSQP_ERR_NULL;
  if (!n_ids) return MI_OSQP_OK;
  mi_osqp_batch *h = sc->h;
  DevGuard guard(h->device);
  int rc;
  if ((rc = cont_enter(h)) || (rc = cont_check_ids(h, n_ids, ids, true))) return rc;
  if ((rc = gomp_launch(sc, n_ids, ids, x, 2, ok_out))) return rc;
  std::vector<int64_t> bad;
  for (int64_t j = 0; j < n_ids; j++) if (!ok_out[j]) bad.push_back(ids[j]);
  if (bad.empty()) return MI_OSQP_OK;
  return cont_new_data(h, (int64_t)bad.size(), bad.data(), nullptr, nullptr, nullptr, false, sc->A.p, sc->l.p, sc->u.p);
}

}

extern "C" {


int mi_osqp_setup(mi_osqp_solver **out, int64_t n, int64_t m, const int64_t *Pp, const int64_t *Pi, const double *Pv,
                  const double *q, const int64_t *Ap, const int64_t *Ai, const double *Av, const double *l,
                  const double *u, const mi_osqp_settings *settings) {
  if (!out) return MI_OSQP_ERR_NULL;
  *out = nullptr;
  mi_osqp_batch *b = nullptr;
  int rc = mi_osqp_batch_setup(&b, 1, n, m, Pp, Pi, Pv, q, Ap, Ai, Av, l, u, settings, -1);
  if (rc) return rc;
  mi_osqp_solver *s = new (std::nothrow) mi_osqp_solver();
  if (!s) { delete b; return MI_OSQP_ERR_ALLOC; }
  s->b = b; *out = s;
  return MI_OSQP_OK;
}
void mi_osqp_free(mi_osqp_solver *h) { if (h) { delete h->b; delete h; } }
int mi_osqp_update_A_bounds(mi_osqp_solver *h, const int64_t *Ap, const int64_t *Ai, const double *Av, const double *l, const double *u) {
  return h ? mi_osqp_batch_update_A_bounds(h->b, Ap, Ai, Av, l, u) : MI_OSQP_ERR_NULL;
}
int mi_osqp_update_A(mi_osqp_solver *h, const int64_t *Ap, const int64_t *Ai, const double *Av) {
  return h ? mi_osqp_batch_update_A(h->b, Ap, Ai, Av) : MI_OSQP_ERR_NULL;
}
int mi_osqp_update_bounds(mi_osqp_solver *h, const double *l, const double *u) {
  return h ? mi_osqp_batch_update_bounds(h->b, l, u) : MI_OSQP_ERR_NULL;
}
int mi_osqp_warm_start_x(mi_osqp_solver *h, const double *x) { return h ? mi_osqp_batch_warm_start_x(h->b, x) : MI_OSQP_ERR_NULL; }
int mi_osqp_update_q(mi_osqp_solver *h, const double *q) { return h ? mi_osqp_batch_update_q(h->b, q) : MI_OSQP_ERR_NULL; }
int mi_osqp_update_P(mi_osqp_solver *h, const int64_t *Pp, const int64_t *Pi, const double *Pv) {
  return h ? mi_osqp_batch_update_P(h->b, Pp, Pi, Pv) : MI_OSQP_ERR_NULL;
}
int mi_osqp_update_P_A(mi_osqp_solver *h, const int64_t *Pp, const int64_t *Pi, const double *Pv, const int64_t *Ap, const int64_t *Ai,
                       const double *Av) {
  return h ? mi_osqp_batch_update_P_A(h->b, Pp, Pi, Pv, Ap, Ai, Av) : MI_OSQP_ERR_NULL;
}
int mi_osqp_warm_start_y(mi_osqp_solver *h, const double *y) { return h ? mi_osqp_batch_warm_start_y(h->b, y) : MI_OSQP_ERR_NULL; }
int mi_osqp_solve(mi_osqp_solver *h, mi_osqp_info *info) {
  if (!h) return MI_OSQP_ERR_NULL;
  int rc = mi_osqp_batch_solve(h->b);
  if (rc) return rc;
  if (info) return mi_osqp_batch_get_info(h->b, info);
  return MI_OSQP_OK;
}
int mi_osqp_get_primal(mi_osqp_solver *h, double *x) { return h ? mi_osqp_batch_get_primal(h->b, x) : MI_OSQP_ERR_NULL; }
int mi_osqp_get_dual(mi_osqp_solver *h, double *y) { return h ? mi_osqp_batch_get_dual(h->b, y) : MI_OSQP_ERR_NULL; }
int mi_osqp_get_prim_inf_cert(mi_osqp_solver *h, double *dy_out) { return h ? mi_osqp_batch_get_prim_inf_cert(h->b, dy_out) : MI_OSQP_ERR_NULL; }
int mi_osqp_get_dual_inf_cert(mi_osqp_solver *h, double *dx_out) { return h ? mi_osqp_batch_get_dual_inf_cert(h->b, dx_out) : MI_OSQP_ERR_NULL; }
int mi_osqp_adjoint(mi_osqp_solver *h, const double *dx, const double *dy, double *dq, double *dP, double *dA, double *dl, double *du,
                    int32_t *status) {
  return h ? mi_osqp_batch_adjoint(h->b, dx, dy, dq, dP, dA, dl, du, status) : MI_OSQP_ERR_NULL;
}
int mi_osqp_debug_refactor_chunks(int64_t n_flagged, const int64_t *flagged, int64_t n_active, const int64_t *active, int64_t tile,
                                  int64_t chunk_qps, int64_t max_chunks, int64_t *n_chunks, int64_t *work_begin, int64_t *tiles,
                                  int64_t *tile_begin) {
  if (!n_chunks || !work_begin || !tiles || !tile_begin || (n_flagged > 0 && !flagged) || (n_active > 0 && !active)) return MI_OSQP_ERR_NULL;
  if (n_flagged < 0 || n_active < 0 || tile < 1 || chunk_qps < 1 || max_chunks < 1) return MI_OSQP_ERR_INVALID_DATA;
  const std::vector<int> f(flagged, flagged + n_flagged), a(active, active + n_active);
  const RefactorChunks ch = refactor_chunks(f, a, (int)tile, (int)chunk_qps, (int)max_chunks);
  *n_chunks = ch.n_chunks;
  std::copy(ch.work_begin.begin(), ch.work_begin.end(), work_begin);
  std::copy(ch.tiles.begin(), ch.tiles.end(), tiles);
  std::copy(ch.tile_begin.begin(), ch.tile_begin.end(), tile_begin);
  return MI_OSQP_OK;
}
int mi_osqp_get_stats(mi_osqp_solver *h, mi_osqp_stats *st) { return h ? mi_osqp_batch_get_stats(h->b, st) : MI_OSQP_ERR_NULL; }
int mi_osqp_get_settings(mi_osqp_solver *h, mi_osqp_settings *out) { return h ? mi_osqp_batch_get_settings(h->b, out) : MI_OSQP_ERR_NULL; }
int mi_osqp_update_settings(mi_osqp_solver *h, const mi_osqp_settings *s) { return h ? mi_osqp_batch_update_settings(h->b, s) : MI_OSQP_ERR_NULL; }


}

struct ShardWorker {
  std::thread th;
  std::mutex mu;
  std::condition_variable cv;
  std::function<int()> job;
  bool has_job = false, busy = false, quit = false;
  int rc = 0;
  std::string err;
  void start() {
    th = std::thread([this] {
      std::unique_lock<std::mutex> lk(mu);
      for (;;) {
        cv.wait(lk, [this] { return has_job || quit; });
        if (quit) return;
        std::function<int()> f = std::move(job);
        has_job = false;
        lk.unlock();
        const int r = f();
        const std::string e = r ? g_last_error : std::string();
        lk.lock();
        rc = r; err = e; busy = false;
        cv.notify_all();
      }
    });
  }
  void post(std::function<int()> f) {
    std::unique_lock<std::mutex> lk(mu);
    cv.wait(lk, [this] { return !busy; });
    job = std::move(f); has_job = true; busy = true; rc = 0; err.clear();
    cv.notify_all();
  }
  int wait(std::string &e) {
    std::unique_lock<std::mutex> lk(mu);
    cv.wait(lk, [this] { return !busy; });
    e = err;
    return rc;
  }
  ~ShardWorker() {
    { std::lock_guard<std::mutex> lk(mu); quit = true; }
    cv.notify_all();
    if (th.joinable()) th.join();
  }
};

struct mi_osqp_multi {
  int64_t B = 0, n = 0, m = 0;
  std::vector<int64_t> dev, begin;
  std::vector<mi_osqp_batch *> shard;
  std::vector<std::unique_ptr<ShardWorker>> worker;
  bool async_pending = false;
  ~mi_osqp_multi() { worker.clear(); for (mi_osqp_batch *b : shard) delete b; }
  size_t count() const { return shard.size(); }
};

static int multi_join(mi_osqp_multi *h) {
  int rc = MI_OSQP_OK;
  for (size_t k = 0; k < h->worker.size(); k++) {
    std::string e;
    const int r = h->worker[k]->wait(e);
    if (r && !rc) { rc = r; g_last_error = "shard " + std::to_string(k) + ": " + e; }
  }
  h->async_pending = false;
  return rc;
}
template <class F>
static int multi_fan_out(mi_osqp_multi *h, F &&fn) {
  const size_t ns = h->count();
  if (h->async_pending) { const int rc0 = multi_join(h); if (rc0) return rc0; }
  if (ns == 1) { const int rc = fn(0); if (rc) g_last_error = "shard 0: " + g_last_error; return rc; }
  if (h->worker.size() != ns) {
    h->worker.clear();
    for (size_t k = 0; k < ns; k++) { h->worker.emplace_back(new ShardWorker()); h->worker.back()->start(); }
  }
  for (size_t k = 0; k < ns; k++) h->worker[k]->post([&fn, k]() -> int { return fn(k); });
  return multi_join(h);
}
// ... 228 lines not shown
```

Before: 38790.

## Run pipelined refactor chunks across multiple stream lanes with dependency waits

Refactor-plus-iterate chunks are spread over up to three streams (lanes), by default two. Each chunk has its own scratch offset (wg_base) so that factorizations on different lanes can run concurrently, and cross-lane event waits are added only where a chunk's tiles depend on an earlier chunk. The blocking host sync after the pipelined region is also deferred: failure handling moves into a device kernel (fail_flagged) and the timing bookkeeping is finalized at the next segment. The cost is more scratch memory, more stream and event complexity, and possible contention between concurrent kernels.

```diff
diff --git a/include/mi_osqp.h b/include/mi_osqp.h
--- a/include/mi_osqp.h
+++ b/include/mi_osqp.h
@@ -81,6 +81,7 @@
   int64_t pipelined_refactors;
   int64_t resident_factor_steps, lds_bytes_factor;
   int64_t dense_tail_tasks, dense_tail_waves_used, dense_tail_wave_tasks_max;
+  int64_t refactor_lanes;
 } mi_osqp_stats;
 
 typedef struct mi_osqp_solver mi_osqp_solver;
@@ -287,6 +288,11 @@
                                   int64_t chunk_qps, int64_t max_chunks, int64_t *n_chunks, int64_t *work_begin, int64_t *tiles,
                                   int64_t *tile_begin);
 
+int mi_osqp_debug_refactor_lanes(int64_t n_flagged, const int64_t *flagged, int64_t n_active, const int64_t *active, int64_t tile,
+                                 int64_t chunk_qps, int64_t max_chunks, int64_t kbt, int64_t lanes, int64_t chunk0_first,
+                                 int64_t scratch_slots, int64_t *n_lanes, int64_t *lane_of, int64_t *order, int64_t *order_begin,
+                                 int64_t *scratch_begin, int64_t *n_waits, int64_t *wait_chunk, int64_t *wait_for);
+
 int mi_osqp_debug_trace_kkt_solve(mi_osqp_batch *h, int32_t which, const double *d_rhs, double *d_sol,
                                   uint32_t *out, int64_t out_capacity_words, int64_t *dims);
 
diff --git a/osqp-solver_amd/__init__.py b/osqp-solver_amd/__init__.py
--- a/osqp-solver_amd/__init__.py
+++ b/osqp-solver_amd/__init__.py
@@ -48,7 +48,8 @@
                [("nnz_L_before_tail", C.c_int64), ("solve_groups", C.c_int64), ("solve_group_threads", C.c_int64),
                 ("resident_state", C.c_int64), ("lds_bytes_iterate", C.c_int64), ("pipelined_refactors", C.c_int64),
                 ("resident_factor_steps", C.c_int64), ("lds_bytes_factor", C.c_int64),
-                ("dense_tail_tasks", C.c_int64), ("dense_tail_waves_used", C.c_int64), ("dense_tail_wave_tasks_max", C.c_int64)]
+                ("dense_tail_tasks", C.c_int64), ("dense_tail_waves_used", C.c_int64), ("dense_tail_wave_tasks_max", C.c_int64),
+                ("refactor_lanes", C.c_int64)]
 
     def as_dict(self):
         return {k: getattr(self, k) for k, _ in self._fields_}
@@ -187,6 +188,7 @@
         L.mi_osqp_debug_host_kkt_solve.argtypes = [C.c_int64, C.c_int64, ip, ip, dp, ip, ip, dp, dp, dp,
                                                    C.POINTER(Settings), C.c_int64, dp, dp, dp, C.POINTER(Stats)]
         L.mi_osqp_debug_refactor_chunks.argtypes = [C.c_int64, ip, C.c_int64, ip, C.c_int64, C.c_int64, C.c_int64, ip, ip, ip, ip]
+        L.mi_osqp_debug_refactor_lanes.argtypes = [C.c_int64, ip, C.c_int64, ip] + [C.c_int64] * 7 + [ip] * 8
         L.mi_osqp_prefetch_analysis.argtypes = [C.c_int64, C.c_int64, C.c_int64, ip, ip, ip, ip, C.c_int64]
         L.mi_osqp_debug_host_block_factor.argtypes = [C.c_int64, C.c_int64, ip, ip, dp, ip, ip, dp, dp, dp,
                                                       C.POINTER(Settings), dp, dp, ip]
@@ -832,6 +834,24 @@
     return ([f[wb[c]:wb[c + 1]].tolist() for c in range(k)], [tl[tb[c]:tb[c + 1]].tolist() for c in range(k)])
 
 
+def debug_refactor_lanes(flagged, active, tile, chunk_qps, lanes, kbt=None, chunk0_first=False, scratch_slots=None, max_chunks=8):
+    f, a = _i64(flagged), _i64(active)
+    kbt = tile if kbt is None else kbt
+    work, _ = debug_refactor_chunks(flagged, active, tile, chunk_qps, max_chunks)
+    k = len(work)
+    nl, nw = C.c_int64(), C.c_int64()
+    lane_of = np.zeros(max_chunks + 2, dtype=np.int64); order = np.zeros(max_chunks + 2, dtype=np.int64)
+    ob = np.zeros(4, dtype=np.int64); sb = np.zeros(max_chunks + 2, dtype=np.int64)
+    wc = np.zeros((max_chunks + 1) ** 2, dtype=np.int64); wf = np.zeros((max_chunks + 1) ** 2, dtype=np.int64)
+    _chk(lib().mi_osqp_debug_refactor_lanes(len(f), _ip(f), len(a), _ip(a), tile, chunk_qps, max_chunks, kbt, lanes, int(bool(chunk0_first)),
+                                            2 ** 31 - 1 if scratch_slots is None else scratch_slots, C.byref(nl), _ip(lane_of), _ip(order),
+                                            _ip(ob), _ip(sb), C.byref(nw), _ip(wc), _ip(wf)), "debug_refactor_lanes")
+    L = int(nl.value)
+    return dict(n_lanes=L, lane_of=lane_of[:k].tolist(), order=[order[ob[l]:ob[l + 1]].tolist() for l in range(L)],
+                scratch=[(int(sb[c]), (len(work[c]) + kbt - 1) // kbt * kbt) for c in range(k)],
+                waits=list(zip(wc[:nw.value].tolist(), wf[:nw.value].tolist())))
+
+
 def debug_host_block_factor(P, A, l, u, **settings):
     L = lib()
     P, A = _csc(P), _csc(A)
diff --git a/osqp-solver_amd/csrc/device_types.h b/osqp-solver_amd/csrc/device_types.h
--- a/osqp-solver_amd/csrc/device_types.h
+++ b/osqp-solver_amd/csrc/device_types.h
@@ -75,6 +75,7 @@
   int *iscal, *npos;
   int home_bt;
   const int *work;
+  int wg_base;
   double sigma;
   int dt_k;
   int mw_groups;
@@ -93,6 +94,7 @@
   int nh;
   uint32_t cs_doubles;
   const int *work;
+  int wg_base;
   const uint32_t *lt_pos, *ltcol_col, *tile_tab, *wave_tiles, *diag_tile;
   const uint64_t *asm_q64;
   const int32_t *src_tile;
@@ -211,6 +213,7 @@
 hipError_t launch_gomp_relinearise(const GompArgs &g, hipStream_t st);
 hipError_t launch_gather_status(const int *iscal, int32_t *status, int32_t *iters, int B, int BT, hipStream_t st);
 hipError_t launch_fail_slots(const KernelArgs &a, const int *slots, int nfail, int BT, int iter, hipStream_t st);
+hipError_t launch_fail_flagged(const KernelArgs &a, const int *slots, int nslots, int BT, int iter, hipStream_t st);
 hipError_t launch_bounds(const double *gl, const double *gu, double *l, double *u, const double *Esc,
                          const double *rho_vec, const double *dscal, int *changed, int B, int m, int BT,
                          int scaling, hipStream_t st);
diff --git a/osqp-solver_amd/csrc/host_core.cpp b/osqp-solver_amd/csrc/host_core.cpp
--- a/osqp-solver_amd/csrc/host_core.cpp
+++ b/osqp-solver_amd/csrc/host_core.cpp
@@ -947,6 +947,8 @@
   if (const char *e = getenv("MI_OSQP_REFACTOR_PIPELINE_MIN")) t.pipeline_min = std::max(0, atoi(e));
   if (const char *e = getenv("MI_OSQP_REFACTOR_CHUNKS")) t.pipeline_chunks = std::max(0, std::min(8, atoi(e)));
   if (const char *e = getenv("MI_OSQP_REFACTOR_CHUNK_QPS")) t.pipeline_chunk_qps = std::max(0, atoi(e));
+  if (const char *e = getenv("MI_OSQP_REFACTOR_LANES")) t.refactor_lanes = std::max(1, std::min(3, atoi(e)));
+  if (const char *e = getenv("MI_OSQP_REFACTOR_CHUNK0")) t.lanes_chunk0 = atoi(e) != 0;
   AnalysisTuning &a = t.analysis;
   if (const char *e = getenv("MI_OSQP_DENSE_TAIL")) a.dense_tail = atoi(e);
   if (const char *e = getenv("MI_OSQP_ORDERING")) a.ordering = e[0];
@@ -981,6 +983,45 @@
   for (const auto &p : tc) { rc.tiles.push_back(p.second); rc.tile_begin[(size_t)p.first + 1]++; }
   for (int c = 0; c < rc.n_chunks; c++) rc.tile_begin[(size_t)c + 1] += rc.tile_begin[c];
   return rc;
+}
+
+RefactorLanes refactor_lanes(const RefactorChunks &ch, const std::vector<int> &flagged, int bt, int kbt, int lanes, bool chunk0_first, int scratch_slots) {
+  RefactorLanes rl;
+  const int nc = ch.n_chunks, n_ref = nc - 1;
+  bt = std::max(1, bt); kbt = std::max(1, kbt);
+  int L = std::max(1, std::min(std::min(3, lanes), std::max(1, n_ref)));
+  std::vector<int> padded((size_t)nc + 1, 0);
+  for (int c = 1; c < nc; c++) padded[(size_t)c + 1] = padded[c] + (ch.work_begin[(size_t)c + 1] - ch.work_begin[c] + kbt - 1) / kbt * kbt;
+  if (padded[nc] > scratch_slots) L = 1;
+  rl.n_lanes = L;
+  rl.lane_of.assign(nc, 0);
+  rl.order.assign(L, std::vector<int>());
+  rl.scratch_begin.assign((size_t)nc + 1, 0);
+  if (L == 1) {
+    for (int c = 0; c < nc; c++) rl.order[0].push_back(c);
+    return rl;
+  }
+  rl.scratch_begin = padded;
+  for (int c = 1; c < nc; c++) { rl.lane_of[c] = (c - 1) % L; rl.order[(c - 1) % L].push_back(c); }
+  if (chunk0_first) { rl.lane_of[0] = L - 1; rl.order[L - 1].insert(rl.order[L - 1].begin(), 0); }
+  else {
+    int at = L - 1;
+    for (int a = L - 1; a >= 0; a--) if (rl.order[a].size() < rl.order[at].size()) at = a;
+    rl.lane_of[0] = at; rl.order[at].push_back(0);
+  }
+  for (int c = 1; c < nc; c++) {
+    std::vector<char> need(nc, 0);
+    for (int t = ch.tile_begin[c]; t < ch.tile_begin[(size_t)c + 1]; t++) {
+      const int tile = ch.tiles[t];
+      size_t g = std::lower_bound(flagged.begin(), flagged.end(), tile * bt) - flagged.begin();
+      for (; g < flagged.size() && flagged[g] / bt == tile; g++) {
+        const int d = (int)(std::upper_bound(ch.work_begin.begin() + 1, ch.work_begin.end(), (int)g) - ch.work_begin.begin()) - 1;
+        if (d >= 1 && d < c && rl.lane_of[d] != rl.lane_of[c]) need[d] = 1;
+      }
+    }
+    for (int d = 1; d < c; d++) if (need[d]) { rl.wait_chunk.push_back(c); rl.wait_for.push_back(d); }
+  }
+  return rl;
 }
 
 
diff --git a/osqp-solver_amd/csrc/host_core.hpp b/osqp-solver_amd/csrc/host_core.hpp
--- a/osqp-solver_amd/csrc/host_core.hpp
+++ b/osqp-solver_amd/csrc/host_core.hpp
@@ -53,6 +53,8 @@
   int pipeline_min = 0;
   int pipeline_chunks = 0;
   int pipeline_chunk_qps = 0;
+  int refactor_lanes = 0;
+  int lanes_chunk0 = -1;
   AnalysisTuning analysis;
 };
 Tuning tuning_from_env();
@@ -64,6 +66,15 @@
   std::vector<int> tile_begin;
 };
 RefactorChunks refactor_chunks(const std::vector<int> &flagged, const std::vector<int> &active, int bt, int chunk_qps, int max_chunks);
+
+struct RefactorLanes {
+  int n_lanes = 1;
+  std::vector<int> lane_of;
+  std::vector<std::vector<int>> order;
+  std::vector<int> scratch_begin;
+  std::vector<int> wait_chunk, wait_for;
+};
+RefactorLanes refactor_lanes(const RefactorChunks &ch, const std::vector<int> &flagged, int bt, int kbt, int lanes, bool chunk0_first, int scratch_slots);
 
 struct Schedule {
   int n_phases = 0, nw = 0, bt = 1;
diff --git a/osqp-solver_amd/csrc/kernels.hip b/osqp-solver_amd/csrc/kernels.hip
--- a/osqp-solver_amd/csrc/kernels.hip
+++ b/osqp-solver_amd/csrc/kernels.hip
@@ -2123,8 +2123,9 @@
   double *Ss = smem + (size_t)(threadIdx.x >> 6) * MI_CHUNK * MI_CHUNK * BT;
   double *lds_rest = smem + (size_t)(blockDim.x >> 6) * MI_CHUNK * MI_CHUNK * BT;
   double *Lb, *Dl;
+  const size_t stile = (size_t)tile + (size_t)a.wg_base;
   if constexpr (LBL) { Lb = lds_rest; Dl = lds_rest + (size_t)a.storage * BT; }
-  else { Lb = a.Lblk + (size_t)tile * a.storage * BT; Dl = a.Dl + (size_t)tile * N * BT; }
+  else { Lb = a.Lblk + stile * a.storage * BT; Dl = a.Dl + stile * N * BT; }
   const double rho = a.dscal[H(DS_COUNT, DS_RHO)];
   if (flag && !a.force_all && !a.pmask) {
     for (int e = tid; e < m * BT; e += nthr) {
@@ -2177,7 +2178,7 @@
   int npos = 0, bad_inertia = 0;
   double *dnew;
   if constexpr (LBL) dnew = lds_rest + ((size_t)a.storage + (size_t)N) * BT;
-  else dnew = a.dinv_scratch + (size_t)tile * N * BT;
+  else dnew = a.dinv_scratch + stile * N * BT;
   for (int L = 0; L < a.n_levels; L++) {
     const uint32_t *lv = a.lvl + 6 * L;
     const uint4 *ut4 = reinterpret_cast<const uint4 *>(a.utask), *dt4 = reinterpret_cast<const uint4 *>(a.dtask), *tt4 = reinterpret_cast<const uint4 *>(a.ttask);
@@ -2347,8 +2348,8 @@
   const int lane = tid & 63, wave = __builtin_amdgcn_readfirstlane(tid >> 6);
   const int slot = a.work[g];
   if (slot < 0) return;
-  const int k = a.k, kbt = a.kbt, wt = g / kbt, wb = g % kbt;
-  double *A = a.Sd + (size_t)g * k * k;
+  const int k = a.k, kbt = a.kbt, gs = g + a.wg_base, wt = gs / kbt, wb = gs % kbt;
+  double *A = a.Sd + (size_t)gs * k * k;
   const double *Lb = a.Lblk + (size_t)wt * a.storage * kbt + wb;
   const double *Dl = a.Dl + (size_t)wt * a.N * kbt + wb;
   const int l15 = lane & 15, l4 = lane >> 4;
@@ -2421,10 +2422,10 @@
   const int lane = tid & 63, wave = __builtin_amdgcn_readfirstlane(tid >> 6);
   const int slot = a.work[g];
   if (slot < 0) return;
-  const int k = a.k, kbt = a.kbt, wt = g / kbt, wb = g % kbt, nt = k / 16;
+  const int k = a.k, kbt = a.kbt, gs = g + a.wg_base, wt = gs / kbt, wb = gs % kbt, nt = k / 16;
   const size_t hbt = (size_t)a.home_bt, home = (size_t)slot / hbt, hb = (size_t)slot % hbt;
   auto H = [&](size_t len, size_t i) { return (home * len + i) * hbt + hb; };
-  double *A = a.Sd + (size_t)g * k * k;
+  double *A = a.Sd + (size_t)gs * k * k;
   (void)wt; (void)wb;
   const int l15 = lane & 15, l4 = lane >> 4;
   unsigned long long tr_t = a.trace ? __builtin_amdgcn_s_memtime() : 0ull, tr_acc[8] = {0ull, 0ull, 0ull, 0ull, 0ull, 0ull, 0ull, 0ull};
@@ -2781,6 +2782,20 @@
     double *ds = a.dscal + tile * DS_COUNT * BT;
     ds[DS_OBJ * BT + b] = nanv; ds[DS_PRI_RES * BT + b] = nanv; ds[DS_DUA_RES * BT + b] = nanv;
   }
+}
+__global__ void fail_flagged_kernel(KernelArgs a, const int *__restrict__ slots, int BT, int iter) {
+  const int slot = slots[blockIdx.x];
+  if (slot < 0) return;
+  int *flag = a.iscal + ((size_t)slot / BT) * IS_COUNT * BT + IS_NEED_REFACTOR * BT + (size_t)slot % BT;
+  if (*flag >= 0) return;
+  fail_one_slot(a, slot, BT, iter, threadIdx.x, blockDim.x);
+  __syncthreads();
+  if (threadIdx.x == 0) *flag = 0;
+}
+hipError_t launch_fail_flagged(const KernelArgs &a, const int *slots, int nslots, int BT, int iter, hipStream_t st) {
+  if (nslots <= 0) return hipSuccess;
+  hipLaunchKernelGGL(fail_flagged_kernel, dim3(nslots), dim3(256), 0, st, a, slots, BT, iter);
+  return hipGetLastError();
 }
 __global__ void start_slots_kernel(KernelArgs a, const int *__restrict__ slots, const int *__restrict__ clear, int BT, int cold) {
   const int slot = slots[blockIdx.x], tid = threadIdx.x, nthr = blockDim.x;
diff --git a/osqp-solver_amd/csrc/solver.hip b/osqp-solver_amd/csrc/solver.hip
--- a/osqp-solver_amd/csrc/solver.hip
+++ b/osqp-solver_amd/csrc/solver.hip
@@ -168,12 +168,13 @@
 }
 namespace streampool {
 constexpr int kPipeChunks = 8;
-constexpr int kPipeEvents = 3 + 3 * kPipeChunks;
-struct Bundle { int dev; hipStream_t stream; hipEvent_t ev[5]; hipStream_t pipe_r, pipe_i; hipEvent_t pipe_ev[kPipeEvents]; };
+constexpr int kPipeLanes = 3;
+constexpr int kPipeEvents = 3 + 3 * kPipeChunks + kPipeLanes;
+struct Bundle { int dev; hipStream_t stream; hipEvent_t ev[5]; hipStream_t pipe_r, pipe_i, pipe_x; hipEvent_t pipe_ev[kPipeEvents]; };
 static void destroy(const Bundle &b) {
   for (hipEvent_t e : b.ev) if (e) (void)hipEventDestroy(e);
   for (hipEvent_t e : b.pipe_ev) if (e) (void)hipEventDestroy(e);
-  for (hipStream_t st : {b.stream, b.pipe_r, b.pipe_i}) if (st) (void)hipStreamDestroy(st);
+  for (hipStream_t st : {b.stream, b.pipe_r, b.pipe_i, b.pipe_x}) if (st) (void)hipStreamDestroy(st);
 }
 static std::mutex mu;
 static std::vector<Bundle> idle;
@@ -300,10 +301,11 @@
   double *pin = nullptr;
   size_t pin_n = 0;
   hipEvent_t ev0 = nullptr, ev1 = nullptr, evf0 = nullptr, evf1 = nullptr, evf2 = nullptr;
-  hipStream_t pipe_r = nullptr, pipe_i = nullptr;
+  hipStream_t pipe_r = nullptr, pipe_i = nullptr, pipe_x = nullptr;
   hipEvent_t pipe_ev[streampool::kPipeEvents] = {};
   DevBuf<int> tile_list;
   int64_t pipelined_refactors = 0;
+  int64_t refactor_lanes = 0;
   double factor_ms_sum = 0.0, dense_ms_sum = 0.0;
   int64_t refactor_launches = 0, refactor_qps = 0, peak_qps = 0;
   double peak_factor_ms = 0.0, peak_tail_ms = 0.0;
@@ -363,7 +365,8 @@
     hostpool::give(h_iscal, h_iscal_cap); hostpool::give(h_dscal, h_dscal_cap); hostpool::give(pin, pin_cap); hostpool::give(h_npos, h_npos_cap);
     if (pipe_r) (void)hipStreamSynchronize(pipe_r);
     if (pipe_i) (void)hipStreamSynchronize(pipe_i);
-    streampool::Bundle sb{device, stream, {ev0, ev1, evf0, evf1, evf2}, pipe_r, pipe_i, {}};
+    if (pipe_x) (void)hipStreamSynchronize(pipe_x);
+    streampool::Bundle sb{device, stream, {ev0, ev1, evf0, evf1, evf2}, pipe_r, pipe_i, pipe_x, {}};
     for (int k = 0; k < streampool::kPipeEvents; k++) sb.pipe_ev[k] = pipe_ev[k];
     if (stream && ev0 && ev1 && evf0 && evf1 && evf2) streampool::give(sb);
     else streampool::destroy(sb);
@@ -813,7 +816,7 @@
     streampool::Bundle sb;
     if (streampool::take(h->device, sb)) {
       h->stream = sb.stream; h->ev0 = sb.ev[0]; h->ev1 = sb.ev[1]; h->evf0 = sb.ev[2]; h->evf1 = sb.ev[3]; h->evf2 = sb.ev[4];
-      h->pipe_r = sb.pipe_r; h->pipe_i = sb.pipe_i;
+      h->pipe_r = sb.pipe_r; h->pipe_i = sb.pipe_i; h->pipe_x = sb.pipe_x;
       for (int k = 0; k < streampool::kPipeEvents; k++) h->pipe_ev[k] = sb.pipe_ev[k];
     }
     else {
@@ -1255,82 +1258,146 @@
   return MI_OSQP_OK;
 }
 
+struct PipeRegion {
+  bool open = false;
+  int iter = 0, n_chunks = 0, n_lanes = 1;
+  bool tail = false;
+  double host_s = 0.0;
+  std::vector<int> work, wl, tiles;
+  std::vector<int> lane_last;
+};
+constexpr int kDefaultLanes = 2;
+constexpr bool kDefaultChunk0First = false;
 static bool pipeline_applies(const mi_osqp_batch *h, int n_ref) {
   const int longer_than = h->tune.pipeline_min > 0 ? h->tune.pipeline_min : h->n_cus;
   return h->tune.refactor_pipeline && n_ref > longer_than && h->mw_groups <= 0 && !h->global_xs && !(*h->anp).wide && !(*h->anp).df;
 }
 
-static int pipelined_refactor_iterate(mi_osqp_batch *h, const KernelArgs &a, const std::vector<int> &work, const std::vector<int> &active, std::vector<int> *bad) {
-  using streampool::kPipeChunks; using streampool::kPipeEvents;
+static int pipelined_refactor_iterate(mi_osqp_batch *h, const KernelArgs &a, const std::vector<int> &work, const std::vector<int> &active, PipeRegion *pr) {
+  using streampool::kPipeChunks; using streampool::kPipeEvents; using streampool::kPipeLanes;
   const double t_begin = now_s();
   const int BT = h->BT, nq = (int)work.size();
   int rc;
   if (!h->pipe_r) HIPCHK(hipStreamCreateWithFlags(&h->pipe_r, hipStreamNonBlocking));
   if (!h->pipe_i) HIPCHK(hipStreamCreateWithFlags(&h->pipe_i, hipStreamNonBlocking));
   for (int k = 0; k < kPipeEvents; k++) if (!h->pipe_ev[k]) HIPCHK(hipEventCreate(&h->pipe_ev[k]));
-  hipEvent_t ev_fork = h->pipe_ev[0], ev_i0 = h->pipe_ev[1], ev_i1 = h->pipe_ev[2];
+  hipEvent_t ev_fork = h->pipe_ev[0], ev_i0 = h->pipe_ev[1], ev_join = h->pipe_ev[2];
   auto ev_chunk = [&](int c, int k) { return h->pipe_ev[3 + 3 * (c - 1) + k]; };
+  auto ev_lane = [&](int l) { return h->pipe_ev[3 + 3 * kPipeChunks + l]; };
   int n_even = h->tune.pipeline_chunks > 0 ? h->tune.pipeline_chunks : (nq + h->n_cus - 1) / h->n_cus;
   int chunk_qps = (nq + n_even - 1) / n_even;
   if (h->tune.pipeline_chunks <= 0 && h->tune.pipeline_chunk_qps > 0) chunk_qps = h->tune.pipeline_chunk_qps;
   const RefactorChunks ch = refactor_chunks(work, active, BT, chunk_qps, kPipeChunks);
   const int kbt = nq <= h->n_cus ? 1 : BT;
-  std::vector<int> wl, wl_begin(1, 0);
+  const int lanes_asked = h->tune.refactor_lanes > 0 ? h->tune.refactor_lanes : kDefaultLanes;
+  const RefactorLanes rl = refactor_lanes(ch, work, BT, kbt, std::min(lanes_asked, kPipeLanes), h->tune.lanes_chunk0 < 0 ? kDefaultChunk0First : h->tune.lanes_chunk0 != 0,
+                                          h->ntiles * BT + 4);
+  const int L = rl.n_lanes;
+  if (L > 2 && !h->pipe_x) HIPCHK(hipStreamCreateWithFlags(&h->pipe_x, hipStreamNonBlocking));
+  std::vector<int> &wl = pr->wl;
+  std::vector<int> wl_begin(1, 0);
+  wl.clear();
   for (int c = 1; c < ch.n_chunks; c++) {
     wl.insert(wl.end(), work.begin() + ch.work_begin[c], work.begin() + ch.work_begin[c + 1]);
     wl.resize((wl.size() + kbt - 1) / kbt * kbt, -1);
     wl_begin.push_back((int)wl.size());
   }
+  pr->tiles = ch.tiles; pr->work = work;
   if (h->work.n < wl.size() && (rc = h->work.alloc((size_t)h->ntiles * BT + 4 + (size_t)BT * kPipeChunks))) return rc;
   if (h->tile_list.n < ch.tiles.size() && (rc = h->tile_list.alloc((size_t)h->ntiles))) return rc;
   HIPCHK(hipMemcpyAsync(h->work.p, wl.data(), wl.size() * sizeof(int), hipMemcpyHostToDevice, h->stream));
-  HIPCHK(hipMemcpyAsync(h->tile_list.p, ch.tiles.data(), ch.tiles.size() * sizeof(int), hipMemcpyHostToDevice, h->stream));
-  const double t_fork = now_s();
+  HIPCHK(hipMemcpyAsync(h->tile_list.p, pr->tiles.data(), pr->tiles.size() * sizeof(int), hipMemcpyHostToDevice, h->stream));
+  pr->host_s = now_s() - t_begin;
   HIPCHK(hipEventRecord(ev_fork, h->stream));
-  HIPCHK(hipStreamWaitEvent(h->pipe_r, ev_fork, 0));
-  HIPCHK(hipStreamWaitEvent(h->pipe_i, ev_fork, 0));
   FactorArgs fa = make_factor_args(h, 0);
   const bool tail = (*h->anp).dt.k != 0;
-  for (int c = 1; c < ch.n_chunks; c++) {
+  auto enqueue_refactor = [&](int c, int base, hipStream_t st) -> int {
     const int *wc = h->work.p + wl_begin[c - 1];
     const int slots = wl_begin[c] - wl_begin[c - 1];
-    fa.work = wc;
-    HIPCHK(hipEventRecord(ev_chunk(c, 0), h->pipe_r));
-    HIPCHK(launch_factor(fa, kbt, slots / kbt, h->tune.factor_threads, h->pipe_r));
-    HIPCHK(hipEventRecord(ev_chunk(c, 1), h->pipe_r));
-    if (tail) HIPCHK(launch_tail(make_tail_args(h, kbt, wc), slots, h->dt_lds_asm, h->dt_lds, h->pipe_r));
-    HIPCHK(hipEventRecord(ev_chunk(c, 2), h->pipe_r));
-  }
+    fa.work = wc; fa.wg_base = base / kbt;
+    HIPCHK(hipEventRecord(ev_chunk(c, 0), st));
+    HIPCHK(launch_factor(fa, kbt, slots / kbt, h->tune.factor_threads, st));
+    HIPCHK(hipEventRecord(ev_chunk(c, 1), st));
+    if (tail) {
+      TailArgs da = make_tail_args(h, kbt, wc);
+      da.wg_base = base;
+      HIPCHK(launch_tail(da, slots, h->dt_lds_asm, h->dt_lds, st));
+    }
+    HIPCHK(hipEventRecord(ev_chunk(c, 2), st));
+    return 0;
+  };
   KernelArgs ai = a;
-  HIPCHK(hipEventRecord(ev_i0, h->pipe_i));
-  for (int c = 0; c < ch.n_chunks; c++) {
+  auto enqueue_iterate = [&](int c, hipStream_t st) -> int {
     const int nt = ch.tile_begin[c + 1] - ch.tile_begin[c];
-    if (c) HIPCHK(hipStreamWaitEvent(h->pipe_i, ev_chunk(c, 2), 0));
-    if (!nt) continue;
+    if (!nt) return 0;
     ai.tiles = h->tile_list.p + ch.tile_begin[c];
-    HIPCHK(launch_iterate(ai, BT, nt, h->threads, h->lds_iter + h->lds_factor, h->pipe_i));
-  }
-  HIPCHK(hipEventRecord(ev_i1, h->pipe_i));
-  HIPCHK(hipStreamWaitEvent(h->stream, ev_i1, 0));
-  HIPCHK(hipMemcpyAsync(h->h_iscal, h->iscal.p, (size_t)h->ntiles * IS_COUNT * BT * sizeof(int), hipMemcpyDeviceToHost, h->stream));
-  HIPCHK(hipStreamSynchronize(h->stream));
-  const double t_end = now_s();
-  float f_ms = 0.f, d_ms = 0.f, r_ms = 0.f, i_ms = 0.f;
-  for (int c = 1; c < ch.n_chunks; c++) {
+    HIPCHK(launch_iterate(ai, BT, nt, h->threads, h->lds_iter + h->lds_factor, st));
+    return 0;
+  };
+  pr->lane_last.assign(L, 0);
+  if (L == 1) {
+    HIPCHK(hipStreamWaitEvent(h->pipe_r, ev_fork, 0));
+    HIPCHK(hipStreamWaitEvent(h->pipe_i, ev_fork, 0));
+    for (int c = 1; c < ch.n_chunks; c++) if ((rc = enqueue_refactor(c, 0, h->pipe_r))) return rc;
+    pr->lane_last[0] = ch.n_chunks - 1;
+    HIPCHK(hipEventRecord(ev_i0, h->pipe_i));
+    for (int c = 0; c < ch.n_chunks; c++) {
+      if (c) HIPCHK(hipStreamWaitEvent(h->pipe_i, ev_chunk(c, 2), 0));
+      if ((rc = enqueue_iterate(c, h->pipe_i))) return rc;
+    }
+    HIPCHK(hipEventRecord(ev_lane(0), h->pipe_i));
+    HIPCHK(hipStreamWaitEvent(h->stream, ev_lane(0), 0));
+  } else {
+    hipStream_t lane[kPipeLanes] = {h->pipe_r, h->pipe_i, h->pipe_x};
+    for (int l = 0; l < L; l++) HIPCHK(hipStreamWaitEvent(lane[l], ev_fork, 0));
+    const bool chunk0_first = rl.order[rl.lane_of[0]].front() == 0;
+    if (chunk0_first && (rc = enqueue_iterate(0, lane[rl.lane_of[0]]))) return rc;
+    size_t w = 0;
+    for (int c = 1; c < ch.n_chunks; c++) {
+      const int l = rl.lane_of[c];
+      if ((rc = enqueue_refactor(c, rl.scratch_begin[c], lane[l]))) return rc;
+      pr->lane_last[l] = c;
+      for (; w < rl.wait_chunk.size() && rl.wait_chunk[w] == c; w++) HIPCHK(hipStreamWaitEvent(lane[l], ev_chunk(rl.wait_for[w], 2), 0));
+      if ((rc = enqueue_iterate(c, lane[l]))) return rc;
+    }
+    if (!chunk0_first && (rc = enqueue_iterate(0, lane[rl.lane_of[0]]))) return rc;
+    for (int l = 0; l < L; l++) { HIPCHK(hipEventRecord(ev_lane(l), lane[l])); HIPCHK(hipStreamWaitEvent(h->stream, ev_lane(l), 0)); }
+  }
+  HIPCHK(hipEventRecord(ev_join, h->stream));
+  HIPCHK(launch_fail_flagged(a, h->work.p, (int)wl.size(), BT, a.iter_begin, h->stream));
+  pr->open = true; pr->iter = a.iter_begin; pr->n_chunks = ch.n_chunks; pr->n_lanes = L; pr->tail = tail;
+  h->refactor_lanes = std::max<int64_t>(h->refactor_lanes, L);
+  return 0;
+}
+
+static int pipelined_region_finish(mi_osqp_batch *h, PipeRegion *pr) {
+  using streampool::kPipeChunks;
+  if (!pr->open) return 0;
+  pr->open = false;
+  const int BT = h->BT, nq = (int)pr->work.size();
+  hipEvent_t ev_fork = h->pipe_ev[0], ev_i0 = h->pipe_ev[1], ev_join = h->pipe_ev[2];
+  auto ev_chunk = [&](int c, int k) { return h->pipe_ev[3 + 3 * (c - 1) + k]; };
+  float f_ms = 0.f, d_ms = 0.f, r_ms = 0.f, i_ms = 0.f, w_ms = 0.f;
+  for (int c = 1; c < pr->n_chunks; c++) {
     float f = 0.f, d = 0.f;
     HIPCHK(hipEventElapsedTime(&f, ev_chunk(c, 0), ev_chunk(c, 1))); HIPCHK(hipEventElapsedTime(&d, ev_chunk(c, 1), ev_chunk(c, 2)));
-    f_ms += f; d_ms += tail ? d : 0.f;
-  }
-  HIPCHK(hipEventElapsedTime(&r_ms, ev_fork, ev_chunk(ch.n_chunks - 1, 2)));
-  HIPCHK(hipEventElapsedTime(&i_ms, ev_i0, ev_i1));
-  const double wall = t_end - t_begin, ref_s = std::min(wall, (t_fork - t_begin) + 1e-3 * r_ms);
+    f_ms += f; d_ms += pr->tail ? d : 0.f;
+  }
+  for (int c : pr->lane_last) {
+    float r = 0.f;
+    if (c) HIPCHK(hipEventElapsedTime(&r, ev_fork, ev_chunk(c, 2)));
+    r_ms = std::max(r_ms, r);
+  }
+  HIPCHK(hipEventElapsedTime(&w_ms, ev_fork, ev_join));
+  if (pr->n_lanes == 1) HIPCHK(hipEventElapsedTime(&i_ms, ev_i0, h->pipe_ev[3 + 3 * kPipeChunks])); else i_ms = w_ms;
+  const double wall = pr->host_s + 1e-3 * std::max(w_ms, r_ms), ref_s = pr->host_s + 1e-3 * r_ms;
   h->last_refactor_s += ref_s; h->last_device_s += wall - ref_s;
   h->kernel_ms_sum += i_ms; h->kernel_launches++; h->last_launches++;
   h->factor_ms_sum += f_ms; h->dense_ms_sum += d_ms; h->refactor_launches++; h->refactor_qps += nq;
   if (nq >= h->peak_qps) { h->peak_qps = nq; h->peak_factor_ms = f_ms; h->peak_tail_ms = d_ms; }
   h->pipelined_refactors++;
-  for (int s : work)
-    if (h->h_iscal[(size_t)(s / BT) * IS_COUNT * BT + IS_NEED_REFACTOR * BT + s % BT] < 0) bad->push_back(s);
+  for (int s : pr->work)
+    if (s >= 0 && s < h->B && h->h_iscal[(size_t)(s / BT) * IS_COUNT * BT + IS_STATUS * BT + s % BT] == -7) h->failed[s] = 1;
   return 0;
 }
 
@@ -1361,6 +1428,7 @@
   auto loop = [&]() -> int {
     int iter = 0;
     bool iterated = false;
+    PipeRegion region;
     while (true) {
       const int seg_end = segment_end(iter);
       a.iter_begin = iter; a.iter_end = seg_end; a.info_at_end = 1;
@@ -1391,7 +1459,7 @@
         float ms = 0.f;
         HIPCHK(hipEventElapsedTime(&ms, h->ev0, h->ev1));
         h->last_device_s += ms * 1e-3; h->kernel_ms_sum += ms; h->kernel_launches++; h->last_launches++;
-      }
+      } else if ((rc = pipelined_region_finish(h, &region))) return rc;
       iterated = false;
       iter = seg_end;
       std::vector<int> active, work;
@@ -1409,7 +1477,7 @@
         if (!active.empty() && pipeline_applies(h, n_ref)) {
           KernelArgs nx = a;
           nx.iter_begin = iter; nx.iter_end = segment_end(iter); nx.info_at_end = 1;
-          if ((rc2 = pipelined_refactor_iterate(h, nx, work, active, &bad))) return rc2;
+          if ((rc2 = pipelined_refactor_iterate(h, nx, work, active, &region))) return rc2;
           iterated = true;
           tr = now_s();
         } else if ((rc2 = device_refactor_slots(h, std::move(work), &bad))) return rc2;
@@ -1431,6 +1499,7 @@
   if (rc) {
     if (h->pipe_r) (void)hipStreamSynchronize(h->pipe_r);
     if (h->pipe_i) (void)hipStreamSynchronize(h->pipe_i);
+    if (h->pipe_x) (void)hipStreamSynchronize(h->pipe_x);
     (void)hipStreamSynchronize(h->stream);
     return rc;
   }
@@ -1700,6 +1769,7 @@
   if (!h || !st) return MI_OSQP_ERR_NULL;
   *st = h->stats;
   st->pipelined_refactors = h->pipelined_refactors;
+  st->refactor_lanes = h->refactor_lanes;
   return MI_OSQP_OK;
 }
 
@@ -3381,6 +3451,30 @@
   std::copy(ch.tile_begin.begin(), ch.tile_begin.end(), tile_begin);
   return MI_OSQP_OK;
 }
+int mi_osqp_debug_refactor_lanes(int64_t n_flagged, const int64_t *flagged, int64_t n_active, const int64_t *active, int64_t tile,
+                                 int64_t chunk_qps, int64_t max_chunks, int64_t kbt, int64_t lanes, int64_t chunk0_first,
+                                 int64_t scratch_slots, int64_t *n_lanes, int64_t *lane_of, int64_t *order, int64_t *order_begin,
+                                 int64_t *scratch_begin, int64_t *n_waits, int64_t *wait_chunk, int64_t *wait_for) {
+  if (!n_lanes || !lane_of || !order || !order_begin || !scratch_begin || !n_waits || !wait_chunk || !wait_for ||
+      (n_flagged > 0 && !flagged) || (n_active > 0 && !active)) return MI_OSQP_ERR_NULL;
+  if (n_flagged < 0 || n_active < 0 || tile < 1 || chunk_qps < 1 || max_chunks < 1 || kbt < 1 || lanes < 1 || lanes > 3 || scratch_slots < 0)
+    return MI_OSQP_ERR_INVALID_DATA;
+  const std::vector<int> f(flagged, flagged + n_flagged), a(active, active + n_active);
+  const RefactorChunks ch = refactor_chunks(f, a, (int)tile, (int)chunk_qps, (int)max_chunks);
+  const RefactorLanes rl = refactor_lanes(ch, f, (int)tile, (int)kbt, (int)lanes, chunk0_first != 0, (int)std::min<int64_t>(scratch_slots, INT32_MAX));
+  *n_lanes = rl.n_lanes;
+  std::copy(rl.lane_of.begin(), rl.lane_of.end(), lane_of);
+  order_begin[0] = 0;
+  for (int l = 0; l < rl.n_lanes; l++) {
+    std::copy(rl.order[l].begin(), rl.order[l].end(), order + order_begin[l]);
+    order_begin[l + 1] = order_begin[l] + (int64_t)rl.order[l].size();
+  }
+  std::copy(rl.scratch_begin.begin(), rl.scratch_begin.begin() + ch.n_chunks, scratch_begin);
+  *n_waits = (int64_t)rl.wait_chunk.size();
+  std::copy(rl.wait_chunk.begin(), rl.wait_chunk.end(), wait_chunk);
+  std::copy(rl.wait_for.begin(), rl.wait_for.end(), wait_for);
+  return MI_OSQP_OK;
+}
 int mi_osqp_get_stats(mi_osqp_solver *h, mi_osqp_stats *st) { return h ? mi_osqp_batch_get_stats(h->b, st) : MI_OSQP_ERR_NULL; }
 int mi_osqp_get_settings(mi_osqp_solver *h, mi_osqp_settings *out) { return h ? mi_osqp_batch_get_settings(h->b, out) : MI_OSQP_ERR_NULL; }
 int mi_osqp_update_settings(mi_osqp_solver *h, const mi_osqp_settings *s) { return h ? mi_osqp_batch_update_settings(h->b, s) : MI_OSQP_ERR_NULL; }
```

Measured after the change: 39720 (median of 6 runs). 2.4% higher.
